# SuperScientificSoftwareLaboratory/PanguLU

Hardware: AMD Instinct MI355X
Metric: numeric factorisation GFLOP/s (pangulu_gstrf, R64) (higher is better)
Workload: dtype f64

## Files before the change

include/pangulu_platform.h:

```cpp
#ifndef PANGULU_PLATFORM_H
#define PANGULU_PLATFORM_H

#include <stddef.h>
#include <stdint.h>

typedef long long int pangulu_int64_t;
typedef unsigned long long int pangulu_uint64_t;
typedef int pangulu_int32_t;
typedef unsigned int pangulu_uint32_t;
typedef short int pangulu_int16_t;
typedef unsigned short int pangulu_uint16_t;

typedef pangulu_uint64_t pangulu_exblock_ptr;
typedef pangulu_uint32_t pangulu_exblock_idx;
typedef pangulu_uint32_t pangulu_inblock_ptr;
typedef pangulu_uint16_t pangulu_inblock_idx;

#if defined(CALCULATE_TYPE_CR64)
#define PANGULU_COMPLEX 1
typedef double calculate_real_type;
#elif defined(CALCULATE_TYPE_CR32)
#define PANGULU_COMPLEX 1
typedef float calculate_real_type;
#elif defined(CALCULATE_TYPE_R32)
typedef float calculate_real_type;
#else
#ifndef CALCULATE_TYPE_R64
#define CALCULATE_TYPE_R64
#endif
typedef double calculate_real_type;
#endif

#ifdef PANGULU_COMPLEX
#if defined(__cplusplus)
typedef struct pangulu_complex_t
{
    calculate_real_type re, im;
} calculate_type;
#elif defined(CALCULATE_TYPE_CR64)
typedef double _Complex calculate_type;
#else
typedef float _Complex calculate_type;
#endif
#else
typedef calculate_real_type calculate_type;
#endif

#define PANGULU_TASK_GETRF 1
#define PANGULU_TASK_TSTRF 2
#define PANGULU_TASK_GESSM 3
#define PANGULU_TASK_SSSSM 4
#define PANGULU_LOWER 0
#define PANGULU_UPPER 1
#define PANGULU_DATA_INVALID 0
#define PANGULU_DATA_PREPARING 1
#define PANGULU_DATA_READY 2
#define PANGULU_TOL 1e-16
#define PANGULU_SPTRSV_TOL 1e-16

#define PANGULU_PLATFORM_CPU_NAIVE 0x0100000
#define PANGULU_PLATFORM_GPU_CUDA 0x0201000
#define PANGULU_PLATFORM_GPU_HIP 0x0201001

#ifdef __cplusplus
extern "C"
{
#endif

    typedef struct pangulu_aggregate_queue_t
    {
        unsigned long long capacity;
        unsigned long long length;
        void *task_descriptors;
    } pangulu_aggregate_queue_t;

    typedef struct pangulu_storage_slot_t
    {
        pangulu_exblock_idx brow_pos;
        pangulu_exblock_idx bcol_pos;
        pangulu_inblock_ptr *columnpointer;
        pangulu_inblock_idx *rowindex;
        calculate_type *value;
        pangulu_inblock_ptr *rowpointer;
        pangulu_inblock_idx *columnindex;
        pangulu_inblock_ptr *idx_of_csc_value_for_csr;
        volatile char data_status;
        struct pangulu_storage_slot_t *related_block;
        pangulu_int32_t is_upper;
        pangulu_int32_t bin_id;
        pangulu_int32_t slot_idx;
        pangulu_aggregate_queue_t *task_queue;
        pangulu_inblock_ptr *d_columnpointer;
        pangulu_inblock_idx *d_rowindex;
        calculate_type *d_value;
        pangulu_inblock_ptr *d_rowpointer;
        pangulu_inblock_idx *d_columnindex;
        pangulu_inblock_ptr *d_idx_of_csc_value_for_csr;
    } pangulu_storage_slot_t;

    typedef struct pangulu_task_t
    {
        pangulu_exblock_idx row;
        pangulu_exblock_idx col;
        pangulu_int16_t kernel_id;
        pangulu_exblock_idx task_level;
        pangulu_int64_t compare_flag;
        pangulu_storage_slot_t *opdst;
        pangulu_storage_slot_t *op1;
        pangulu_storage_slot_t *op2;
    } pangulu_task_t;

#if defined(__cplusplus)
    static_assert(sizeof(pangulu_storage_slot_t) == 144, "slot ABI must match src/pangulu_common.h:207-231 (GPU_OPEN)");
    static_assert(offsetof(pangulu_storage_slot_t, value) == 24, "slot ABI");
    static_assert(offsetof(pangulu_storage_slot_t, related_block) == 64, "slot ABI");
    static_assert(offsetof(pangulu_storage_slot_t, d_columnpointer) == 96, "slot ABI");
    static_assert(offsetof(pangulu_storage_slot_t, d_value) == 112, "slot ABI");
    static_assert(sizeof(pangulu_task_t) == 48, "task ABI must match src/pangulu_common.h:233-243");
    static_assert(offsetof(pangulu_task_t, opdst) == 24, "task ABI");
#endif

    extern int pangulu_gpu_kernel_warp_per_block;
    extern int pangulu_gpu_data_move_warp_per_block;
    extern int pangulu_gpu_shared_mem_size;

    void pangulu_platform_0201001_malloc(void **platform_address, size_t size);
    void pangulu_platform_0201001_malloc_pinned(void **platform_address, size_t size);
    void pangulu_platform_0201001_synchronize(void);
    void pangulu_platform_0201001_memset(void *s, int c, size_t n);
    void pangulu_platform_0201001_create_stream(void **stream);
    void pangulu_platform_0201001_memcpy(void *dst, const void *src, size_t count, unsigned int kind);
    void pangulu_platform_0201001_memcpy_async(void *dst, const void *src, size_t count, unsigned int kind, void *stream);
    void pangulu_platform_0201001_free(void *devptr);
    void pangulu_platform_0201001_get_device_num(int *device_num);
    void pangulu_platform_0201001_set_default_device(int device_num);
    void pangulu_platform_0201001_get_device_name(char *name, int device_num);
    void pangulu_platform_0201001_get_device_memory_usage(size_t *used_byte);

    void pangulu_platform_0201001_getrf(pangulu_inblock_idx nb, pangulu_storage_slot_t *opdst, int tid);
    void pangulu_platform_0201001_tstrf(pangulu_inblock_idx nb, pangulu_storage_slot_t *opdst, pangulu_storage_slot_t *opdiag, int tid);
    void pangulu_platform_0201001_gessm(pangulu_inblock_idx nb, pangulu_storage_slot_t *opdst, pangulu_storage_slot_t *opdiag, int tid);
    void pangulu_platform_0201001_ssssm(pangulu_inblock_idx nb, pangulu_storage_slot_t *opdst, pangulu_storage_slot_t *op1, pangulu_storage_slot_t *op2, int tid);
    void pangulu_platform_0201001_ssssm_batched(pangulu_inblock_idx nb, pangulu_uint64_t ntask, pangulu_task_t *tasks);
    void pangulu_platform_0201001_hybrid_batched(pangulu_inblock_idx nb, pangulu_uint64_t ntask, pangulu_task_t *tasks);

    void pangulu_platform_0201001_spmv(pangulu_inblock_idx nb, pangulu_storage_slot_t *a, calculate_type *x, calculate_type *y);
    void pangulu_platform_0201001_vecadd(pangulu_int64_t length, calculate_type *bval, calculate_type *xval);
    void pangulu_platform_0201001_sptrsv(pangulu_inblock_idx nb, pangulu_storage_slot_t *s, calculate_type *xval, pangulu_int64_t uplo);

#define PANGULU_HIP_OPT_HOST_MIRROR 1
#define PANGULU_HIP_OPT_DENSE_THRESHOLD_PERMILLE 2
#define PANGULU_HIP_OPT_PROFILE 3
#define PANGULU_HIP_OPT_ASSUME_INDEPENDENT 4
#define PANGULU_HIP_OPT_GETRF_STRICT_ORDER 5
#define PANGULU_HIP_OPT_COUNT_FLOPS 6
#define PANGULU_HIP_OPT_RESET_BLOCK_STATE 7
#define PANGULU_HIP_OPT_SSSSM_GROUP_CHUNK 8
#define PANGULU_HIP_OPT_TRSM_DENSE_PERMILLE 9
#define PANGULU_HIP_OPT_TWO_STREAMS 10
#define PANGULU_HIP_OPT_SMALL_LAUNCH_TASKS 11
#define PANGULU_HIP_OPT_XCD_SWIZZLE 12
#define PANGULU_HIP_OPT_RECORDS_STREAM 13
#define PANGULU_HIP_OPT_BACKGROUND_UPDATES 14
#define PANGULU_HIP_OPT_FRONT_STAGES 15
#define PANGULU_HIP_OPT_TILES_STAGES 16
#define PANGULU_HIP_OPT_QUERY_FREE_MIB 17
    int pangulu_platform_0201001_set_option(int option, long long value);
    void pangulu_platform_0201001_prepare_diag(pangulu_inblock_idx nb, pangulu_storage_slot_t *diag);
    void pangulu_platform_0201001_prepare_blocks(pangulu_inblock_idx nb, pangulu_uint64_t nslot, pangulu_storage_slot_t **slots);
    void *pangulu_platform_0201001_marker_record(void);
    int pangulu_platform_0201001_marker_done(void *marker);
    void pangulu_platform_0201001_marker_wait(void *marker);
    typedef struct pangulu_hip_solve_row_t
    {
        pangulu_exblock_idx brow, nblk;
        pangulu_uint64_t first;
        pangulu_storage_slot_t *diag;
    } pangulu_hip_solve_row_t;
    void pangulu_platform_0201001_block_trsv(pangulu_inblock_idx nb, int upper, pangulu_uint64_t nlevel, const pangulu_uint64_t *level_ptr,
                                             const pangulu_hip_solve_row_t *rows, pangulu_storage_slot_t *const *blk_slots,
                                             const pangulu_exblock_idx *blk_bcol, calculate_type *x, pangulu_uint64_t xlen);
    typedef struct pangulu_hip_solve_sweep_t
    {
        pangulu_uint64_t nlevel;
        const pangulu_uint64_t *level_ptr;
        const pangulu_hip_solve_row_t *rows;
        pangulu_storage_slot_t *const *blk_slots;
        const pangulu_exblock_idx *blk_bcol;
    } pangulu_hip_solve_sweep_t;
    int pangulu_platform_0201001_block_trsm_multi(pangulu_inblock_idx nb, const pangulu_hip_solve_sweep_t *lower, const pangulu_hip_solve_sweep_t *upper,
                                                  calculate_type *X, pangulu_uint64_t xlen, pangulu_uint64_t npanel, const int *w);
    int pangulu_platform_0201001_block_trsm_multi_trans(pangulu_inblock_idx nb, const pangulu_hip_solve_sweep_t *forward_ut,
                                                        const pangulu_hip_solve_sweep_t *backward_lt, int conjugate, calculate_type *X,
                                                        pangulu_uint64_t xlen, pangulu_uint64_t npanel, const int *w);
    typedef struct pangulu_hip_solve_maps_t
    {
        pangulu_uint64_t n, n_user;
        const unsigned int *in_idx, *out_idx;
        const double *s_in, *s_out;
    } pangulu_hip_solve_maps_t;
    int pangulu_platform_0201001_block_trsm_multi_device(pangulu_inblock_idx nb, const pangulu_hip_solve_sweep_t *first,
                                                         const pangulu_hip_solve_sweep_t *second, int mode, calculate_type *d_rhs,
                                                         pangulu_uint64_t ldb, pangulu_uint64_t nrhs, pangulu_uint64_t npanel, const int *w,
                                                         pangulu_uint64_t xlen, const pangulu_hip_solve_maps_t *maps, void **workspace,
                                                         void *caller_stream);
    void pangulu_platform_0201001_solve_workspace_free(void **workspace);
    unsigned long long pangulu_platform_0201001_get_solve_workspace_bytes(void);
    void pangulu_platform_0201001_block_spmv_add(pangulu_inblock_idx nb, pangulu_uint64_t nblk, pangulu_storage_slot_t *const *slots,
                                                 const pangulu_exblock_idx *src_seg, const pangulu_exblock_idx *dst_seg, const int *csr,
                                                 const calculate_type *x, calculate_type *y, pangulu_uint64_t xlen);
    int pangulu_platform_0201001_bind_near_device(int enable);
    long long pangulu_platform_0201001_schedule(int cmd, const void *owner);
    int pangulu_platform_0201001_schedule_range(const void *owner, long long first, long long last);
    void *pangulu_platform_0201001_marker_record_replay(void);
    void *pangulu_platform_0201001_get_stream(void);
#define PANGULU_HIP_STAT_CLASSES 9
    typedef struct pangulu_hip_stats_t
    {
        unsigned long long launches[PANGULU_HIP_STAT_CLASSES];
        unsigned long long tasks[PANGULU_HIP_STAT_CLASSES];
        double alg_bytes[PANGULU_HIP_STAT_CLASSES];
        double flops[PANGULU_HIP_STAT_CLASSES];
        double elapsed_ms[PANGULU_HIP_STAT_CLASSES];
        double mfma_flops_executed;
        unsigned long long trsm_dense_tasks;
        unsigned long long ssssm_front_workgroups, ssssm_general_workgroups;
        unsigned long long chase_launches, chase_solves;
        double ssssm_kernel_ms[2];
        double ssssm_front_flops_executed;
    } pangulu_hip_stats_t;
    void pangulu_platform_0201001_get_stats(pangulu_hip_stats_t *out, int reset);
    void pangulu_platform_0201001_get_memory(unsigned long long out[4]);

#ifdef __cplusplus
}
#endif

#endif
```

pangulu_amd/_lib.py:

```python
import ctypes
import os

import numpy as np

_HERE = os.path.dirname(os.path.abspath(__file__))
REPO_ROOT = os.path.dirname(_HERE)
LIB_DIR = os.environ.get("PANGULU_AMD_LIB_DIR") or os.path.join(_HERE, "lib")

VALUE_TYPES = {
    "r64": (np.float64, 8, 0),
    "r32": (np.float32, 4, 0),
    "cr64": (np.complex128, 16, 1),
    "cr32": (np.complex64, 8, 1),
}


class InitOptions(ctypes.Structure):

    _fields_ = [
        ("nthread", ctypes.c_int),
        ("nb", ctypes.c_int),
        ("gpu_kernel_warp_per_block", ctypes.c_int),
        ("gpu_data_move_warp_per_block", ctypes.c_int),
        ("sizeof_value", ctypes.c_int),
        ("is_complex_matrix", ctypes.c_int),
        ("mpi_recv_buffer_level", ctypes.c_float),
    ]


class GstrfOptions(ctypes.Structure):
    _fields_ = [("reserved_", ctypes.c_char)]


class GstrsOptions(ctypes.Structure):
    _fields_ = [("reserved_", ctypes.c_char)]


class Info(ctypes.Structure):

    _fields_ = [
        ("n", ctypes.c_ulonglong),
        ("nnz", ctypes.c_ulonglong),
        ("nb", ctypes.c_ulonglong),
        ("block_length", ctypes.c_ulonglong),
        ("n_padded", ctypes.c_ulonglong),
        ("symbolic_nnz", ctypes.c_ulonglong),
        ("flop", ctypes.c_longlong),
        ("nblocks_nondiag", ctypes.c_ulonglong),
        ("nblocks_owned", ctypes.c_ulonglong),
        ("ntask_getrf", ctypes.c_ulonglong),
        ("ntask_tstrf", ctypes.c_ulonglong),
        ("ntask_gessm", ctypes.c_ulonglong),
        ("ntask_ssssm", ctypes.c_ulonglong),
        ("owned_bytes", ctypes.c_ulonglong),
        ("recv_blocks", ctypes.c_ulonglong),
        ("sent_bytes", ctypes.c_ulonglong),
        ("recv_bytes", ctypes.c_ulonglong),
        ("time_reorder", ctypes.c_double),
        ("time_symbolic", ctypes.c_double),
        ("time_preprocess", ctypes.c_double),
        ("time_numeric", ctypes.c_double),
        ("time_solve", ctypes.c_double),
        ("time_numeric_host_sched", ctypes.c_double),
        ("model_bytes_total", ctypes.c_double),
        ("model_flop_total", ctypes.c_double),
        ("model_tmin_hbm_bound", ctypes.c_double),
        ("model_tmin_fp_bound", ctypes.c_double),
        ("batches", ctypes.c_ulonglong),
        ("sampled_flop", ctypes.c_double),
        ("sampled_tasks", ctypes.c_ulonglong),
        ("time_numeric_platform", ctypes.c_double),
        ("replayed", ctypes.c_ulonglong),
        ("time_schedule_record", ctypes.c_double),
        ("model_ranks_tstar_max", ctypes.c_double),
        ("model_ranks_tstar_sum", ctypes.c_double),
        ("model_ranks_tstar_hbm", ctypes.c_double),
        ("model_ranks_tstar_fp", ctypes.c_double),
        ("model_ranks_bytes_total", ctypes.c_double),
        ("model_rank_flop_share", ctypes.c_double),
        ("model_rank_time_share", ctypes.c_double),
        ("model_comm_seconds_max", ctypes.c_double),
        ("model_sent_bytes_total", ctypes.c_double),
        ("model_critical_path", ctypes.c_double),
        ("model_critical_path_tasks", ctypes.c_ulonglong),
        ("snapshot_device_bytes", ctypes.c_ulonglong),
        ("model_critical_path_latency", ctypes.c_double),
        ("model_rank_hbm_bytes_max", ctypes.c_double),
        ("model_rank_hbm_records", ctypes.c_double),
        ("model_rank_hbm_received", ctypes.c_double),
        ("model_rank_hbm_mirrors", ctypes.c_double),
        ("inserted_diagonals", ctypes.c_ulonglong),
        ("deferred_queues", ctypes.c_ulonglong),
    ]

    def as_dict(self):
        return {name: getattr(self, name) for name, _ in self._fields_}


class HipStats(ctypes.Structure):

    _fields_ = [
        ("launches", ctypes.c_ulonglong * 9),
        ("tasks", ctypes.c_ulonglong * 9),
        ("alg_bytes", ctypes.c_double * 9),
        ("flops", ctypes.c_double * 9),
        ("elapsed_ms", ctypes.c_double * 9),
        ("mfma_flops_executed", ctypes.c_double),
        ("trsm_dense_tasks", ctypes.c_ulonglong),
        ("ssssm_front_workgroups", ctypes.c_ulonglong),
        ("ssssm_general_workgroups", ctypes.c_ulonglong),
        ("chase_launches", ctypes.c_ulonglong),
        ("chase_solves", ctypes.c_ulonglong),
        ("ssssm_kernel_ms", ctypes.c_double * 2),
        ("ssssm_front_flops_executed", ctypes.c_double),
    ]


KERNEL_CLASSES = {1: "getrf", 2: "tstrf", 3: "gessm", 4: "ssssm_sparse", 5: "ssssm_dense_mfma",
                  6: "densify", 7: "sparsify", 8: "remote_lu_image"}

_cache = {}


def library_path(vtype="r64"):
    return os.path.join(LIB_DIR, "libpangulu_amd_%s.so" % vtype)


def test_library_path(vtype="r64"):
    return os.path.join(REPO_ROOT, "oracle", "_build", "libpangulu_amd_test_%s.so" % vtype)


def load(vtype="r64", test_hooks=False):
    vtype = vtype.lower()
    key = (vtype, bool(test_hooks))
    if key in _cache:
        return _cache[key]
    path = test_library_path(vtype) if test_hooks else library_path(vtype)
    if not os.path.exists(path):
        raise RuntimeError(
            "%s is missing: build it with `python -c 'import __graft_entry__ as g; g.build()'` "
            "(or `make -C pangulu_amd/csrc TYPE=%s`); there is no fallback implementation" % (path, vtype.upper())
        )
    lib = ctypes.CDLL(path, mode=ctypes.RTLD_LOCAL)
    vp, vpp = ctypes.c_void_p, ctypes.POINTER(ctypes.c_void_p)
    lib.pangulu_init.argtypes = [ctypes.c_uint32, ctypes.c_uint64, vp, vp, vp, ctypes.POINTER(InitOptions), vpp]
    lib.pangulu_init.restype = None
    lib.pangulu_gstrf.argtypes = [ctypes.POINTER(GstrfOptions), vpp]
    lib.pangulu_gstrf.restype = None
    lib.pangulu_gstrs.argtypes = [vp, ctypes.POINTER(GstrsOptions), vpp]
    lib.pangulu_gstrs.restype = None
    lib.pangulu_amd_gstrs_multi.argtypes = [vp, ctypes.c_uint32, ctypes.c_uint64, ctypes.POINTER(GstrsOptions), vpp]
    lib.pangulu_amd_gstrs_multi.restype = ctypes.c_int
    lib.pangulu_amd_gstrs_trans.argtypes = [vp, ctypes.c_uint32, ctypes.c_uint64, ctypes.c_int, ctypes.POINTER(GstrsOptions), vpp]
    lib.pangulu_amd_gstrs_trans.restype = ctypes.c_int
    lib.pangulu_amd_gstrs_device.argtypes = [vp, ctypes.c_uint32, ctypes.c_uint64, ctypes.c_int, vp, ctypes.POINTER(GstrsOptions), vpp]
    lib.pangulu_amd_gstrs_device.restype = ctypes.c_int
    lib.pangulu_amd_last_solve_path.argtypes = [vpp, ctypes.POINTER(ctypes.c_int), ctypes.POINTER(ctypes.c_int), ctypes.POINTER(ctypes.c_int)]
    lib.pangulu_amd_last_solve_path.restype = ctypes.c_int
    lib.pangulu_gssv.argtypes = [vp, ctypes.POINTER(GstrfOptions), ctypes.POINTER(GstrsOptions), vpp]
    lib.pangulu_gssv.restype = None
    lib.pangulu_finalize.argtypes = [vpp]
    lib.pangulu_finalize.restype = None

    lib.pangulu_amd_comm_init.argtypes = [ctypes.c_int, ctypes.c_int, ctypes.c_char_p, ctypes.c_int, ctypes.c_int, vp]
    lib.pangulu_amd_comm_init.restype = ctypes.c_int
    lib.pangulu_amd_comm_barrier.restype = None
    lib.pangulu_amd_comm_allreduce_max_f64.argtypes = [vp, ctypes.c_int]
    lib.pangulu_amd_comm_allreduce_max_f64.restype = None
    lib.pangulu_amd_comm_finalize.restype = None
    lib.pangulu_amd_comm_transport.restype = ctypes.c_int
    lib.pangulu_amd_comm_rccl_ranks.restype = ctypes.c_int
    lib.pangulu_amd_comm_rank.restype = ctypes.c_int
    lib.pangulu_amd_comm_size.restype = ctypes.c_int
    if test_hooks:
        lib.pangulu_amd_use_platform_library.argtypes = [ctypes.c_char_p, ctypes.c_uint]
        lib.pangulu_amd_use_platform_library.restype = ctypes.c_int
    lib.pangulu_amd_active_platform.restype = ctypes.c_uint
    lib.pangulu_amd_use_builtin_platform.restype = None
    lib.pangulu_amd_set_ordering.argtypes = [ctypes.c_int]
    lib.pangulu_amd_set_ordering.restype = None
    lib.pangulu_amd_set_user_perm.argtypes = [vp, ctypes.c_uint32]
    lib.pangulu_amd_set_user_perm.restype = None
    lib.pangulu_amd_set_coordinates.argtypes = [vp, ctypes.c_uint32, ctypes.c_int]
    lib.pangulu_amd_set_coordinates.restype = None
    lib.pangulu_amd_set_eager_host_mirror.argtypes = [ctypes.c_int]
    lib.pangulu_amd_set_eager_host_mirror.restype = None
    lib.pangulu_amd_set_scaling.argtypes = [ctypes.c_int]
    lib.pangulu_amd_set_scaling.restype = None
    lib.pangulu_amd_reset_options.restype = None
    lib.pangulu_amd_get_info.argtypes = [vpp, ctypes.POINTER(Info)]
    lib.pangulu_amd_get_info.restype = None
    lib.pangulu_amd_model_roofline.argtypes = [vpp, ctypes.c_double, ctypes.c_double]
    lib.pangulu_amd_model_roofline.restype = None
    lib.pangulu_amd_block_owner.argtypes = [vpp, ctypes.c_uint32, ctypes.c_uint32]
    lib.pangulu_amd_block_owner.restype = ctypes.c_int
    lib.pangulu_amd_rank_model.argtypes = [vpp, vp, vp, vp]
    lib.pangulu_amd_rank_model.restype = ctypes.c_int
    lib.pangulu_amd_owned_block_count.argtypes = [vpp]
    lib.pangulu_amd_owned_block_count.restype = ctypes.c_longlong
    lib.pangulu_amd_owned_block.argtypes = [
        vpp, ctypes.c_longlong, ctypes.POINTER(ctypes.c_uint32), ctypes.POINTER(ctypes.c_uint32),
        ctypes.POINTER(ctypes.c_int), ctypes.POINTER(ctypes.c_ulonglong), vpp, vpp, vpp,
    ]
    lib.pangulu_amd_owned_block.restype = ctypes.c_int
    lib.pangulu_amd_update_values.argtypes = [vpp, vp]
    lib.pangulu_amd_update_values.restype = ctypes.c_int
    lib.pangulu_amd_snapshot.argtypes = [vpp]
    lib.pangulu_amd_snapshot.restype = ctypes.c_int
    lib.pangulu_amd_reset_numeric.argtypes = [vpp]
    lib.pangulu_amd_reset_numeric.restype = ctypes.c_int
    lib.pangulu_amd_set_replay.argtypes = [ctypes.c_int]
    lib.pangulu_amd_set_replay.restype = ctypes.c_int
    lib.pangulu_amd_get_perm.argtypes = [vpp]
    lib.pangulu_amd_get_perm.restype = ctypes.POINTER(ctypes.c_uint32)
    lib.pangulu_amd_apply_lu.argtypes = [vpp, vp, vp]
    lib.pangulu_amd_apply_lu.restype = ctypes.c_int
    lib.pangulu_amd_factor_check.argtypes = [vpp, ctypes.POINTER(ctypes.c_double)]
    lib.pangulu_amd_factor_check.restype = ctypes.c_int
    lib.pangulu_amd_factor_check_vectors.argtypes = [vpp, ctypes.c_int, ctypes.c_ulonglong, ctypes.POINTER(ctypes.c_double)]
    lib.pangulu_amd_factor_check_vectors.restype = ctypes.c_int
    lib.pangulu_amd_model_for_ranks.argtypes = [vpp, ctypes.c_int, ctypes.POINTER(ctypes.c_double)]
    lib.pangulu_amd_model_for_ranks.restype = ctypes.c_int

    lib.pangulu_platform_0201001_set_option.argtypes = [ctypes.c_int, ctypes.c_longlong]
    lib.pangulu_platform_0201001_set_option.restype = ctypes.c_int
    lib.pangulu_platform_0201001_get_stats.argtypes = [ctypes.POINTER(HipStats), ctypes.c_int]
    lib.pangulu_platform_0201001_get_stats.restype = None
    lib.pangulu_platform_0201001_get_stream.restype = ctypes.c_void_p
    lib.pangulu_platform_0201001_get_solve_workspace_bytes.restype = ctypes.c_ulonglong
    _cache[key] = lib
    return lib


PLATFORM_SYMBOLS = [
    "malloc", "malloc_pinned", "synchronize", "memset", "create_stream", "memcpy", "memcpy_async", "free",
    "get_device_num", "set_default_device", "get_device_name", "get_device_memory_usage",
    "getrf", "tstrf", "gessm", "ssssm", "ssssm_batched", "hybrid_batched", "spmv", "vecadd", "sptrsv",
]

HIP_OPT_HOST_MIRROR = 1
HIP_OPT_DENSE_THRESHOLD_PERMILLE = 2
HIP_OPT_PROFILE = 3
HIP_OPT_ASSUME_INDEPENDENT = 4
HIP_OPT_GETRF_STRICT_ORDER = 5
HIP_OPT_COUNT_FLOPS = 6
HIP_OPT_RESET_BLOCK_STATE = 7
HIP_OPT_SSSSM_GROUP_CHUNK = 8
HIP_OPT_TRSM_DENSE_PERMILLE = 9
HIP_OPT_TWO_STREAMS = 10
HIP_OPT_SMALL_LAUNCH_TASKS = 11
HIP_OPT_XCD_SWIZZLE = 12
HIP_OPT_RECORDS_STREAM = 13
HIP_OPT_BACKGROUND_UPDATES = 14
HIP_OPT_FRONT_STAGES = 15
HIP_OPT_TILES_STAGES = 16

ORDER_IDENTITY, ORDER_ND, ORDER_USER = 0, 1, 2
TRANSPORT_HOST, TRANSPORT_RCCL, TRANSPORT_IPC = 0, 1, 2
PLATFORM_CPU_NAIVE = 0x0100000
PLATFORM_GPU_HIP = 0x0201001
```

pangulu_amd/csrc/host/pg_api.cpp:

```cpp
#include <cmath>
#include <cstdarg>
#include <dlfcn.h>
#include <omp.h>
#include <sys/time.h>

#include <sys/mman.h>
#include "pg_host.h"

namespace pg
{
#ifdef PANGULU_COMPLEX
static inline val_t make_value(double re) { return val_t{(decltype(val_t{}.re))re, 0}; }
#else
static inline val_t make_value(double re) { return (val_t)re; }
#endif


void fatal(const char *fmt, ...)
{
    va_list ap;
    va_start(ap, fmt);
    fprintf(stderr, "[PanguLU-AMD ERROR] ");
    vfprintf(stderr, fmt, ap);
    fprintf(stderr, "\n");
    va_end(ap);
    fflush(stderr);
    exit(1);
}

double wall_seconds()
{
    struct timeval tv;
    gettimeofday(&tv, nullptr);
    return (double)tv.tv_sec + 1e-6 * (double)tv.tv_usec;
}

static Platform g_platform;
static bool g_platform_ready = false;
static bool g_platform_builtin = true;

void bind_builtin_hip(Platform &p)
{
    p = Platform();
    p.id = PANGULU_PLATFORM_GPU_HIP;
    p.host_memory = false;
    p.malloc_ = pangulu_platform_0201001_malloc;
    p.malloc_pinned = pangulu_platform_0201001_malloc_pinned;
    p.synchronize = pangulu_platform_0201001_synchronize;
    p.memset_ = pangulu_platform_0201001_memset;
    p.create_stream = pangulu_platform_0201001_create_stream;
    p.memcpy_ = pangulu_platform_0201001_memcpy;
    p.memcpy_async = pangulu_platform_0201001_memcpy_async;
    p.free_ = pangulu_platform_0201001_free;
    p.get_device_num = pangulu_platform_0201001_get_device_num;
    p.set_default_device = pangulu_platform_0201001_set_default_device;
    p.get_device_name = pangulu_platform_0201001_get_device_name;
    p.get_device_memory_usage = pangulu_platform_0201001_get_device_memory_usage;
    p.getrf = pangulu_platform_0201001_getrf;
    p.tstrf = pangulu_platform_0201001_tstrf;
    p.gessm = pangulu_platform_0201001_gessm;
    p.ssssm = pangulu_platform_0201001_ssssm;
    p.ssssm_batched = pangulu_platform_0201001_ssssm_batched;
    p.hybrid_batched = pangulu_platform_0201001_hybrid_batched;
    p.spmv = pangulu_platform_0201001_spmv;
    p.vecadd = pangulu_platform_0201001_vecadd;
    p.sptrsv = pangulu_platform_0201001_sptrsv;
    p.set_option = pangulu_platform_0201001_set_option;
    p.prepare_diag = pangulu_platform_0201001_prepare_diag;
    p.prepare_blocks = pangulu_platform_0201001_prepare_blocks;
    p.marker_record = pangulu_platform_0201001_marker_record;
    p.marker_done = pangulu_platform_0201001_marker_done;
    p.marker_wait = pangulu_platform_0201001_marker_wait;
    p.block_trsv = pangulu_platform_0201001_block_trsv;
    p.block_trsm_multi = pangulu_platform_0201001_block_trsm_multi;
    p.block_trsm_multi_trans = pangulu_platform_0201001_block_trsm_multi_trans;
    p.block_trsm_multi_device = pangulu_platform_0201001_block_trsm_multi_device;
    p.solve_workspace_free = pangulu_platform_0201001_solve_workspace_free;
    p.block_spmv_add = pangulu_platform_0201001_block_spmv_add;
    p.schedule = pangulu_platform_0201001_schedule;
    p.schedule_range = pangulu_platform_0201001_schedule_range;
    p.marker_record_replay = pangulu_platform_0201001_marker_record_replay;
    p.bind_near_device = pangulu_platform_0201001_bind_near_device;
}

Platform &active_platform()
{
    if (!g_platform_ready)
    {
        bind_builtin_hip(g_platform);
        g_platform_ready = true;
        g_platform_builtin = true;
    }
    return g_platform;
}

bool platform_is_builtin_hip() { return g_platform_builtin; }

static Options g_options;
Options &pending_options() { return g_options; }

}

using namespace pg;

namespace
{
struct NearDevice
{
    Platform &plat;
    bool bound = false;
    explicit NearDevice(Platform &p) : plat(p)
    {
        if (!plat.host_memory && plat.bind_near_device)
        {
#pragma omp parallel
            {
            }
            bound = plat.bind_near_device(1) == 0;
        }
    }
    ~NearDevice()
    {
        if (bound)
            plat.bind_near_device(0);
    }
};

inline val_t value_times(val_t v, double s)
{
#ifdef PANGULU_COMPLEX
    return val_t{(calculate_real_type)(v.re * s), (calculate_real_type)(v.im * s)};
#else
    return (val_t)(v * s);
#endif
}
}

const SolveMaps &pg::solve_maps(Solver &S, bool transposed)
{
    SolveMaps &M = S.solve_maps[transposed ? 1 : 0];
    if (M.ready)
        return M;
    const bool scaled = !S.scale_row.empty();
    std::vector<u32> row_idx(S.n, SOLVE_MAP_PAD), col_idx(S.n, SOLVE_MAP_PAD);
    std::vector<double> row_s, col_s;
    if (scaled)
    {
        row_s.assign(S.n, 0.0);
        col_s.assign(S.n, 0.0);
    }
    for (u32 i = 0; i < S.n; i++)
    {
        const u32 j = S.perm[i];
        if (j >= S.n_user)
            continue;
        row_idx[i] = j;
        col_idx[i] = scaled ? S.match_col[j] : j;
        if (scaled)
        {
            row_s[i] = S.scale_row[j];
            col_s[i] = S.scale_col[S.match_col[j]];
        }
    }
    M.in_idx = transposed ? col_idx : row_idx;
    M.out_idx = transposed ? row_idx : col_idx;
    M.s_in = transposed ? col_s : row_s;
    M.s_out = transposed ? row_s : col_s;
    M.ready = true;
    return M;
}

namespace
{
void rhs_into_factor_space(const SolveMaps &M, u32 n, const val_t *rhs, val_t *b)
{
    const bool scaled = !M.s_in.empty();
    for (u32 i = 0; i < n; i++)
    {
        if (M.in_idx[i] == SOLVE_MAP_PAD)
            memset(&b[i], 0, sizeof(val_t));
        else
            b[i] = scaled ? value_times(rhs[M.in_idx[i]], M.s_in[i]) : rhs[M.in_idx[i]];
    }
}
void solution_out_of_factor_space(const SolveMaps &M, u32 n, const val_t *b, val_t *rhs)
{
    const bool scaled = !M.s_out.empty();
    for (u32 i = 0; i < n; i++)
        if (M.out_idx[i] != SOLVE_MAP_PAD)
            rhs[M.out_idx[i]] = scaled ? value_times(b[i], M.s_out[i]) : b[i];
}
void rhs_to_factor_space(Solver &S, const val_t *rhs, val_t *b) { rhs_into_factor_space(solve_maps(S, false), S.n, rhs, b); }
void solution_from_factor_space(Solver &S, const val_t *b, val_t *rhs) { solution_out_of_factor_space(solve_maps(S, false), S.n, b, rhs); }
void rhs_to_factor_space_trans(Solver &S, const val_t *rhs, val_t *b) { rhs_into_factor_space(solve_maps(S, true), S.n, rhs, b); }
void solution_from_factor_space_trans(Solver &S, const val_t *b, val_t *rhs) { solution_out_of_factor_space(solve_maps(S, true), S.n, b, rhs); }
}

extern "C"
{

#ifdef PANGULU_AMD_TEST_HOOKS
    int pangulu_amd_use_platform_library(const char *so_path, unsigned int platform_id)
    {
        void *h = dlopen(so_path, RTLD_NOW | RTLD_LOCAL);
        if (!h)
        {
            fprintf(stderr, "[PanguLU-AMD] cannot load platform library %s: %s\n", so_path, dlerror());
            return 1;
        }
        Platform p;
        p.id = platform_id;
        p.dl_handle = h;
        p.host_memory = (platform_id >> 20) == 0x01;
        char sym[128];
        int missing = 0;
        auto get = [&](const char *name) -> void *
        {
            snprintf(sym, sizeof(sym), "pangulu_platform_%07x_%s", platform_id, name);
            void *f = dlsym(h, sym);
            if (!f)
            {
                fprintf(stderr, "[PanguLU-AMD] %s lacks %s\n", so_path, sym);
                missing++;
            }
            return f;
        };
        p.malloc_ = (void (*)(void **, size_t))get("malloc");
        p.malloc_pinned = (void (*)(void **, size_t))get("malloc_pinned");
        p.synchronize = (void (*)())get("synchronize");
        p.memset_ = (void (*)(void *, int, size_t))get("memset");
        p.create_stream = (void (*)(void **))get("create_stream");
        p.memcpy_ = (void (*)(void *, const void *, size_t, unsigned))get("memcpy");
        p.memcpy_async = (void (*)(void *, const void *, size_t, unsigned, void *))get("memcpy_async");
        p.free_ = (void (*)(void *))get("free");
        p.get_device_num = (void (*)(int *))get("get_device_num");
        p.set_default_device = (void (*)(int))get("set_default_device");
        p.get_device_name = (void (*)(char *, int))get("get_device_name");
        p.get_device_memory_usage = (void (*)(size_t *))get("get_device_memory_usage");
        p.getrf = (void (*)(pangulu_inblock_idx, slot_t *, int))get("getrf");
        p.tstrf = (void (*)(pangulu_inblock_idx, slot_t *, slot_t *, int))get("tstrf");
        p.gessm = (void (*)(pangulu_inblock_idx, slot_t *, slot_t *, int))get("gessm");
        p.ssssm = (void (*)(pangulu_inblock_idx, slot_t *, slot_t *, slot_t *, int))get("ssssm");
        p.ssssm_batched = (void (*)(pangulu_inblock_idx, pangulu_uint64_t, task_t *))get("ssssm_batched");
        p.hybrid_batched = (void (*)(pangulu_inblock_idx, pangulu_uint64_t, task_t *))get("hybrid_batched");
        p.spmv = (void (*)(pangulu_inblock_idx, slot_t *, val_t *, val_t *))get("spmv");
        p.vecadd = (void (*)(pangulu_int64_t, val_t *, val_t *))get("vecadd");
        p.sptrsv = (void (*)(pangulu_inblock_idx, slot_t *, val_t *, pangulu_int64_t))get("sptrsv");
        if (missing)
            return 2;
        snprintf(sym, sizeof(sym), "pangulu_platform_%07x_block_trsm_multi_trans", platform_id);
        p.block_trsm_multi_trans = (int (*)(pangulu_inblock_idx, const pangulu_hip_solve_sweep_t *, const pangulu_hip_solve_sweep_t *, int, val_t *,
                                            pangulu_uint64_t, pangulu_uint64_t, const int *))dlsym(h, sym);
        snprintf(sym, sizeof(sym), "pangulu_platform_%07x_block_trsm_multi_device", platform_id);
        p.block_trsm_multi_device = (decltype(p.block_trsm_multi_device))dlsym(h, sym);
        snprintf(sym, sizeof(sym), "pangulu_platform_%07x_solve_workspace_free", platform_id);
        p.solve_workspace_free = (decltype(p.solve_workspace_free))dlsym(h, sym);
        int (*sz)() = (int (*)())dlsym(h, "pangulu_oracle_sizeof_value");
        if (sz && sz() != (int)sizeof(val_t))
        {
            fprintf(stderr, "[PanguLU-AMD] %s was built for another value type\n", so_path);
            return 3;
        }
        g_platform = p;
        g_platform_ready = true;
        g_platform_builtin = false;
        return 0;
    }

    void pangulu_amd_test_set_analysis_ranks(int size) { set_fake_world(size); }

    void pangulu_amd_test_set_task_sampling(int stride) { g_task_sample_stride = stride < 1 ? 1 : stride; }

    long long pangulu_amd_test_heap_script(long long nscript, const long long *script, const pangulu_task_t *tasks, pangulu_task_t *out)
    {
        TaskHeap heap;
        long long npop = 0;
        for (long long i = 0; i < nscript; i++)
        {
            if (script[i] >= 0)
                heap.push(tasks[script[i]]);
            else if (!heap.pop(out[npop++]))
                return -2;
        }
        return npop;
    }

    int pangulu_amd_test_matching(sparse_index_t n, const sparse_pointer_t *colptr, const sparse_index_t *rowidx, const sparse_value_t *value,
                                  sparse_index_t *col_of_row, double *dr, double *dc)
    {
        CscMatrix A;
        A.n = n;
        A.colptr.assign(colptr, colptr + n + 1);
        A.rowidx.assign(rowidx, rowidx + colptr[n]);
        A.value.assign((const val_t *)value, (const val_t *)value + colptr[n]);
        std::vector<u32> q;
        std::vector<double> r, c;
        if (!max_product_matching(A, q, r, c))
            return 1;
        std::copy(q.begin(), q.end(), col_of_row);
        std::copy(r.begin(), r.end(), dr);
        std::copy(c.begin(), c.end(), dc);
        return 0;
    }

    int pangulu_amd_test_symbolic(sparse_index_t n, const sparse_pointer_t *colptr, const sparse_index_t *rowidx,
                                  sparse_pointer_t **out_ptr, sparse_index_t **out_idx, unsigned long long *out_symbolic_nnz, long long *out_flop)
    {
        CscMatrix A;
        A.n = n;
        A.colptr.assign(colptr, colptr + n + 1);
        A.rowidx.assign(rowidx, rowidx + colptr[n]);
        A.value.assign((size_t)colptr[n], val_t());
        Symbolic sym;
        symbolic_factorize(A, sym);
        *out_ptr = (sparse_pointer_t *)malloc(sizeof(sparse_pointer_t) * ((size_t)n + 1));
        *out_idx = (sparse_index_t *)malloc(sizeof(sparse_index_t) * std::max<size_t>(1, sym.idx.size()));
        std::copy(sym.ptr.begin(), sym.ptr.end(), *out_ptr);
        std::copy(sym.idx.begin(), sym.idx.end(), *out_idx);
        *out_symbolic_nnz = sym.symbolic_nnz;
        *out_flop = sym.flop;
        return 0;
    }
#endif

    void pangulu_amd_use_builtin_platform(void)
    {
        bind_builtin_hip(g_platform);
        g_platform_ready = true;
        g_platform_builtin = true;
    }

    unsigned int pangulu_amd_active_platform(void) { return active_platform().id; }

    int pangulu_amd_comm_init(int rank, int size, const char *addr, int base_port, int transport, const void *nccl_unique_id)
    {
        if (size <= 1)
        {
            set_world(nullptr);
            return 0;
        }
        if (size > 64)
        {
            fprintf(stderr, "[PanguLU-AMD ERROR] %d ranks requested: at most 64 are supported\n", size);
            return 1;
        }
        Platform &plat = active_platform();
        if (!plat.host_memory && plat.get_device_num && plat.set_default_device)
        {
            int ndev = 0;
            plat.get_device_num(&ndev);
            if (ndev > 0)
            {
                const char *lr = getenv("LOCAL_RANK");
                plat.set_default_device(lr ? atoi(lr) % ndev : rank % ndev);
// ... 793 lines not shown
```

pangulu_amd/csrc/host/pg_host.h:

```cpp
#pragma once

#include <atomic>
#include <condition_variable>
#include <cstdint>
#include <cstdio>
#include <cstdlib>
#include <cstring>
#include <mutex>
#include <string>
#include <thread>
#include <deque>
#include <vector>

#include "../../../include/pangulu_amd_ext.h"

namespace pg
{

using u16 = uint16_t;
using u32 = uint32_t;
using u64 = uint64_t;
using i32 = int32_t;
using i64 = int64_t;
using val_t = calculate_type;
using slot_t = pangulu_storage_slot_t;
using task_t = pangulu_task_t;

[[noreturn]] void fatal(const char *fmt, ...);
double wall_seconds();

struct Platform
{
    unsigned id = 0;
    bool host_memory = false;
    void *dl_handle = nullptr;
    void (*malloc_)(void **, size_t) = nullptr;
    void (*malloc_pinned)(void **, size_t) = nullptr;
    void (*synchronize)() = nullptr;
    void (*memset_)(void *, int, size_t) = nullptr;
    void (*create_stream)(void **) = nullptr;
    void (*memcpy_)(void *, const void *, size_t, unsigned) = nullptr;
    void (*memcpy_async)(void *, const void *, size_t, unsigned, void *) = nullptr;
    void (*free_)(void *) = nullptr;
    void (*get_device_num)(int *) = nullptr;
    void (*set_default_device)(int) = nullptr;
    void (*get_device_name)(char *, int) = nullptr;
    void (*get_device_memory_usage)(size_t *) = nullptr;
    void (*getrf)(pangulu_inblock_idx, slot_t *, int) = nullptr;
    void (*tstrf)(pangulu_inblock_idx, slot_t *, slot_t *, int) = nullptr;
    void (*gessm)(pangulu_inblock_idx, slot_t *, slot_t *, int) = nullptr;
    void (*ssssm)(pangulu_inblock_idx, slot_t *, slot_t *, slot_t *, int) = nullptr;
    void (*ssssm_batched)(pangulu_inblock_idx, pangulu_uint64_t, task_t *) = nullptr;
    void (*hybrid_batched)(pangulu_inblock_idx, pangulu_uint64_t, task_t *) = nullptr;
    void (*spmv)(pangulu_inblock_idx, slot_t *, val_t *, val_t *) = nullptr;
    void (*vecadd)(pangulu_int64_t, val_t *, val_t *) = nullptr;
    void (*sptrsv)(pangulu_inblock_idx, slot_t *, val_t *, pangulu_int64_t) = nullptr;
    int (*set_option)(int, long long) = nullptr;
    void (*prepare_diag)(pangulu_inblock_idx, slot_t *) = nullptr;
    void (*prepare_blocks)(pangulu_inblock_idx, pangulu_uint64_t, slot_t **) = nullptr;
    void *(*marker_record)() = nullptr;
    int (*marker_done)(void *) = nullptr;
    void (*marker_wait)(void *) = nullptr;
    int (*bind_near_device)(int) = nullptr;
    void (*block_trsv)(pangulu_inblock_idx, int, pangulu_uint64_t, const pangulu_uint64_t *, const pangulu_hip_solve_row_t *, slot_t *const *,
                       const pangulu_exblock_idx *, val_t *, pangulu_uint64_t) = nullptr;
    long long (*schedule)(int, const void *) = nullptr;
    int (*schedule_range)(const void *, long long, long long) = nullptr;
    void *(*marker_record_replay)() = nullptr;
    void (*block_spmv_add)(pangulu_inblock_idx, pangulu_uint64_t, slot_t *const *, const pangulu_exblock_idx *, const pangulu_exblock_idx *, const int *,
                           const val_t *, val_t *, pangulu_uint64_t) = nullptr;
    int (*block_trsm_multi)(pangulu_inblock_idx, const pangulu_hip_solve_sweep_t *, const pangulu_hip_solve_sweep_t *, val_t *, pangulu_uint64_t,
                            pangulu_uint64_t, const int *) = nullptr;
    int (*block_trsm_multi_trans)(pangulu_inblock_idx, const pangulu_hip_solve_sweep_t *, const pangulu_hip_solve_sweep_t *, int, val_t *,
                                  pangulu_uint64_t, pangulu_uint64_t, const int *) = nullptr;
    int (*block_trsm_multi_device)(pangulu_inblock_idx, const pangulu_hip_solve_sweep_t *, const pangulu_hip_solve_sweep_t *, int, val_t *,
                                   pangulu_uint64_t, pangulu_uint64_t, pangulu_uint64_t, const int *, pangulu_uint64_t,
                                   const pangulu_hip_solve_maps_t *, void **, void *) = nullptr;
    void (*solve_workspace_free)(void **) = nullptr;
};
Platform &active_platform();
bool platform_is_builtin_hip();

struct CscMatrix
{
    u32 n = 0;
    std::vector<u64> colptr;
    std::vector<u32> rowidx;
    std::vector<val_t> value;
    u64 nnz() const { return colptr.empty() ? 0 : colptr.back(); }
};

void order_identity(u32 n, std::vector<u32> &perm);
void order_nested_dissection(const CscMatrix &A, const double *coords, int dim, u32 align, std::vector<u32> &perm);
void permute_symmetric(const CscMatrix &A, const std::vector<u32> &perm, CscMatrix &B);

struct Symbolic
{
    u32 n = 0;
    std::vector<u64> ptr;
    std::vector<u32> idx;
    u64 symbolic_nnz = 0;
    i64 flop = 0;
};
void symbolic_factorize(const CscMatrix &A, Symbolic &S);

struct BlockPattern
{
    u32 nb = 0, nbk = 0, n = 0;
    std::vector<u64> lcolptr;
    std::vector<u32> lrowidx;
    std::vector<u32> lnnz;
    std::vector<u64> colptr, first_after_diag;
    std::vector<u32> rowidx;
    std::vector<u64> rowptr, first_after_diag_csr, csr_to_csc;
    std::vector<u32> colidx;
    std::vector<u32> nnz;
    std::vector<u32> diag_lower_nnz;
    std::vector<u32> diag_upper_nnz;
    u64 find(u32 br, u32 bc) const;
};
void build_block_pattern(const Symbolic &S, u32 nb, BlockPattern &P);

size_t record_bytes(u32 nb, u64 nnz, bool lower_offdiag);
void bind_record(slot_t &s, u32 nb, u64 nnz, char *hrec, char *drec, bool lower_offdiag, bool diag_upper);

struct RecvBin
{
    size_t slot_capacity = 0;
    std::vector<slot_t> slots;
    std::deque<i32> free_list;
    char *hbuf = nullptr, *dbuf = nullptr;
};

struct Storage
{
    u32 nb = 0;
    std::vector<slot_t> owned;
    size_t n_owned_nondiag = 0;
    char *harena = nullptr, *darena = nullptr;
    std::vector<char *> dchunks;
    size_t dchunk_bytes = 0;
    char *device_ptr(size_t off) const { return dchunks.empty() ? darena + off : dchunks[off / dchunk_bytes] + off % dchunk_bytes; }
    size_t chunk_len(size_t c) const { return std::min(dchunk_bytes, arena_bytes - c * dchunk_bytes); }
    size_t arena_bytes = 0;
    std::vector<RecvBin> bins;
    std::mutex mutex;
    slot_t *allocate(size_t bytes);
    void recycle(slot_t *s);
};

struct TaskHeap
{
    std::vector<task_t> store;
    std::vector<i64> heap;
    std::vector<i64> free_ids;
    std::mutex mutex;
    void reserve(size_t cap);
    void clear();
    void push(const task_t &t);
    bool pop(task_t &out);
    bool empty();
    size_t size();
    static bool before(const task_t &a, const task_t &b);
};

struct BlockHeader
{
    u64 nnz;
    u32 brow, bcol;
    u32 is_upper;
    u32 bytes_lo;
    u64 reserved;
};
static_assert(sizeof(BlockHeader) == 32, "record header is 32 bytes");

struct Marker
{
    std::atomic<void *> ev{nullptr};
};

class Comm
{
public:
    int rank = 0, size = 1;
    int transport = PANGULU_AMD_TRANSPORT_HOST;
    virtual ~Comm() {}
    virtual void barrier() = 0;
    virtual void bcast(void *buf, size_t bytes, int root) = 0;
    virtual void allreduce_sum_i64(i64 *v, int count) = 0;
    virtual void allreduce_max_f64(double *v, int count) = 0;
    virtual void send_bytes(int dst, int tag, const void *buf, size_t bytes) = 0;
    virtual void recv_bytes(int src, int tag, void *buf, size_t bytes) = 0;
    virtual void isend_block(slot_t *s, const BlockHeader &h, int dst) = 0;
    virtual bool probe_block(BlockHeader &h, int &src) = 0;
    virtual void recv_block(slot_t *s, const BlockHeader &h, int src) = 0;
    virtual void recv_block_begin(slot_t *s, const BlockHeader &h, int src) { recv_block(s, h, src); }
    virtual void recv_blocks_finish() {}
    virtual void flush_sends() = 0;
    virtual bool set_send_gate(Marker * ) { return false; }
    virtual void register_arena(char *const * , size_t , size_t , size_t ) {}
    u64 sent_bytes = 0, recv_bytes_total = 0;
    virtual int rccl_ranks() const { return 0; }
    bool abandoned = false;
};
Comm *world();
void set_world(Comm *c);
void set_fake_world(int size);
Comm *make_socket_comm(int rank, int size, const char *addr, int base_port, int transport, const void *nccl_id);
int rccl_make_unique_id(void *out128);
Comm *make_rccl_comm(int rank, int size, const char *addr, int base_port, const void *nccl_id);
Comm *make_ipc_comm(int rank, int size, const char *addr, int base_port);

bool max_product_matching(const CscMatrix &A, std::vector<u32> &col_of_row, std::vector<double> &dr, std::vector<double> &dc);
void apply_matching(const CscMatrix &A, const std::vector<u32> &col_of_row, const std::vector<double> &dr, const std::vector<double> &dc, CscMatrix &out);

struct Options
{
    bool scaling = false;
    int ordering = PANGULU_AMD_ORDER_ND;
    std::vector<u32> user_perm;
    std::vector<double> coords;
    int coord_dim = 0;
    bool eager_host_mirror = false;
};
Options &pending_options();

struct TaskModel
{
    double bytes[5] = {0, 0, 0, 0, 0};
    double flop[5] = {0, 0, 0, 0, 0};
    u64 count[5] = {0, 0, 0, 0, 0};
};

struct StructureModel
{
    double hbm_bytes_per_s = 8e12, fp_flops_per_s = 78.6e12, link_bytes_per_s = 153e9;
    std::vector<u16> lcount;
    std::vector<double> col_time, col_flop;
    std::vector<double> rank_time_hbm, rank_time_fp, rank_flop, rank_bytes, rank_comm_s;
    std::vector<double> sent_bytes;
    std::vector<double> rank_mem_records, rank_mem_recv, rank_mem_mirrors;
    double critical_path_s = 0;
    double critical_path_latency_s = 0;
    u64 critical_path_tasks = 0;
};

struct SolveSweepPlan
{
    u32 nlevel = 0;
    std::vector<pangulu_uint64_t> level_ptr;
    std::vector<pangulu_hip_solve_row_t> rows;
    std::vector<slot_t *> blk_slots;
    std::vector<pangulu_exblock_idx> blk_bcol;
};

constexpr u32 SOLVE_MAP_PAD = 0xffffffffu;
struct SolveMaps
{
    std::vector<u32> in_idx, out_idx;
    std::vector<double> s_in, s_out;
    bool ready = false;
};

struct Solver
{
    u32 n = 0, nb = 0, nbk = 0;
    u32 n_user = 0;
    int rank = 0, nproc = 1, p = 1, q = 1;
    float recv_buffer_level = 0.5f;
    bool eager_host_mirror = false;
    std::vector<u32> match_col;
    std::vector<double> scale_row, scale_col;
    std::vector<u32> perm, iperm;
    Symbolic sym;
    BlockPattern pat;
    CscMatrix Aperm;
    std::vector<u64> user_colptr;
    std::vector<u32> user_rowidx;
    Storage storage;
    std::vector<slot_t *> slot_of;
    std::vector<slot_t *> diag_lower, diag_upper;
    std::vector<i32> remain;
    std::vector<u64> consumers;
    std::vector<i32> remain_diag;
    std::vector<i32> remain0, remain_diag0;
    i64 rank_remain_task = 0, rank_remain_task0 = 0;
    i64 rank_remain_recv = 0, rank_remain_recv0 = 0;
    TaskHeap heap;
    std::mutex info_mutex;
    std::vector<std::vector<task_t>> pending;
    std::vector<u32> pending_dirty;
    u64 pending_total = 0;
    bool factored = false, host_values_current = true;
    bool schedule_recorded = false;
    SolveSweepPlan solve_plan[2];
    bool solve_plan_ready = false;
    SolveSweepPlan solve_plan_trans[2];
    bool solve_plan_trans_ready = false;
    int last_solve_device_columns = 0, last_solve_panel_width = 0, last_solve_panels = 0;
    SolveMaps solve_maps[2];
    void *solve_workspace = nullptr;
    struct RankLog
    {
        struct Entry
        {
            long long op_end = 0;
            int marker = -1;
            u32 need = 0;
        };
        struct Send
        {
            int marker;
            slot_t *slot;
            BlockHeader h;
            int dst;
        };
        struct Arrival
        {
            u32 brow, bcol, is_upper;
            slot_t *slot;
            u64 nnz;
        };
        std::vector<Entry> entries;
        std::vector<Send> sends;
        std::vector<Arrival> arrivals;
        int nmarkers = 0;
        bool valid = false, slot_reused = false;
        bool unusable = false;
    };
    RankLog rank_log;
    char *arena_snapshot = nullptr;
    bool snapshot_on_host = false;
    std::vector<char *> snapshot_dchunks;
    pangulu_amd_info_t info;
    TaskModel model;
    StructureModel smodel;
    std::vector<int> home;
    struct Group
    {
        unsigned short lo, p, q;
    };
    std::vector<Group> grp;
    bool analysis_only = false;
    int owner(u32 br, u32 bc) const
    {
        if (!home.empty())
        {
            const u32 c = br < bc ? br : bc;
            const int h = home[c];
            if (h >= 0)
                return h;
            if (!grp.empty())
            {
                const Group &g = grp[c];
                return (int)(g.lo + (br % g.p) * g.q + (bc % g.q));
            }
        }
        return (int)((br % (u32)p) * (u32)q + (bc % (u32)q));
    }
    ~Solver();
};

void assign_subtrees(Solver &S);
void preprocess(Solver &S, const CscMatrix &Aperm);
void scatter_values(Solver &S, const CscMatrix &Aperm);
void reload_values(Solver &S, const CscMatrix &Aperm);
void numeric_factorize(Solver &S);
void record_schedule(Solver &S);
void download_factors(Solver &S);
void triangular_solve(Solver &S, val_t *rhs_permuted);
void triangular_solve_multi(Solver &S, val_t *B, u32 nrhs);
void triangular_solve_multi_trans(Solver &S, val_t *B, u32 nrhs, bool conjugate);
const SolveMaps &solve_maps(Solver &S, bool transposed);
int triangular_solve_device(Solver &S, val_t *d_rhs, u32 nrhs, u64 ldb, int trans, void *stream);
void drop_solve_workspace(Solver &S);
double factor_check(Solver &S);
double factor_check_vectors(Solver &S, int nvec, unsigned long long seed);
void compute_task_model(Solver &S, double hbm_bytes_per_s, double fp_flops_per_s);
void build_structure_model(Solver &S);
void evaluate_model_for_ranks(Solver &S, int nranks, double *out12);
void compute_rank_model(Solver &S);
double task_structural_flop(u32 nb, const task_t &t);
extern int g_task_sample_stride;
extern int g_replay_enabled;

}
```

pangulu_amd/csrc/host/pg_preprocess.cpp:

```cpp
#include <algorithm>
#include <cmath>
#include <queue>
#include <string>
#include <omp.h>
#include <sys/mman.h>

#include "pg_host.h"

namespace pg
{

static inline size_t pad8(size_t x) { return (x + 7) & ~(size_t)7; }

size_t record_bytes(u32 nb, u64 nnz, bool lower_offdiag)
{
    size_t sz = 32 + sizeof(val_t) * nnz + sizeof(pangulu_inblock_ptr) * (nb + 1) + sizeof(pangulu_inblock_idx) * nnz;
    sz = pad8(sz);
    if (lower_offdiag)
    {
        sz += sizeof(pangulu_inblock_ptr) * nnz + sizeof(pangulu_inblock_ptr) * (nb + 1) + sizeof(pangulu_inblock_idx) * nnz;
        sz = pad8(sz);
    }
    return sz;
}
// ... 186 lines not shown
            w.lo = 0;
            w.cnt = np;
            todo.push_back(std::move(w));
        }
        while (!todo.empty())
        {
            Work w = std::move(todo.back());
            todo.pop_back();
            if (w.nodes.empty())
                continue;
            if (w.cnt == 1)
            {
                for (u32 k : w.nodes)
                    whole_subtree_to(k, w.lo);
                continue;
            }
            if (w.nodes.size() == 1)
            {
                const u32 k = w.nodes[0];
                if (own[k] >= heavy_abs || own[k] >= heavy_rel)
                {
                    int p = (int)std::sqrt((double)w.cnt);
                    while (w.cnt % p)
                        p--;
                    S.grp[k] = Solver::Group{(unsigned short)w.lo, (unsigned short)p, (unsigned short)(w.cnt / p)};
                    for (int r = w.lo; r < w.lo + w.cnt; r++)
                        load[(size_t)r] += own[k] / w.cnt;
                    ndist++;
                }
                else
                {
                    int best = w.lo;
                    for (int r = w.lo; r < w.lo + w.cnt; r++)
                        if (load[(size_t)r] < load[(size_t)best])
                            best = r;
                    S.home[k] = best;
                    load[(size_t)best] += own[k];
                }
                Work next;
                next.nodes = kids[k];
                next.lo = w.lo;
                next.cnt = w.cnt;
                todo.push_back(std::move(next));
                continue;
            }
            std::sort(w.nodes.begin(), w.nodes.end(), [&](u32 a, u32 b)
                      { return sub[a] > sub[b] || (sub[a] == sub[b] && a < b); });
            double wsum = 0;
            for (u32 k : w.nodes)
                wsum += sub[k];
            const double ideal0 = wsum > 0 ? sub[w.nodes[0]] / wsum * w.cnt : 0.0;
            Work h[2];
            if (ideal0 >= (double)w.cnt - 0.5)
            {
                for (size_t t = 1; t < w.nodes.size(); t++)
                {
                    int best = w.lo;
                    for (int r = w.lo; r < w.lo + w.cnt; r++)
                        if (load[(size_t)r] < load[(size_t)best])
                            best = r;
                    whole_subtree_to(w.nodes[t], best);
                }
                h[0].nodes.assign(1, w.nodes[0]);
                h[0].lo = w.lo;
                h[0].cnt = w.cnt;
            }
            else if (ideal0 >= 1.0)
            {
                const int c0 = std::max(1, std::min(w.cnt - 1, (int)std::floor(ideal0 + 0.5)));
                h[0].nodes.assign(1, w.nodes[0]);
                h[0].lo = w.lo;
                h[0].cnt = c0;
                h[1].nodes.assign(w.nodes.begin() + 1, w.nodes.end());
                h[1].lo = w.lo + c0;
                h[1].cnt = w.cnt - c0;
            }
            else
            {
                h[0].lo = w.lo;
                h[0].cnt = (w.cnt + 1) / 2;
                h[1].lo = w.lo + h[0].cnt;
                h[1].cnt = w.cnt - h[0].cnt;
                double wt[2] = {0, 0};
                for (u32 k : w.nodes)
                {
                    const int side = (wt[0] / h[0].cnt <= wt[1] / h[1].cnt) ? 0 : 1;
                    h[side].nodes.push_back(k);
                    wt[side] += sub[k];
                }
            }
            todo.push_back(std::move(h[1]));
            todo.push_back(std::move(h[0]));
        }
    }
    else
    {
        const char *per_env = getenv("PANGULU_AMD_SUBTREES_PER_RANK");
        const double per_rank = per_env ? atof(per_env) : 8.0;
        const double target = total / (per_rank * (double)np);
        auto cmp = [&](u32 a, u32 b)
        { return sub[a] < sub[b] || (sub[a] == sub[b] && a > b); };
        std::priority_queue<u32, std::vector<u32>, decltype(cmp)> pq(cmp);
        for (u32 k = 0; k < nbk; k++)
            if (parent[k] == NONE)
                pq.push(k);
        while (!pq.empty() && sub[pq.top()] > target)
        {
            u32 k = pq.top();
            pq.pop();
            for (u32 c : kids[k])
                pq.push(c);
        }
        while (!pq.empty())
        {
            u32 root = pq.top();
            pq.pop();
            whole_subtree_to(root, (int)(std::min_element(load.begin(), load.end()) - load.begin()));
        }
        if (mode == "rank0")
        {
            for (u32 k = 0; k < nbk; k++)
                if (S.home[k] < 0)
                    S.home[k] = 0;
        }
        else if (mode == "path")
        {
            for (u32 k = 0; k < nbk; k++)
                if (S.home[k] < 0)
                {
                    int best = -1;
                    double w = -1;
                    for (u32 c : kids[k])
                        if (S.home[c] >= 0 && sub[c] > w)
                        {
                            w = sub[c];
                            best = S.home[c];
                        }
                    S.home[k] = best >= 0 ? best : 0;
                }
        }
        else if (mode != "cyclic")
            fatal("PANGULU_AMD_SEPARATOR_MAP must be group, path, cyclic or rank0");
    }
    if (S.rank == 0 && getenv("PANGULU_AMD_TRACE"))
    {
        size_t top = 0;
        for (int h : S.home)
            top += h < 0;
        fprintf(stderr, "[pangulu_amd trace] mapping '%s': %zu whole subtrees over %d ranks, %zu of %u block columns distributed block-cyclic (%zu over rank groups)\n",
                mode.c_str(), nsub, np, top, nbk, ndist);
    }
}

void scatter_values(Solver &S, const CscMatrix &A)
{
    const BlockPattern &P = S.pat;
    const u32 nb = S.nb, n = S.n;
    const int me = S.rank;
#pragma omp parallel for schedule(dynamic, 256)
    for (i64 j_ = 0; j_ < (i64)n; j_++)
    {
        u32 j = (u32)j_, bj = j / nb, c = j % nb;
        for (u64 p = A.colptr[j]; p < A.colptr[j + 1]; p++)
        {
            u32 i = A.rowidx[p], bi = i / nb, r = i % nb;
            slot_t *s = nullptr;
            bool csr_row_search = false;
            if (bi == bj)
            {
                if (i > j)
                    s = S.diag_lower[bj];
                else
                {
                    s = S.diag_upper[bj];
                    csr_row_search = true;
                }
            }
            else
            {
                if (S.owner(bi, bj) != me)
                    continue;
                u64 b = P.find(bi, bj);
                if (b == ~0ull)
                    fatal("entry (%u,%u) of A outside the symbolic block pattern", i, j);
                s = S.slot_of[b];
            }
            if (!s)
                continue;
            u32 major = csr_row_search ? r : c, minor = csr_row_search ? c : r;
            const pangulu_inblock_idx *b0 = s->rowindex + s->columnpointer[major];
            const pangulu_inblock_idx *b1 = s->rowindex + s->columnpointer[major + 1];
            const pangulu_inblock_idx *hit = std::lower_bound(b0, b1, (pangulu_inblock_idx)minor);
            if (hit == b1 || *hit != minor)
                fatal("entry (%u,%u) of A outside the symbolic pattern", i, j);
            s->value[hit - s->rowindex] = A.value[p];
        }
    }
}

void reload_values(Solver &S, const CscMatrix &A)
{
    Platform &plat = active_platform();
    Storage &st = S.storage;
    const u32 nb = S.nb;
    for (auto &s : st.owned)
        if (s.value)
            memset((void *)s.value, 0, sizeof(val_t) * (size_t)s.columnpointer[nb]);
    scatter_values(S, A);
    if (!plat.host_memory)
    {
        plat.synchronize();
        for (size_t c = 0; c < st.dchunks.size(); c++)
            plat.memcpy_(st.dchunks[c], st.harena + c * st.dchunk_bytes, st.chunk_len(c), 0);
        plat.synchronize();
    }
    S.remain = S.remain0;
    S.remain_diag = S.remain_diag0;
    S.rank_remain_task = S.rank_remain_task0;
    S.rank_remain_recv = S.rank_remain_recv0;
    for (auto &s : st.owned)
        s.data_status = PANGULU_DATA_PREPARING;
    for (auto &q : S.pending)
        q.clear();
    S.pending_dirty.clear();
    S.pending_total = 0;
    S.factored = false;
    S.host_values_current = true;
}

void preprocess(Solver &S, const CscMatrix &A)
{
    assign_subtrees(S);
    const BlockPattern &P = S.pat;
    const Symbolic &sym = S.sym;
    Platform &plat = active_platform();
    u32 nb = S.nb, nbk = S.nbk, n = S.n;
    int me = S.rank;
    u64 nblk = P.colptr[nbk];

    const bool trace_pre = getenv("PANGULU_AMD_TRACE") != nullptr && S.rank == 0;
    double t_mark = wall_seconds();
    auto lap = [&](const char *what)
    {
        const double now = wall_seconds();
        if (trace_pre)
            fprintf(stderr, "[pangulu_amd trace] preprocess: %s %.2f s\n", what, now - t_mark);
        t_mark = now;
    };
    Storage &st = S.storage;
    st.nb = nb;
    std::vector<u64> owned_bidx;
    for (u32 bc = 0; bc < nbk; bc++)
        for (u64 b = P.colptr[bc]; b < P.colptr[bc + 1]; b++)
            if (S.owner(P.rowidx[b], bc) == me)
                owned_bidx.push_back(b);
    std::vector<u32> owned_diag;
    for (u32 k = 0; k < nbk; k++)
        if (S.owner(k, k) == me)
            owned_diag.push_back(k);
    st.n_owned_nondiag = owned_bidx.size();
    st.owned.assign(owned_bidx.size() + 2 * owned_diag.size(), slot_t());
    for (auto &s : st.owned)
        memset((void *)&s, 0, sizeof(slot_t));

    std::vector<size_t> off(st.owned.size() + 1, 0);
    auto align64 = [](size_t x)
    { return (x + 63) & ~(size_t)63; };
    size_t cursor = 0;
    const char *chunk_env = getenv("PANGULU_AMD_ARENA_CHUNK_MB");
    const size_t chunk = (size_t)(chunk_env ? atol(chunk_env) : 1024) << 20;
    auto place = [&](size_t bytes)
    {
        if (bytes > chunk)
            fatal("a block record of %zu bytes does not fit an arena chunk (PANGULU_AMD_ARENA_CHUNK_MB)", bytes);
        if (cursor / chunk != (cursor + bytes - 1) / chunk)
            cursor = (cursor / chunk + 1) * chunk;
        size_t at = cursor;
        cursor = align64(cursor + bytes);
        return at;
    };
    for (size_t i = 0; i < owned_bidx.size(); i++)
    {
        u64 b = owned_bidx[i];
        u32 br = P.rowidx[b];
        u32 bc = (u32)(std::upper_bound(P.colptr.begin(), P.colptr.end(), b) - P.colptr.begin() - 1);
        off[i] = place(record_bytes(nb, P.nnz[b], br > bc));
    }
    for (size_t d = 0; d < owned_diag.size(); d++)
    {
        u32 k = owned_diag[d];
        size_t i = owned_bidx.size() + 2 * d;
        off[i] = place(record_bytes(nb, P.diag_lower_nnz[k], false));
        off[i + 1] = place(record_bytes(nb, P.diag_upper_nnz[k], false));
    }
    st.arena_bytes = cursor ? cursor : 64;
    S.info.nblocks_owned = st.owned.size();
    S.info.owned_bytes = st.arena_bytes;
    const bool analysis_only = S.analysis_only;
    if (analysis_only)
        st.arena_bytes = 64;
    if (posix_memalign((void **)&st.harena, st.arena_bytes >= ((size_t)2 << 20) ? ((size_t)2 << 20) : 64, st.arena_bytes) != 0)
        fatal("host arena allocation of %zu bytes failed", st.arena_bytes);
#ifdef MADV_HUGEPAGE
    if (st.arena_bytes >= ((size_t)2 << 20) && !getenv("PANGULU_AMD_NO_HUGEPAGES"))
        (void)madvise(st.harena, st.arena_bytes, MADV_HUGEPAGE);
#endif
    lap("mapping + slots");
    {
        const size_t piece = (size_t)64 << 20;
        const i64 npiece = (i64)((st.arena_bytes + piece - 1) / piece);
#pragma omp parallel for schedule(static)
        for (i64 k = 0; k < npiece; k++)
            memset(st.harena + (size_t)k * piece, 0, std::min(piece, st.arena_bytes - (size_t)k * piece));
    }
    lap("host arena zeroed");
    if (plat.host_memory || analysis_only)
    {
        st.darena = st.harena;
    }
    else
    {
        st.dchunk_bytes = chunk;
        size_t nchunks = (st.arena_bytes + chunk - 1) / chunk;
        st.dchunks.assign(nchunks, nullptr);
        for (size_t c = 0; c < nchunks; c++)
            plat.malloc_((void **)&st.dchunks[c], st.chunk_len(c));
    }

    S.slot_of.assign(nblk, nullptr);
    S.diag_lower.assign(nbk, nullptr);
    S.diag_upper.assign(nbk, nullptr);
    for (size_t i = 0; i < owned_bidx.size() && !analysis_only; i++)
    {
        u64 b = owned_bidx[i];
        u32 br = P.rowidx[b];
        u32 bc = (u32)(std::upper_bound(P.colptr.begin(), P.colptr.end(), b) - P.colptr.begin() - 1);
        slot_t &s = st.owned[i];
        s.brow_pos = br;
        s.bcol_pos = bc;
        s.is_upper = 0;
        s.bin_id = 0;
        s.slot_idx = (i32)i;
        s.data_status = PANGULU_DATA_PREPARING;
        bind_record(s, nb, P.nnz[b], st.harena + off[i], st.device_ptr(off[i]), br > bc, false);
        S.slot_of[b] = &s;
    }
    for (size_t d = 0; d < owned_diag.size() && !analysis_only; d++)
    {
        u32 k = owned_diag[d];
        size_t i = owned_bidx.size() + 2 * d;
        slot_t &lo = st.owned[i], &up = st.owned[i + 1];
        lo.brow_pos = lo.bcol_pos = up.brow_pos = up.bcol_pos = k;
        lo.is_upper = 0;
        up.is_upper = 1;
        lo.slot_idx = (i32)i;
        up.slot_idx = (i32)(i + 1);
        lo.related_block = &up;
        up.related_block = &lo;
        lo.data_status = up.data_status = PANGULU_DATA_PREPARING;
        bind_record(lo, nb, P.diag_lower_nnz[k], st.harena + off[i], st.device_ptr(off[i]), false, false);
        bind_record(up, nb, P.diag_upper_nnz[k], st.harena + off[i + 1], st.device_ptr(off[i + 1]), false, true);
        S.diag_lower[k] = &lo;
        S.diag_upper[k] = &up;
    }
    lap("device arena + records bound");
#pragma omp parallel if (!analysis_only)
    {
        std::vector<i64> local_of(nbk, -1);
        std::vector<std::vector<pangulu_inblock_idx>> tmp_ri;
        std::vector<std::vector<pangulu_inblock_ptr>> tmp_cp;
        std::vector<u32> cursor_nnz;
#pragma omp for schedule(dynamic, 2)
        for (i64 bc_ = 0; bc_ < (analysis_only ? (i64)0 : (i64)nbk); bc_++)
        {
            u32 bc = (u32)bc_;
            u64 l0 = P.lcolptr[bc], l1 = P.lcolptr[bc + 1];
            size_t nl = (size_t)(l1 - l0);
            std::vector<char> need(nl, 0);
            bool any = false;
            for (size_t t = 0; t < nl; t++)
            {
                u32 br = P.lrowidx[l0 + t];
                bool mine = (br == bc) ? (S.owner(bc, bc) == me) : (S.owner(br, bc) == me || S.owner(bc, br) == me);
                need[t] = mine;
                any |= mine;
                local_of[br] = (i64)t;
            }
            if (any)
            {
                tmp_ri.assign(nl, {});
                tmp_cp.assign(nl, {});
                for (size_t t = 0; t < nl; t++)
                    if (need[t])
                    {
                        tmp_ri[t].reserve(P.lnnz[l0 + t]);
                        tmp_cp[t].assign(nb + 1, 0);
                    }
                u32 j0 = bc * nb, j1 = std::min(n, j0 + nb);
                for (u32 j = j0; j < j1; j++)
                {
                    u32 c = j - j0;
                    for (u64 p = sym.ptr[j]; p < sym.ptr[j + 1]; p++)
                    {
                        u32 i = sym.idx[p];
                        i64 t = local_of[i / nb];
                        if (t >= 0 && need[(size_t)t])
                        {
                            tmp_ri[(size_t)t].push_back((pangulu_inblock_idx)(i % nb));
                        }
                    }
                    for (size_t t = 0; t < nl; t++)
                        if (need[t])
                            tmp_cp[t][c + 1] = (pangulu_inblock_ptr)tmp_ri[t].size();
                }
                for (u32 c = j1 - j0; c < nb; c++)
                    for (size_t t = 0; t < nl; t++)
                        if (need[t])
                            tmp_cp[t][c + 1] = (pangulu_inblock_ptr)tmp_ri[t].size();

                for (size_t t = 0; t < nl; t++)
                {
                    if (!need[t])
                        continue;
                    u32 br = P.lrowidx[l0 + t];
                    const auto &cp = tmp_cp[t];
                    const auto &ri = tmp_ri[t];
                    if (br == bc)
                    {
                        slot_t *lo = S.diag_lower[bc], *up = S.diag_upper[bc];
                        u32 ol = 0, ou = 0;
                        lo->columnpointer[0] = 0;
                        up->columnpointer[0] = 0;
                        for (u32 c = 0; c < nb; c++)
                        {
                            for (u32 p = cp[c]; p < cp[c + 1]; p++)
                            {
                                u32 r = ri[p];
                                up->rowindex[ou++] = (pangulu_inblock_idx)r;
                                if (r != c)
                                    lo->rowindex[ol++] = (pangulu_inblock_idx)r;
                            }
                            lo->columnpointer[c + 1] = ol;
                            up->columnpointer[c + 1] = ou;
                        }
                        continue;
                    }
                    u64 bl = P.find(br, bc);
                    u64 bu = P.find(bc, br);
                    slot_t *sl = S.slot_of[bl], *su = S.slot_of[bu];
                    if (sl)
                    {
                        std::copy(cp.begin(), cp.end(), sl->columnpointer);
                        std::copy(ri.begin(), ri.end(), sl->rowindex);
                        transpose_inblock(nb, sl->columnpointer, sl->rowindex, sl->rowpointer, sl->columnindex, sl->idx_of_csc_value_for_csr);
                    }
                    if (su)
                    {
                        transpose_inblock(nb, cp.data(), ri.data(), su->columnpointer, su->rowindex, nullptr);
                    }
                }
            }
            for (size_t t = 0; t < nl; t++)
                local_of[P.lrowidx[l0 + t]] = -1;
        }
    }

    if (!analysis_only)
        scatter_values(S, A);

    lap("patterns + values into the records");
    S.remain.assign(nblk, 0);
    S.remain_diag.assign(nbk, 0);
    const bool consumer_rule = S.nproc > 1 && S.nproc <= 64 && !getenv("PANGULU_AMD_REFERENCE_FORWARDING");
    S.consumers.clear();
    if (consumer_rule)
        S.consumers.assign(nblk, 0);
    i64 my_ssssm = 0;
#pragma omp parallel
    {
        std::vector<i64> pos(nbk, -1);
#pragma omp for schedule(dynamic, 2) reduction(+ : my_ssssm)
        for (i64 b_ = 0; b_ < (i64)nbk; b_++)
        {
            u32 b = (u32)b_;
            for (u64 t = P.colptr[b]; t < P.colptr[b + 1]; t++)
                pos[P.rowidx[t]] = (i64)t;
            for (u64 t = P.colptr[b]; t < P.first_after_diag[b]; t++)
            {
                u32 k = P.rowidx[t];
                u64 ukb = t;
                for (u64 la = P.first_after_diag[k]; la < P.colptr[k + 1]; la++)
                {
                    u32 a = P.rowidx[la];
                    bool dst_mine;
                    if (consumer_rule && (a == b || pos[a] >= 0))
                    {
                        const int od = a == b ? S.owner(b, b) : S.owner(a, b);
                        if (S.owner(a, k) != od)
                        {
#pragma omp atomic
                            S.consumers[la] |= 1ull << od;
                        }
                        if (S.owner(k, b) != od)
                        {
#pragma omp atomic
                            S.consumers[ukb] |= 1ull << od;
                        }
                    }
                    if (a == b)
                    {
                        dst_mine = S.owner(b, b) == me;
                        if (dst_mine)
                        {
#pragma omp atomic
                            S.remain_diag[b]++;
                        }
                    }
                    else
                    {
                        i64 d = pos[a];
                        if (d < 0)
                            continue;
                        dst_mine = S.owner(a, b) == me;
                        if (dst_mine)
                            S.remain[(size_t)d]++;
                    }
                    if (dst_mine)
                    {
                        my_ssssm++;
                        if (S.owner(a, k) != me)
                        {
#pragma omp atomic
                            S.remain[la]++;
                        }
                        if (S.owner(k, b) != me)
                        {
#pragma omp atomic
                            S.remain[ukb]++;
                        }
                    }
                }
            }
            for (u64 t = P.colptr[b]; t < P.colptr[b + 1]; t++)
                pos[P.rowidx[t]] = -1;
        }
    }
    i64 my_tasks = 0, my_getrf = 0, my_tstrf = 0, my_gessm = 0, my_recv = 0;
    std::vector<i64> last_owned_col(nbk, -1), last_owned_row(nbk, -1);
    for (u32 bc = 0; bc < nbk; bc++)
        for (u64 t = P.colptr[bc]; t < P.colptr[bc + 1]; t++)
            if (S.owner(P.rowidx[t], bc) == me)
            {
                u32 br = P.rowidx[t];
                last_owned_col[br] = std::max<i64>(last_owned_col[br], bc);
                last_owned_row[bc] = std::max<i64>(last_owned_row[bc], br);
            }
    for (u32 k = 0; k < nbk; k++)
        if (S.owner(k, k) == me)
        {
            last_owned_col[k] = std::max<i64>(last_owned_col[k], k);
            last_owned_row[k] = std::max<i64>(last_owned_row[k], k);
        }
    for (u32 bc = 0; bc < nbk; bc++)
    {
        for (u64 t = P.colptr[bc]; t < P.colptr[bc + 1]; t++)
        {
            u32 br = P.rowidx[t];
            if (S.owner(br, bc) == me)
            {
                S.remain[t] += 1;
                my_tasks++;
                u32 level = std::min(br, bc);
                if (br > bc)
                    my_tstrf++;
                else
                    my_gessm++;
                if (S.owner(level, level) != me)
                    S.remain_diag[level]++;
            }
            else
            {
                bool sent_to_me = consumer_rule ? ((S.consumers[t] >> me) & 1ull) != 0
                                                : ((br > bc) ? (last_owned_col[br] > (i64)bc) : (last_owned_row[bc] > (i64)br));
                if (sent_to_me)
                    my_recv++;
            }
        }
    }
    for (u32 k = 0; k < nbk; k++)
    {
        if (S.owner(k, k) == me)
        {
            S.remain_diag[k] += 1;
            my_tasks++;
            my_getrf++;
        }
        else if (S.remain_diag[k] > 0)
        {
            bool need_u = false, need_l = false;
            for (u64 t = P.first_after_diag[k]; t < P.colptr[k + 1] && !need_u; t++)
                need_u = S.owner(P.rowidx[t], k) == me;
            for (u64 t = P.first_after_diag_csr[k]; t < P.rowptr[k + 1] && !need_l; t++)
                need_l = S.owner(k, P.colidx[t]) == me;
            my_recv += (need_u ? 1 : 0) + (need_l ? 1 : 0);
        }
    }
    S.rank_remain_task = my_tasks;
    S.rank_remain_recv = my_recv;
    S.remain0 = S.remain;
    S.remain_diag0 = S.remain_diag;
    S.rank_remain_task0 = S.rank_remain_task;
    S.rank_remain_recv0 = S.rank_remain_recv;
    S.info.ntask_getrf = (u64)my_getrf;
    S.info.ntask_tstrf = (u64)my_tstrf;
    S.info.ntask_gessm = (u64)my_gessm;
    S.info.ntask_ssssm = (u64)my_ssssm;
    S.info.recv_blocks = (u64)my_recv;
    S.heap.reserve((size_t)my_tasks + 1);
    S.pending.assign(st.owned.size(), {});

    lap("dependency counters");
    st.bins.clear();
    st.bins.resize(7);
    if (S.nproc > 1 && !analysis_only)
    {
        u64 full = (u64)nb * nb;
        u64 cls_nnz[7] = {0,
                          std::max<u64>(5, full / 1024),
                          std::max<u64>(4ull * nb, full / 256),
                          std::max<u64>((u64)nb * std::max<u32>(nb / 100, 8), full / 64),
                          full / 16,
                          full / 4,
                          full};
        for (int b = 1; b <= 6; b++)
            cls_nnz[b] = std::min(cls_nnz[b], full);
        u64 need_cnt[7] = {0, 0, 0, 0, 0, 0, 0};
        size_t cls_cap[7] = {0, 0, 0, 0, 0, 0, 0};
        for (int b = 1; b <= 6; b++)
            cls_cap[b] = (record_bytes(nb, cls_nnz[b], true) + 63) & ~(size_t)63;
        auto classify = [&](u64 nnz, bool lower_offdiag)
        {
            const size_t bytes = record_bytes(nb, nnz, lower_offdiag);
            for (int b = 1; b <= 6; b++)
                if (bytes <= cls_cap[b])
                    return b;
            return 6;
        };
        for (u32 bc = 0; bc < nbk; bc++)
            for (u64 t = P.colptr[bc]; t < P.colptr[bc + 1]; t++)
            {
                u32 br = P.rowidx[t];
                if (S.owner(br, bc) == me)
                    continue;
                bool sent_to_me = consumer_rule ? ((S.consumers[t] >> me) & 1ull) != 0
                                                : ((br > bc) ? (last_owned_col[br] > (i64)bc) : (last_owned_row[bc] > (i64)br));
                if (sent_to_me)
                    need_cnt[classify(P.nnz[t], br > bc)]++;
            }
        for (u32 k = 0; k < nbk; k++)
            if (S.owner(k, k) != me && S.remain_diag[k] > 0)
            {
                need_cnt[classify(P.diag_lower_nnz[k], false)]++;
                need_cnt[classify(P.diag_upper_nnz[k], false)]++;
            }
        float level = S.recv_buffer_level > 0 ? S.recv_buffer_level : 0.5f;
        const char *budget_env = getenv("PANGULU_AMD_RECV_BUDGET_GB");
        double budget = (budget_env ? atof(budget_env) : 48.0) * 1e9;
        double full_bytes = 0;
        for (int b = 1; b <= 6; b++)
            full_bytes += (double)((record_bytes(nb, cls_nnz[b], true) + 63) & ~(size_t)63) * (double)(need_cnt[b] + 2);
        bool provision_all = full_bytes <= budget;
        for (int b = 1; b <= 6; b++)
        {
            RecvBin &bin = st.bins[b];
            bin.slot_capacity = (record_bytes(nb, cls_nnz[b], true) + 63) & ~(size_t)63;
            u64 want = (u64)(level * (float)need_cnt[b]) + 64;
            u64 cnt = provision_all ? need_cnt[b] + 2 : std::min<u64>(need_cnt[b] + 2, want);
            if (need_cnt[b] == 0)
                cnt = 0;
            size_t bytes = bin.slot_capacity * cnt;
            bin.slots.assign(cnt, slot_t());
            bin.free_list.clear();
            if (cnt == 0)
                continue;
            if (posix_memalign((void **)&bin.hbuf, 64, bytes) != 0)
                fatal("receive bin allocation failed");
            if (plat.host_memory)
                bin.dbuf = bin.hbuf;
            else
                plat.malloc_((void **)&bin.dbuf, bytes);
            for (u64 i = 0; i < cnt; i++)
            {
                slot_t &s = bin.slots[i];
                memset((void *)&s, 0, sizeof(slot_t));
                s.value = (val_t *)(bin.hbuf + i * bin.slot_capacity + 32);
                s.d_value = (val_t *)(bin.dbuf + i * bin.slot_capacity + 32);
                s.bin_id = b;
                s.slot_idx = (i32)i;
                bin.free_list.push_back((i32)i);
            }
        }
    }

    lap("receive bins");
    if (!plat.host_memory && !analysis_only)
    {
        for (size_t c = 0; c < st.dchunks.size(); c++)
            plat.memcpy_(st.dchunks[c], st.harena + c * st.dchunk_bytes, st.chunk_len(c), 0);
        plat.synchronize();
        lap("upload of the records");
        if (plat.prepare_diag)
            for (u32 k : owned_diag)
                plat.prepare_diag((pangulu_inblock_idx)nb, S.diag_lower[k]);
        if (plat.prepare_blocks && st.n_owned_nondiag)
        {
            std::vector<slot_t *> offdiag(st.n_owned_nondiag);
            for (size_t i = 0; i < st.n_owned_nondiag; i++)
                offdiag[i] = &st.owned[i];
            plat.prepare_blocks((pangulu_inblock_idx)nb, offdiag.size(), offdiag.data());
        }
        lap("back-end preparation (diagonal column views, pattern summaries)");
    }
    if (world()->size > 1 && !analysis_only)
        world()->register_arena(st.dchunks.data(), plat.host_memory ? 0 : st.dchunks.size(), st.dchunk_bytes, st.arena_bytes);
    S.host_values_current = true;
}

void download_factors(Solver &S)
{
    if (S.host_values_current)
        return;
    Platform &plat = active_platform();
    if (!plat.host_memory)
    {
        plat.synchronize();
        for (size_t c = 0; c < S.storage.dchunks.size(); c++)
            plat.memcpy_(S.storage.harena + c * S.storage.dchunk_bytes, S.storage.dchunks[c], S.storage.chunk_len(c), 1);
    }
    S.host_values_current = true;
}

Solver::~Solver()
{
    Platform &plat = active_platform();
    drop_solve_workspace(*this);
    if (schedule_recorded && plat.schedule)
        plat.schedule(0, this);
    for (char *c : snapshot_dchunks)
        if (c)
            plat.free_(c);
    if (arena_snapshot)
    {
        if (plat.host_memory || snapshot_on_host)
            free(arena_snapshot);
        else
            plat.free_(arena_snapshot);
    }
    if (storage.harena)
    {
        for (char *c : storage.dchunks)
            if (c)
                plat.free_(c);
        free(storage.harena);
    }
    for (auto &bin : storage.bins)
    {
        if (bin.hbuf)
        {
            if (!plat.host_memory && bin.dbuf)
                plat.free_(bin.dbuf);
            free(bin.hbuf);
        }
    }
}

}
```

pangulu_amd/csrc/platform/pg_hip_backend.h:

```cpp
#pragma once

struct DiagAux
{
    u32 *d_cp = nullptr;
    u16 *d_ri = nullptr;
    u32 *d_vi = nullptr;
    u32 nnz = 0;
    u32 brow = 0;
};

struct Ring
{
    static const int NSEG = 32;
    std::vector<int> pending;
    size_t seg_bytes = 0;
    char *h = nullptr, *d = nullptr;
    hipEvent_t ev[NSEG];
    bool used[NSEG];
    int cur = 0;
};

struct EventPair
{
    hipEvent_t a, b;
    int cls;
    int split_cls;
    double split_frac;
    unsigned long long tag[3];
};

#define PG_FLOP_WORDS 48

struct Backend
{
    bool ready = false;
    int device = 0;
    hipStream_t stream = nullptr;
    bool bulk_streams_masked = false;
    hipStream_t stream2 = nullptr;
    hipStream_t stream3 = nullptr;
    hipEvent_t ev_fork = nullptr, ev_join = nullptr, ev_fork3 = nullptr, ev_join3 = nullptr;
    hipStream_t stream_front = nullptr;
    hipEvent_t ev_front_fork = nullptr, ev_front_join = nullptr;
    long long opt_front_fork = 1;
    bool getrf_join_pending = false;
    hipStream_t stream_rec = nullptr;
    hipEvent_t ev_rec_fork = nullptr, ev_rec = nullptr;
    std::atomic<bool> rec_dirty{false};
    hipStream_t stream_bg = nullptr;
    hipEvent_t ev_bg_fork = nullptr, ev_bg_done = nullptr;
    hipStream_t stream_early = nullptr;
    bool bg_active = false;
    std::unordered_set<const void *> bg_tiles;
    long long opt_background_updates = 1;
    long long opt_front_stages = 2;
    long long opt_front_min_wgs = 2048;
    long long opt_ksplit = 1;
    long long opt_front_unit = 1;
    long long opt_tiles_stages = 2;
    long long opt_tiles_unit = 1;
    unsigned long long front_workgroups = 0, general_workgroups = 0;
    long long opt_records_stream = 1;
    int nb_cfg = 0;
    unsigned long long generation = 0;
    long long opt_host_mirror = 1;
    long long opt_dense_permille = 2;
    long long opt_profile = 0;
    long long opt_assume_independent = 0;
    long long opt_getrf_strict = 0;
    long long opt_count_flops = 1;
    long long opt_group_chunk = 8;
    long long opt_small_launch_tasks = 2048;
    long long opt_trsm_dense_permille = 5;
    long long opt_two_streams = 1;
    double mfma_flops_executed = 0;
    Ring ring;
    unsigned *d_progress = nullptr;
    size_t progress_next = 0;
    unsigned long long chase_launches = 0, chase_solves = 0;
    unsigned long long zgetrf_tasks = 0;
    unsigned long long *d_flops = nullptr;
    val_t *getrf_scratch = nullptr;
    int getrf_scratch_slots = 0;
    std::unordered_map<const void *, DiagAux> diag_aux;
    pangulu_hip_stats_t stats;
    std::vector<EventPair> pending_events;
    std::vector<hipEvent_t> event_pool;
    std::mutex mutex;
};

Backend B;

struct Recorder
{
    int mode = 0;
    bool valid = false;
    const void *owner = nullptr;
    unsigned long long signature = 0;
    std::vector<std::function<void()>> ops;
    std::vector<std::function<void()>> prologue;
    bool in_prologue = false;
    std::vector<hipEvent_t> early_events;
    struct Seg
    {
        char *h, *d, *twin;
        size_t cap;
    };
    std::vector<Seg> segs;
    size_t descriptor_bytes = 0;
    bool pack = false;
    struct Tail
    {
        int seg;
        size_t used;
    };
    std::vector<Tail> tails;
    int nb = 0;
    unsigned long long generation = 0;
    pangulu_hip_stats_t stats_before, stats_delta;
    unsigned long long wgs_before[4] = {0, 0, 0, 0}, wgs_delta[4] = {0, 0, 0, 0};
};
Recorder REC;

#define PROGRESS_WORDS 8192
struct PendingGetrf
{
    bool active = false, hold = false;
    int nb = 0;
    size_t take = 0;
    const void *d_tasks = nullptr;
    unsigned *d_progress = nullptr;
    std::vector<const double *> images;
    std::function<void()> plain;
    std::function<void()> post;
};
PendingGetrf PEND;
inline void flush_pending_getrf()
{
    if (!PEND.active || PEND.hold)
        return;
    PEND.active = false;
    PEND.plain();
    PEND.post();
    PEND.plain = nullptr;
    PEND.post = nullptr;
}

inline void flush_pending_getrf_locked();

template <class T>
inline T rec_xl(T v)
{
    if constexpr (std::is_pointer<T>::value)
    {
        const char *p = reinterpret_cast<const char *>(v);
        for (const Recorder::Seg &sg : REC.segs)
            if (p >= sg.d && p < sg.d + sg.cap)
                return reinterpret_cast<T>(const_cast<char *>(sg.twin + (p - sg.d)));
    }
    return v;
}

template <class K, class... A>
inline void pg_launch(K kernel, dim3 grid, dim3 block, size_t shmem, hipStream_t st, A... args)
{
    flush_pending_getrf();
    if (REC.mode != 0)
    {
        auto targs = std::make_tuple(rec_xl(args)...);
        (REC.in_prologue ? REC.prologue : REC.ops).emplace_back([=]()
                             { std::apply([&](auto... a)
                                          { hipLaunchKernelGGL(kernel, grid, block, (unsigned)shmem, st, a...); },
                                          targs); });
        if (REC.mode == 2)
            return;
    }
    hipLaunchKernelGGL(kernel, grid, block, (unsigned)shmem, st, args...);
}
#define PG_LAUNCH(kernel_, grid_, block_, shmem_, stream_, ...) pg_launch(kernel_, grid_, block_, shmem_, stream_, __VA_ARGS__)

inline void pg_event_record(hipEvent_t e, hipStream_t s)
{
    flush_pending_getrf();
    if (REC.mode != 0)
        (REC.in_prologue ? REC.prologue : REC.ops).emplace_back([e, s]() { HIP_CHECK(hipEventRecord(e, s)); });
    if (REC.mode != 2)
        HIP_CHECK(hipEventRecord(e, s));
}
inline void pg_stream_wait(hipStream_t s, hipEvent_t e)
{
    flush_pending_getrf();
    if (REC.mode != 0)
        REC.ops.emplace_back([e, s]() { HIP_CHECK(hipStreamWaitEvent(s, e, 0)); });
    if (REC.mode != 2)
        HIP_CHECK(hipStreamWaitEvent(s, e, 0));
}

inline void flush_pending_getrf_locked()
{
    if (!PEND.active)
        return;
    std::lock_guard<std::mutex> g(B.mutex);
    flush_pending_getrf();
}

void ensure_ready()
{
    if (B.ready)
        return;
    int ndev = 0;
    hipError_t e = hipGetDeviceCount(&ndev);
    if (e != hipSuccess || ndev <= 0)
    {
        fprintf(stderr, "[PanguLU-AMD ERROR] no HIP device available (%s); the GPU_HIP platform has no CPU fallback\n",
                e == hipSuccess ? "device count is 0" : hipGetErrorString(e));
        exit(EXIT_FAILURE);
    }
    HIP_CHECK(hipSetDevice(B.device));
    {
        long reserved = 0;
        if (const char *e = getenv("PANGULU_HIP_RESERVED_CUS"))
            reserved = atol(e);
        hipDeviceProp_t prop;
        HIP_CHECK(hipGetDeviceProperties(&prop, B.device));
        const int ncu = prop.multiProcessorCount;
        if (reserved > 0 && reserved < ncu / 2 && ncu % 32 == 0)
        {
            std::vector<uint32_t> mask((size_t)ncu / 32, 0xFFFFFFFFu);
            for (int i = ncu - (int)reserved; i < ncu; i++)
                mask[(size_t)i / 32] &= ~(1u << (i % 32));
            HIP_CHECK(hipExtStreamCreateWithCUMask(&B.stream, (uint32_t)mask.size(), mask.data()));
            HIP_CHECK(hipExtStreamCreateWithCUMask(&B.stream2, (uint32_t)mask.size(), mask.data()));
            B.bulk_streams_masked = true;
        }
        else
        {
            HIP_CHECK(hipStreamCreateWithFlags(&B.stream, hipStreamNonBlocking));
            HIP_CHECK(hipStreamCreateWithFlags(&B.stream2, hipStreamNonBlocking));
        }
    }
    HIP_CHECK(hipStreamCreateWithFlags(&B.stream_front, hipStreamNonBlocking));
    HIP_CHECK(hipEventCreateWithFlags(&B.ev_front_fork, hipEventDisableTiming));
    HIP_CHECK(hipEventCreateWithFlags(&B.ev_front_join, hipEventDisableTiming));
    if (const char *e = getenv("PANGULU_HIP_FRONT_FORK"))
        B.opt_front_fork = atol(e);
    HIP_CHECK(hipEventCreateWithFlags(&B.ev_fork, hipEventDisableTiming));
    HIP_CHECK(hipEventCreateWithFlags(&B.ev_join, hipEventDisableTiming));
    HIP_CHECK(hipStreamCreateWithFlags(&B.stream3, hipStreamNonBlocking));
    HIP_CHECK(hipEventCreateWithFlags(&B.ev_fork3, hipEventDisableTiming));
    HIP_CHECK(hipEventCreateWithFlags(&B.ev_join3, hipEventDisableTiming));
    HIP_CHECK(hipStreamCreateWithFlags(&B.stream_rec, hipStreamNonBlocking));
    HIP_CHECK(hipEventCreateWithFlags(&B.ev_rec_fork, hipEventDisableTiming));
    HIP_CHECK(hipEventCreateWithFlags(&B.ev_rec, hipEventDisableTiming));
    if (const char *e = getenv("PANGULU_HIP_RECORDS_STREAM"))
        B.opt_records_stream = atol(e);
    HIP_CHECK(hipStreamCreateWithFlags(&B.stream_early, hipStreamNonBlocking));
    HIP_CHECK(hipStreamCreateWithFlags(&B.stream_bg, hipStreamNonBlocking));
    HIP_CHECK(hipEventCreateWithFlags(&B.ev_bg_fork, hipEventDisableTiming));
    HIP_CHECK(hipEventCreateWithFlags(&B.ev_bg_done, hipEventDisableTiming));
    if (const char *e = getenv("PANGULU_HIP_BACKGROUND_UPDATES"))
        B.opt_background_updates = atol(e);
    if (const char *e = getenv("PANGULU_HIP_FRONT_STAGES"))
        B.opt_front_stages = atol(e);
    if (const char *e = getenv("PANGULU_HIP_FRONT_UNIT"))
        B.opt_front_unit = atol(e);
    if (const char *e = getenv("PANGULU_HIP_FRONT_MIN_WGS"))
        B.opt_front_min_wgs = atol(e);
    if (const char *e = getenv("PANGULU_HIP_KSPLIT"))
        B.opt_ksplit = atol(e);
    if (const char *e = getenv("PANGULU_HIP_TILES_STAGES"))
        B.opt_tiles_stages = atol(e);
    if (const char *e = getenv("PANGULU_HIP_GROUP_CHUNK"))
        B.opt_group_chunk = atol(e);
    if (const char *e = getenv("PANGULU_HIP_TILES_UNIT"))
        B.opt_tiles_unit = atol(e);
    if (const char *e = getenv("PANGULU_HIP_DENSE_PERMILLE"))
        B.opt_dense_permille = atol(e);
    if (const char *e = getenv("PANGULU_HIP_TRSM_DENSE_PERMILLE"))
        B.opt_trsm_dense_permille = atol(e);
    if (const char *e = getenv("PANGULU_HIP_SMALL_LAUNCH_TASKS"))
        B.opt_small_launch_tasks = atol(e);
    B.ring.seg_bytes = (size_t)8 << 20;
    HIP_CHECK(hipHostMalloc((void **)&B.ring.h, B.ring.seg_bytes * Ring::NSEG, hipHostMallocNonCoherent | hipHostMallocMapped));
    HIP_CHECK(hipHostGetDevicePointer((void **)&B.ring.d, B.ring.h, 0));
    for (int i = 0; i < Ring::NSEG; i++)
    {
        HIP_CHECK(hipEventCreateWithFlags(&B.ring.ev[i], hipEventDisableTiming));
        B.ring.used[i] = false;
    }
    HIP_CHECK(hipMalloc((void **)&B.d_flops, sizeof(unsigned long long) * PG_FLOP_WORDS));
    HIP_CHECK(hipMemset(B.d_flops, 0, sizeof(unsigned long long) * PG_FLOP_WORDS));
    memset(&B.stats, 0, sizeof(B.stats));
    B.ready = true;
}

struct Segment
{
    char *h, *d;
    size_t cap, used;
    int index;
    int rec_idx = -1;
    size_t rec_off = 0;
    template <typename T>
    T *alloc(size_t count, T **dev)
    {
        size_t off = (used + 15) & ~(size_t)15;
        if (off + sizeof(T) * count > cap)
            return nullptr;
        used = off + sizeof(T) * count;
        *dev = reinterpret_cast<T *>(d + off);
        return reinterpret_cast<T *>(h + off);
    }
};

double g_host_seconds[6] = {0, 0, 0, 0, 0, 0};
struct HostTimer
{
    int k;
    std::chrono::steady_clock::time_point t0;
    explicit HostTimer(int k_) : k(k_), t0(std::chrono::steady_clock::now()) {}
    ~HostTimer() { g_host_seconds[k] += std::chrono::duration<double>(std::chrono::steady_clock::now() - t0).count(); }
};

void release_pending_segments(hipStream_t on = nullptr)
{
    Ring &r = B.ring;
    for (int i : r.pending)
    {
        HIP_CHECK(hipEventRecord(r.ev[i], on ? on : B.stream));
        r.used[i] = true;
    }
    r.pending.clear();
}

void join_records(hipStream_t s)
{
    if (!B.rec_dirty.load(std::memory_order_acquire))
        return;
    pg_stream_wait(s, B.ev_rec);
    if (s == B.stream)
        B.rec_dirty.store(false, std::memory_order_release);
}

void join_background(hipStream_t s)
{
    if (!B.bg_active)
        return;
    pg_stream_wait(s, B.ev_bg_done);
    if (s == B.stream)
    {
        B.bg_active = false;
        B.bg_tiles.clear();
    }
}

Segment acquire_segment(size_t want = 0)
{
    Ring &r = B.ring;
    if (REC.mode != 0)
    {
        const size_t min_room = want ? std::min(r.seg_bytes, (want + 4096 + 65535) & ~(size_t)65535) : ((size_t)2 << 20);
        for (size_t k = REC.tails.size(); k-- > 0;)
        {
            const Recorder::Tail t = REC.tails[k];
            const Recorder::Seg &sg = REC.segs[(size_t)t.seg];
            if (sg.cap - t.used < min_room)
                continue;
            REC.tails.erase(REC.tails.begin() + (long)k);
            Segment s;
            s.h = sg.h + t.used;
            s.d = sg.d + t.used;
            s.cap = sg.cap - t.used;
            s.used = 0;
            s.index = -2;
            s.rec_idx = t.seg;
            s.rec_off = t.used;
            return s;
        }
        const size_t bytes = std::min(r.seg_bytes, std::max(min_room, (size_t)4 << 20));
        char *h = nullptr, *d = nullptr, *twin = nullptr;
        HIP_CHECK(hipHostMalloc((void **)&h, bytes, hipHostMallocNonCoherent | hipHostMallocMapped));
        HIP_CHECK(hipHostGetDevicePointer((void **)&d, h, 0));
        HIP_CHECK(hipMalloc((void **)&twin, bytes));
        REC.segs.push_back(Recorder::Seg{h, d, twin, bytes});
        REC.descriptor_bytes += bytes;
        Segment s;
        s.h = h;
        s.d = d;
        s.cap = bytes;
        s.used = 0;
        s.index = -2;
        s.rec_idx = (int)REC.segs.size() - 1;
        s.rec_off = 0;
        return s;
    }
    int i = r.cur;
    r.cur = (r.cur + 1) % Ring::NSEG;
    if (r.used[i])
// ... 201 lines not shown
```

pangulu_amd/csrc/platform/pg_hip_dense.h:

```cpp
#pragma once

#define MIRROR_MAP_BYTES 64
__host__ __device__ inline size_t mirror_plane_stride(int nb)
{
    return (size_t)nb * nb + MIRROR_MAP_BYTES / sizeof(double) + (size_t)16 * nb;
}
__device__ inline const unsigned short *mirror_map(const double *mirror, int nb)
{
    return reinterpret_cast<const unsigned short *>(mirror + (size_t)nb * nb);
}

#define DG_TILE 128
#define DG_K 16
__device__ inline const char __attribute__((address_space(1))) *dg_scalar_base(const char __attribute__((address_space(1))) *p)
{
    unsigned long long v = (unsigned long long)p;
    asm("" : "+s"(v));
    return (const char __attribute__((address_space(1))) *)v;
}
__device__ inline unsigned dg_lane_offset(unsigned v)
{
    asm("" : "+v"(v));
    return v;
}
// ... 284 lines not shown
                }
    }
    else
    {
#pragma unroll
        for (int ni = 0; ni < DG_NI; ni++)
#pragma unroll
            for (int mi = 0; mi < 4; mi++)
                acc[ni][mi] = (v4f64){0.0, 0.0, 0.0, 0.0};
    }
#if DG_WAVES == 8
    DG_FETCH(ab1, bb1, k01, pa1, pb1, sg1)
    DG_STAMP(1)
    DG_STORE_LDS(0, raX, rbX, sg0)
    DG_STAMP(2)
    __syncthreads();
    DG_STAMP(3)
    do
    {
        DG_LOAD_SLAB(raX, rbX, ab1, bb1, k01, pa1, pb1)
        DG_STAMP(4)
        DG_PRODUCTS(0, ab0, bb0)
        DG_STAMP(5)
        DG_STORE_LDS(1, raX, rbX, sg1)
        DG_STAMP(2)
        __syncthreads();
        DG_STAMP(3)
        DG_FETCH(ab0, bb0, k00, pa0, pb0, sg0)
        DG_LOAD_SLAB(raX, rbX, ab0, bb0, k00, pa0, pb0)
        DG_STAMP(4)
        DG_PRODUCTS(1, ab1, bb1)
        DG_STAMP(5)
        if (stamping)
            atomicAdd(&dbg[7], (ab1 ? 2ull : 1ull));
        DG_STORE_LDS(0, raX, rbX, sg0)
        DG_STAMP(2)
        __syncthreads();
        DG_STAMP(3)
        DG_FETCH(ab1, bb1, k01, pa1, pb1, sg1)
    } while (ab0 | bb0);
#else
    DG_FETCH(ab1, bb1, k01, pa1, pb1, sg1)
    DG_LOAD_SLAB(raY, rbY, ab1, bb1, k01, pa1, pb1)
    DG_STAMP(1)
    DG_STORE_LDS(0, raX, rbX, sg0)
    DG_STAMP(2)
    __syncthreads();
    DG_STAMP(3)
    do
    {
        const unsigned cab0 = ab0, cbb0 = bb0;
        DG_FETCH(ab0, bb0, k00, pa0, pb0, sg0)
        DG_LOAD_SLAB(raX, rbX, ab0, bb0, k00, pa0, pb0)
        DG_STAMP(4)
        DG_PRODUCTS(0, cab0, cbb0)
        DG_STAMP(5)
        DG_STORE_LDS(1, raY, rbY, sg1)
        DG_STAMP(2)
        __syncthreads();
        DG_STAMP(3)
        const unsigned cab1 = ab1, cbb1 = bb1;
        DG_FETCH(ab1, bb1, k01, pa1, pb1, sg1)
        DG_LOAD_SLAB(raY, rbY, ab1, bb1, k01, pa1, pb1)
        DG_STAMP(4)
        DG_PRODUCTS(1, cab1, cbb1)
        DG_STAMP(5)
        if (stamping)
            atomicAdd(&dbg[7], (cab1 ? 2ull : 1ull));
        DG_STORE_LDS(0, raX, rbX, sg0)
        DG_STAMP(2)
        __syncthreads();
        DG_STAMP(3)
    } while (ab0 | bb0);
#endif
#undef DG_STORE_LDS
#undef DG_FETCH
#undef DG_FILL_WINDOW
#undef DG_LOAD_SLAB
#undef DG_PRODUCTS
#undef DG_SIGNED
#undef DG_SET_SIGN
#undef DG_STEP_SIGN
#undef DG_STEP_NOSIGN
    if (product_counter && lane == 0 && nprod)
        atomicAdd(product_counter, (unsigned long long)nprod);

    if (pre)
    {
#pragma unroll
        for (int ni = 0; ni < DG_NI; ni++)
#pragma unroll
            for (int mi = 0; mi < 4; mi++)
                if ((pre >> (4 * ni + mi)) & 1u)
                {
#pragma unroll
                    for (int r = 0; r < 4; r++)
                        DG_C(ni, mi, r) = acc[ni][mi][r];
                }
        touched = 0;
    }
#pragma unroll
    for (int ni = 0; ni < DG_NI; ni++)
    {
        const unsigned t4 = (touched >> (4 * ni)) & 0xFu;
        if (!t4)
            continue;
        if (G.atomic)
        {
#pragma unroll
            for (int mi = 0; mi < 4; mi++)
            {
                if (!((t4 >> mi) & 1u))
                    continue;
#pragma unroll
                for (int r = 0; r < 4; r++)
                {
                    if (acc[ni][mi][r] != 0.0)
                        atomicAdd((double *)&DG_C(ni, mi, r), acc[ni][mi][r]);
                }
            }
            continue;
        }
        double old[4][4];
#pragma unroll
        for (int mi = 0; mi < 4; mi++)
#pragma unroll
            for (int r = 0; r < 4; r++)
                old[mi][r] = ((t4 >> mi) & 1u) ? DG_C(ni, mi, r) : 0.0;
#pragma unroll
        for (int mi = 0; mi < 4; mi++)
        {
            if (!((t4 >> mi) & 1u))
                continue;
#pragma unroll
            for (int r = 0; r < 4; r++)
                DG_C(ni, mi, r) = old[mi][r] + acc[ni][mi][r];
        }
    }
    DG_STAMP(6)
#undef DG_STAMP
#undef DG_C
}

struct MirrorJobD
{
    BlkView lo;
    const u32 *ucp;
    const u16 *uri;
    const u32 *uvi;
    val_t *uval;
    double *dense;
    const double *diag_tiles;
    unsigned long long move_bytes;
};

#define MIRROR_MAX_COLS 256
__device__ inline int mirror_column_of(const u32 *sp, int ncols, u32 p)
{
    int lo = 0, hi = ncols;
    while (hi - lo > 1)
    {
        const int mid = (lo + hi) >> 1;
        if (sp[mid] <= p)
            lo = mid;
        else
            hi = mid;
    }
    return lo;
}

__device__ inline void mirror_put(double *dense, size_t at, int nb, val_t v)
{
#if PG_PLANES > 1
    dense[at] = v.re;
    dense[at + mirror_plane_stride(nb)] = v.im;
#else
    (void)nb;
    dense[at] = v;
#endif
}
__device__ inline val_t mirror_get(const double *dense, size_t at, int nb)
{
#if PG_PLANES > 1
    return val_t{(real_t)dense[at], (real_t)dense[at + mirror_plane_stride(nb)]};
#else
    (void)nb;
    return dense[at];
#endif
}

__global__ __launch_bounds__(256) void densify_kernel(const MirrorJobD *__restrict__ jobs, int nb)
{
    __shared__ unsigned occ[16];
    __shared__ u32 sp[MIRROR_MAX_COLS + 1], su[MIRROR_MAX_COLS + 1];
    const MirrorJobD J = jobs[blockIdx.x];
    int per = (nb + (int)gridDim.y - 1) / (int)gridDim.y;
    if (per > MIRROR_MAX_COLS)
        per = MIRROR_MAX_COLS;
    const bool mapped = nb <= 256;
    unsigned short *map = reinterpret_cast<unsigned short *>(J.dense + (size_t)nb * nb);
    for (int c0 = (int)blockIdx.y * per; c0 < nb; c0 += per * (int)gridDim.y)
    {
        const int c1 = min(nb, c0 + per), ncols = c1 - c0;
        __syncthreads();
        if (threadIdx.x < 16)
            occ[threadIdx.x] = 0;
        for (int i = threadIdx.x; i <= ncols; i += blockDim.x)
        {
            sp[i] = ptr0(J.lo.ptr, c0 + i);
            su[i] = J.ucp ? J.ucp[c0 + i] : 0u;
        }
        __syncthreads();
        const u32 e0 = sp[0], e1 = sp[ncols], f0 = su[0], f1 = su[ncols];
        const bool by_tiles = mapped && !J.ucp;
        if (by_tiles)
        {
            for (u32 p0 = e0 + threadIdx.x; p0 < e1; p0 += 4 * blockDim.x)
            {
                u32 r4[4];
#pragma unroll
                for (int u = 0; u < 4; u++)
                    r4[u] = p0 + u * blockDim.x < e1 ? J.lo.idx[p0 + u * blockDim.x] : 0u;
#pragma unroll
                for (int u = 0; u < 4; u++)
                    if (p0 + u * blockDim.x < e1)
                        atomicOr(&occ[(c0 + mirror_column_of(sp, ncols, p0 + u * blockDim.x)) >> 4], 1u << (r4[u] >> 4));
            }
            __syncthreads();
            const int tpc = nb / 2;
            for (int i = threadIdx.x; i < ncols * tpc; i += blockDim.x)
            {
                const int c = c0 + i / tpc, within = i % tpc;
                if ((occ[c >> 4] >> (within >> 3)) & 1u)
                {
                    reinterpret_cast<double2 *>(J.dense + (size_t)c * nb)[within] = make_double2(0.0, 0.0);
#if PG_PLANES > 1
                    reinterpret_cast<double2 *>(J.dense + mirror_plane_stride(nb) + (size_t)c * nb)[within] = make_double2(0.0, 0.0);
#endif
                }
            }
        }
        else
        {
#if PG_PLANES > 1
          for (int pl_ = 0; pl_ < PG_PLANES; pl_++)
          {
            double *base = J.dense + pl_ * mirror_plane_stride(nb) + (size_t)c0 * nb;
#else
          {
            double *base = J.dense + (size_t)c0 * nb;
#endif
            const int words = ncols * nb;
            if ((words & 1) == 0 && (((size_t)c0 * nb) & 1) == 0)
            {
                double2 *d2 = reinterpret_cast<double2 *>(base);
                for (int i = threadIdx.x; i < words / 2; i += blockDim.x)
                    d2[i] = make_double2(0.0, 0.0);
            }
            else
                for (int i = threadIdx.x; i < words; i += blockDim.x)
                    base[i] = 0.0;
          }
        }
        __syncthreads();
        for (u32 p0 = e0 + threadIdx.x; p0 < e1; p0 += 4 * blockDim.x)
        {
            u32 r4[4];
            val_t v4[4];
#pragma unroll
            for (int u = 0; u < 4; u++)
            {
                const u32 p = p0 + u * blockDim.x;
                r4[u] = p < e1 ? J.lo.idx[p] : 0u;
                v4[u] = p < e1 ? J.lo.val[p] : v_make(0);
            }
#pragma unroll
            for (int u = 0; u < 4; u++)
            {
                const u32 p = p0 + u * blockDim.x;
                if (p < e1)
                {
                    const int c = c0 + mirror_column_of(sp, ncols, p);
                    mirror_put(J.dense, (size_t)c * nb + r4[u], nb, v4[u]);
                    if (mapped && !by_tiles)
                        atomicOr(&occ[c >> 4], 1u << (r4[u] >> 4));
                }
            }
        }
        for (u32 p = f0 + threadIdx.x; p < f1; p += blockDim.x)
        {
            const int c = c0 + mirror_column_of(su, ncols, p);
            const u32 r = J.uri[p];
            mirror_put(J.dense, (size_t)c * nb + r, nb, J.uval[J.uvi[p]]);
            if (mapped)
                atomicOr(&occ[c >> 4], 1u << (r >> 4));
        }
        if (mapped)
        {
            __syncthreads();
            const int s_ = threadIdx.x;
            if (s_ < 16 && s_ * 16 >= c0 && s_ * 16 < c1)
            {
                map[s_] = (unsigned short)occ[s_];
#if PG_PLANES > 1
                reinterpret_cast<unsigned short *>(J.dense + mirror_plane_stride(nb) + (size_t)nb * nb)[s_] = (unsigned short)occ[s_];
#endif
            }
        }
    }
}

__global__ __launch_bounds__(256) void sparsify_kernel(const MirrorJobD *__restrict__ jobs, int nb)
{
    __shared__ u32 sp[MIRROR_MAX_COLS + 1], su[MIRROR_MAX_COLS + 1];
    const MirrorJobD J = jobs[blockIdx.x];
    int per = (nb + (int)gridDim.y - 1) / (int)gridDim.y;
    if (per > MIRROR_MAX_COLS)
        per = MIRROR_MAX_COLS;
    for (int c0 = (int)blockIdx.y * per; c0 < nb; c0 += per * (int)gridDim.y)
    {
        const int c1 = min(nb, c0 + per), ncols = c1 - c0;
        __syncthreads();
        for (int i = threadIdx.x; i <= ncols; i += blockDim.x)
        {
            sp[i] = ptr0(J.lo.ptr, c0 + i);
            su[i] = J.ucp ? J.ucp[c0 + i] : 0u;
        }
        __syncthreads();
        const u32 e0 = sp[0], e1 = sp[ncols], f0 = su[0], f1 = su[ncols];
        for (u32 p0 = e0 + threadIdx.x; p0 < e1; p0 += 4 * blockDim.x)
        {
            u32 r4[4];
            val_t v4[4];
#pragma unroll
            for (int u = 0; u < 4; u++)
                r4[u] = p0 + u * blockDim.x < e1 ? J.lo.idx[p0 + u * blockDim.x] : 0u;
#pragma unroll
            for (int u = 0; u < 4; u++)
            {
                const u32 p = p0 + u * blockDim.x;
                const int c = c0 + mirror_column_of(sp, ncols, p < e1 ? p : e0);
                const u32 r = r4[u];
#if PG_PLANES == 1
                v4[u] = p >= e1 ? 0.0
                                : (J.diag_tiles && (r >> 4) == (u32)(c >> 4)) ? J.diag_tiles[((c >> 4) << 8) + ((c & 15) << 4) + (r & 15)]
                                                                            : J.dense[(size_t)c * nb + r];
#else
                v4[u] = p >= e1 ? v_make(0) : mirror_get(J.dense, (size_t)c * nb + r, nb);
#endif
            }
#pragma unroll
            for (int u = 0; u < 4; u++)
                if (p0 + u * blockDim.x < e1)
                    J.lo.val[p0 + u * blockDim.x] = v4[u];
        }
        for (u32 p = f0 + threadIdx.x; p < f1; p += blockDim.x)
        {
            const int c = c0 + mirror_column_of(su, ncols, p);
            const u32 r = J.uri[p];
#if PG_PLANES == 1
            J.uval[J.uvi[p]] = (J.diag_tiles && (r >> 4) == (u32)(c >> 4)) ? J.diag_tiles[((c >> 4) << 8) + ((c & 15) << 4) + (r & 15)]
                                                                        : J.dense[(size_t)c * nb + r];
#else
            J.uval[J.uvi[p]] = mirror_get(J.dense, (size_t)c * nb + r, nb);
#endif
        }
    }
}

__global__ __launch_bounds__(256) void ssssm_flop_count_kernel(const SsssmTaskD *__restrict__ tasks, int nb,
                                                               unsigned long long *flop_counter)
{
    const SsssmTaskD T = tasks[blockIdx.x];
    if (!T.count)
        return;
    const u32 nnzb = T.b.ptr[nb];
    unsigned long long s = 0;
    for (u32 p = threadIdx.x; p < nnzb; p += blockDim.x)
    {
        const u32 k = T.b.idx[p];
        s += T.a.ptr[k + 1] - ptr0(T.a.ptr, (int)k);
    }
    s = wave_sum(s);
    if ((threadIdx.x & 63) == 0 && s)
        atomicAdd(flop_counter, 2ull * s);
}
```

pangulu_amd/csrc/platform/pg_hip_dense_host.h:

```cpp
#pragma once

#if defined(PG_DENSE_UPDATES)

struct BlockState
{
    double *mirror = nullptr;
    bool mirror_current = false;
    bool sparse_current = true;
    bool lu_image = false;
    bool lu_map = false;
    bool written = false;
    bool densified_once = false;
    unsigned char image_halves = 0;
    u32 brow = 0, bcol = 0, nnz = 0;
    bool occ_valid = false;
    unsigned short occ_a[2] = {0, 0}, occ_b[2] = {0, 0}, occ_rows = 0, occ_cols = 0;
    unsigned short occ_map[16] = {0}, occ_map_t[16] = {0};
};

struct BlockTable
{
    struct Entry
    {
        const void *key = nullptr;
        BlockState st;
    };
    std::vector<Entry> tab;
    size_t mask = 0, count = 0;
    static size_t hash(const void *k)
    {
        unsigned long long x = (unsigned long long)(uintptr_t)k >> 3;
        x *= 0x9E3779B97F4A7C15ull;
        return (size_t)(x >> 24);
    }
    void prefetch(const void *k) const
    {
        if (count)
            __builtin_prefetch(&tab[hash(k) & mask]);
    }
    BlockState *find(const void *k)
    {
        if (count == 0)
            return nullptr;
        for (size_t i = hash(k) & mask;; i = (i + 1) & mask)
        {
            if (tab[i].key == k)
                return &tab[i].st;
            if (!tab[i].key)
                return nullptr;
        }
    }
    BlockState &operator[](const void *k)
    {
        if ((count + 1) * 2 > tab.size())
            grow();
        for (size_t i = hash(k) & mask;; i = (i + 1) & mask)
        {
            if (tab[i].key == k)
                return tab[i].st;
            if (!tab[i].key)
            {
                tab[i].key = k;
                tab[i].st = BlockState();
                count++;
                return tab[i].st;
            }
        }
    }
    void grow()
    {
        std::vector<Entry> old;
        old.swap(tab);
        tab.resize(old.empty() ? (size_t)1 << 16 : old.size() * 2);
        mask = tab.size() - 1;
        count = 0;
        for (const Entry &e : old)
            if (e.key)
                (*this)[e.key] = e.st;
    }
    void clear()
    {
        for (Entry &e : tab)
            e.key = nullptr;
        count = 0;
    }
    template <class F>
    void for_each(F f)
    {
        for (Entry &e : tab)
            if (e.key)
                f(e.st);
    }
};

struct MirrorPool
{
    std::vector<char *> chunks;
    size_t chunk_bytes = 0, cursor = 0, mirror_bytes = 0;
    size_t limit_mirrors = 0, peak = 0;
    BlockTable blocks;
    std::vector<MirrorJobD> to_densify, to_sparsify;
    std::vector<MirrorJobD> early;
    char *early_h = nullptr, *early_d = nullptr;
    size_t early_cap = 0, early_used = 0;
    unsigned long long early_jobs = 0, early_chunks = 0;
};
MirrorPool MP;

inline bool dense_mode_available(int nb)
{
    return (nb % DG_TILE == 0) && nb <= 256 && B.opt_dense_permille <= 1000;
}

inline bool is_heavy_update(u32 nnz_a, u32 nnz_b, int nb)
{
    const double full = (double)nb * (double)nb;
    const double t = (double)B.opt_dense_permille / 1000.0;
    return (double)nnz_a * (double)nnz_b >= t * t * full * full;
}

inline const void *block_key(slot_t *s)
{
    if (s->brow_pos == s->bcol_pos && s->is_upper && s->related_block)
        return (const void *)s->related_block->d_value;
    return (const void *)s->d_value;
}

BlockState &block_state(slot_t *s, int nb)
{
    s = canon_dst(s);
    BlockState &st = MP.blocks[block_key(s)];
    u32 nnz = host_nnz(s, nb);
    if (st.brow != s->brow_pos || st.bcol != s->bcol_pos || st.nnz != nnz)
    {
        double *keep = st.mirror;
        st = BlockState();
        st.mirror = keep;
        st.brow = s->brow_pos;
        st.bcol = s->bcol_pos;
        st.nnz = nnz;
    }
    return st;
}

double *obtain_mirror(BlockState &st, int nb)
{
    if (st.mirror)
        return st.mirror;
    size_t mb = PG_PLANES * (sizeof(double) * (size_t)nb * nb + MIRROR_MAP_BYTES + sizeof(double) * 16 * (size_t)nb);
    if (MP.mirror_bytes != mb)
    {
        B.generation++;
        for (char *c : MP.chunks)
            HIP_CHECK(hipFree(c));
        MP.chunks.clear();
        MP.blocks.for_each([](BlockState &st)
                           { st.mirror = nullptr; });
        MP.mirror_bytes = mb;
        MP.cursor = 0;
        MP.peak = 0;
        size_t free_b = 0, total_b = 0;
        HIP_CHECK(hipMemGetInfo(&free_b, &total_b));
        const char *frac_env = getenv("PANGULU_HIP_MIRROR_FRACTION");
        double frac = frac_env ? atof(frac_env) : 0.85;
        MP.limit_mirrors = (size_t)(frac * (double)free_b / (double)mb);
        MP.chunk_bytes = mb * 1024;
    }
    if (MP.cursor >= MP.limit_mirrors)
        return nullptr;
    size_t per_chunk = MP.chunk_bytes / mb;
    size_t chunk = MP.cursor / per_chunk, slot = MP.cursor % per_chunk;
    if (chunk >= MP.chunks.size())
    {
        char *c = nullptr;
        if (hipMalloc((void **)&c, MP.chunk_bytes) != hipSuccess)
        {
            (void)hipGetLastError();
            MP.limit_mirrors = MP.cursor;
            return nullptr;
        }
        MP.chunks.push_back(c);
    }
    MP.cursor++;
    MP.peak = std::max(MP.peak, MP.cursor);
    st.mirror = reinterpret_cast<double *>(MP.chunks[chunk] + slot * mb);
    return st.mirror;
}

MirrorJobD mirror_job(slot_t *s, double *dense, int nb)
{
    MirrorJobD J;
    memset(&J, 0, sizeof(J));
    if (s->brow_pos == s->bcol_pos)
    {
        slot_t *up, *lo;
        diag_halves(s, &up, &lo);
        J.lo = BlkView{lo->d_columnpointer, lo->d_rowindex, lo->d_value};
        const DiagAux &aux = get_diag_aux(up, nb);
        J.ucp = aux.d_cp;
        J.uri = aux.d_ri;
        J.uvi = aux.d_vi;
        J.uval = up->d_value;
    }
    else
    {
        J.lo = BlkView{s->d_columnpointer, s->d_rowindex, s->d_value};
    }
    J.dense = dense;
    {
        double nnz = host_nnz(canon_dst(s), nb);
        double ptrs = 4.0 * (nb + 1);
        if (s->brow_pos == s->bcol_pos)
        {
            slot_t *up, *lo;
            diag_halves(s, &up, &lo);
            nnz = (double)host_nnz(lo, nb) + host_nnz(up, nb);
            ptrs *= 2;
        }
        J.move_bytes = (unsigned long long)(nnz * (sizeof(double) + 2.0 + sizeof(double)) + ptrs);
    }
    return J;
}

bool mirror_is_ahead(slot_t *s)
{
    s = canon_dst(s);
    const BlockState *found = MP.blocks.find(block_key(s));
    if (!found)
        return false;
    const BlockState &st = *found;
    return st.brow == s->brow_pos && st.bcol == s->bcol_pos && st.mirror && !st.sparse_current;
}

#if defined(PG_DENSE_PANELS) || defined(PG_COMPLEX_PANELS)
const double *lu_image_of(slot_t *half)
{
    slot_t *lo = canon_dst(half);
    const BlockState *found = MP.blocks.find(block_key(lo));
    if (!found)
        return nullptr;
    const BlockState &st = *found;
    if (st.brow != lo->brow_pos || st.bcol != lo->bcol_pos || !st.lu_image || !(st.image_halves & (half->is_upper ? 2 : 1)))
        return nullptr;
    return st.mirror;
}
bool lu_image_has_map(slot_t *half)
{
    slot_t *lo = canon_dst(half);
    const BlockState *found = MP.blocks.find(block_key(lo));
    return found && found->lu_image && found->lu_map;
}
#endif
#if defined(PG_DENSE_PANELS)

std::vector<HalfImageJobD> g_half_image_jobs;
const double *request_half_image(slot_t *half, int nb)
{
    slot_t *key_slot = canon_dst(half);
    BlockState &st = block_state(key_slot, nb);
    double *m = obtain_mirror(st, nb);
    if (!m)
        return nullptr;
    slot_t *lower = half->is_upper ? half->related_block : half;
    slot_t *upper = half->is_upper ? half : half->related_block;
    HalfImageJobD J;
    memset(&J, 0, sizeof(J));
    unsigned char halves = 0;
    if (lower && lower->d_columnpointer)
    {
        J.lcp = lower->d_columnpointer;
        J.lri = lower->d_rowindex;
        J.lval = lower->d_value;
        halves |= 1;
    }
    if (upper && upper->d_rowpointer)
    {
        J.urp = upper->d_rowpointer;
        J.uci = upper->d_columnindex;
        J.uval = upper->d_value;
        halves |= 2;
    }
    J.dense = m;
    g_half_image_jobs.push_back(J);
    st.lu_image = true;
    st.lu_map = false;
    st.image_halves = halves;
    st.mirror_current = false;
    st.sparse_current = true;
    return m;
}

#endif

inline bool early_densify_on()
{
    static const bool on = getenv("PANGULU_HIP_EARLY_DENSIFY") && atoi(getenv("PANGULU_HIP_EARLY_DENSIFY")) != 0;
    return on && REC.mode == 2;
}

double *current_mirror(slot_t *s, int nb)
{
    BlockState &st = block_state(s, nb);
    double *m = obtain_mirror(st, nb);
    if (!m)
        return nullptr;
    if (!st.mirror_current)
    {
        if (early_densify_on() && !st.written && !st.densified_once)
            MP.early.push_back(mirror_job(s, m, nb));
        else
            MP.to_densify.push_back(mirror_job(s, m, nb));
        st.densified_once = true;
        st.mirror_current = true;
    }
    return m;
}

void require_sparse(slot_t *s, int nb)
{
    s = canon_dst(s);
    BlockState *found = MP.blocks.find(block_key(s));
    if (!found)
        return;
    BlockState &st = *found;
    if (st.brow != s->brow_pos || st.bcol != s->bcol_pos)
        return;
    if (!st.sparse_current && st.mirror)
    {
        MP.to_sparsify.push_back(mirror_job(s, st.mirror, nb));
        st.sparse_current = true;
    }
}

void flush_mirror_jobs(int nb, std::vector<MirrorJobD> &jobs, bool densify, bool on_records_stream = false, hipStream_t after = nullptr,
                       bool fork_recorded = false)
{
    HostTimer ht(3);
    hipStream_t st = B.stream;
    if (on_records_stream && !densify && B.opt_records_stream && !jobs.empty())
    {
        st = B.stream_rec;
        if (!fork_recorded)
            pg_event_record(B.ev_rec_fork, after ? after : B.stream);
        pg_stream_wait(st, B.ev_rec_fork);
    }
    size_t i = 0;
    while (i < jobs.size())
    {
        Segment seg = acquire_segment();
        size_t take = std::min(jobs.size() - i, seg.cap / (sizeof(MirrorJobD) + 16));
        MirrorJobD *d_jobs;
        MirrorJobD *h = seg.alloc<MirrorJobD>(take, &d_jobs);
        memcpy(h, jobs.data() + i, sizeof(MirrorJobD) * take);
        commit_segment(seg);
        static const long target_env = getenv("PANGULU_HIP_MIRROR_JOB_WGS") ? atol(getenv("PANGULU_HIP_MIRROR_JOB_WGS")) : 16384;
        unsigned slices = 16;
        while (slices > 1 && (size_t)slices * take > (size_t)target_env)
            slices >>= 1;
        slices = std::min<unsigned>(slices, (unsigned)std::max(1, nb / 16));
        {
            LaunchTimer lt(densify ? 6 : 7, st);
            if (densify)
                PG_LAUNCH(densify_kernel, dim3((unsigned)take, slices), dim3(256), 0, st, d_jobs, nb);
            else
                PG_LAUNCH(sparsify_kernel, dim3((unsigned)take, slices), dim3(256), 0, st, d_jobs, nb);
        }
        HIP_CHECK(hipGetLastError());
        B.stats.launches[densify ? 6 : 7]++;
        B.stats.tasks[densify ? 6 : 7] += take;
        for (size_t k = 0; k < take; k++)
            B.stats.alg_bytes[densify ? 6 : 7] += jobs[i + k].move_bytes;
        release_pending_segments(st);
        i += take;
    }
    if (st == B.stream_rec)
    {
        pg_event_record(B.ev_rec, st);
        B.rec_dirty.store(true, std::memory_order_release);
    }
    jobs.clear();
}

void flush_early_jobs(int nb)
{
    if (MP.early.empty())
        return;
    HostTimer ht(3);
    const size_t take = MP.early.size();
    const size_t need = sizeof(MirrorJobD) * take + 64;
    if (MP.early_used + need > MP.early_cap)
    {
        Segment seg = acquire_segment();
        if (need > seg.cap)
        {
            MP.to_densify.insert(MP.to_densify.end(), MP.early.begin(), MP.early.end());
            MP.early.clear();
            return;
        }
        MP.early_h = seg.h;
        MP.early_d = seg.d;
        MP.early_cap = seg.cap;
        MP.early_used = 0;
    }
    const size_t off = (MP.early_used + 15) & ~(size_t)15;
    memcpy(MP.early_h + off, MP.early.data(), sizeof(MirrorJobD) * take);
    const MirrorJobD *d_jobs = reinterpret_cast<const MirrorJobD *>(MP.early_d + off);
    MP.early_used = off + sizeof(MirrorJobD) * take;
    static const long target_env = getenv("PANGULU_HIP_MIRROR_JOB_WGS") ? atol(getenv("PANGULU_HIP_MIRROR_JOB_WGS")) : 16384;
    unsigned slices = 16;
    while (slices > 1 && (size_t)slices * take > (size_t)target_env)
        slices >>= 1;
    slices = std::min<unsigned>(slices, (unsigned)std::max(1, nb / 16));
    hipEvent_t ev;
    HIP_CHECK(hipEventCreateWithFlags(&ev, hipEventDisableTiming));
    REC.early_events.push_back(ev);
    REC.in_prologue = true;
    PG_LAUNCH(densify_kernel, dim3((unsigned)take, slices), dim3(256), 0, B.stream_early, d_jobs, nb);
    pg_event_record(ev, B.stream_early);
    REC.in_prologue = false;
    pg_stream_wait(B.stream, ev);
    B.stats.launches[6]++;
    B.stats.tasks[6] += take;
    for (const MirrorJobD &J : MP.early)
        B.stats.alg_bytes[6] += J.move_bytes;
    MP.early_jobs += take;
    MP.early_chunks++;
    MP.early.clear();
}

void reset_block_states()
{
    MP.blocks.for_each([](BlockState &st)
                       {
                           BlockState fresh;
                           fresh.brow = st.brow;
                           fresh.bcol = st.bcol;
                           fresh.nnz = st.nnz;
                           fresh.occ_valid = st.occ_valid;
                           fresh.occ_a[0] = st.occ_a[0];
                           fresh.occ_a[1] = st.occ_a[1];
                           fresh.occ_b[0] = st.occ_b[0];
                           fresh.occ_b[1] = st.occ_b[1];
                           fresh.occ_rows = st.occ_rows;
                           fresh.occ_cols = st.occ_cols;
                           memcpy(fresh.occ_map, st.occ_map, sizeof(fresh.occ_map));
                           memcpy(fresh.occ_map_t, st.occ_map_t, sizeof(fresh.occ_map_t));
                           st = fresh; });
    MP.cursor = 0;
    MP.to_densify.clear();
    MP.to_sparsify.clear();
    MP.early.clear();
}

#else

inline bool dense_mode_available(int) { return false; }
inline void require_sparse(slot_t *, int) {}
inline void reset_block_states() {}

#endif
```

pangulu_amd/csrc/platform/pg_hip_platform.hip:

```cpp
#include <hip/hip_runtime.h>

#include <sched.h>
#include <cctype>

#include <algorithm>
#include <chrono>
#include <cstdio>
#include <cstdlib>
#include <cstring>
#include <atomic>
#include <thread>
#include <mutex>
#include <functional>
#include <tuple>
#include <type_traits>
#include <unordered_map>
#include <unordered_set>
#include <unordered_set>
#include <vector>

#include "../../../include/pangulu_platform.h"

typedef calculate_type val_t;
typedef calculate_real_type real_t;
// ... 256 lines not shown
    u32 c0 = 0, c1 = 0, u0 = 0, u1 = 0;
    const bool atomic = G.atomic != 0;
    if (G.cdense)
    {
        for (int r = lane; r < nb; r += 64)
            acc[r] = atomic ? v_make(0) : cdense_get(G.cdense, (size_t)j * nb + r, nb);
    }
    else
    {
        c0 = ptr0(G.c.ptr, j);
        c1 = G.c.ptr[j + 1];
        for (u32 p = c0 + lane; p < c1; p += 64)
            acc[G.c.idx[p]] = atomic ? v_make(0) : G.c.val[p];
        if (G.ucp)
        {
            u0 = G.ucp[j];
            u1 = G.ucp[j + 1];
            for (u32 p = u0 + lane; p < u1; p += 64)
                acc[G.uri[p]] = atomic ? v_make(0) : G.uval[G.uvi[p]];
        }
    }
    wave_lds_fence();

    for (u32 t = G.task_begin; t < G.task_end; t++)
    {
        const BlkView A = tasks[t].a, B = tasks[t].b;
        const u32 b0 = ptr0(B.ptr, j), b1 = B.ptr[j + 1];
        for (u32 qb = b0; qb < b1; qb += 64)
        {
            const u32 cnt = min(64u, b1 - qb);
            u32 my_k = 0, my_a0 = 0, my_a1 = 0;
            val_t my_b = v_make(0);
            if ((u32)lane < cnt)
            {
                my_k = B.idx[qb + lane];
                my_b = B.val[qb + lane];
                my_a0 = ptr0(A.ptr, (int)my_k);
                my_a1 = A.ptr[my_k + 1];
            }
            if (!STRICT)
            {
                const int sub = lane / SSSSM_SUBW, sl = lane % SSSSM_SUBW;
                for (u32 i = 0; i < cnt; i += 64 / SSSSM_SUBW)
                {
                    const int src = (int)min(i + (u32)sub, cnt - 1);
                    const u32 a0 = __shfl(my_a0, src, 64);
                    const u32 a1s = __shfl(my_a1, src, 64);
                    const u32 a1 = (i + (u32)sub < cnt) ? a1s : a0;
#ifdef PANGULU_COMPLEX
                    val_t bv;
                    bv.re = __shfl(my_b.re, src, 64);
                    bv.im = __shfl(my_b.im, src, 64);
#else
                    const val_t bv = __shfl(my_b, src, 64);
#endif
                    for (u32 r = a0 + (u32)sl; r < a1; r += SSSSM_SUBW)
                    {
                        const val_t prod = v_mul(A.val[r], bv);
                        lds_atomic_sub(&acc[A.idx[r]], prod);
                        fmas++;
                    }
                }
                wave_lds_fence();
                continue;
            }
            for (u32 i = 0; i < cnt; i += 4)
            {
                u32 a0[4], a1[4], row[4];
                val_t bv[4], av[4];
                bool ok[4];
#pragma unroll
                for (int u = 0; u < 4; u++)
                {
                    const int src = (int)min(i + (u32)u, cnt - 1);
                    a0[u] = __shfl(my_a0, src, 64);
                    a1[u] = (i + (u32)u < cnt) ? __shfl(my_a1, src, 64) : a0[u];
#ifdef PANGULU_COMPLEX
                    bv[u].re = __shfl(my_b.re, src, 64);
                    bv[u].im = __shfl(my_b.im, src, 64);
#else
                    bv[u] = __shfl(my_b, src, 64);
#endif
                    const u32 r = a0[u] + (u32)lane;
                    ok[u] = r < a1[u];
                    row[u] = 0;
                    av[u] = v_make(0);
                    if (ok[u])
                    {
                        row[u] = A.idx[r];
                        av[u] = A.val[r];
                    }
                }
#pragma unroll
                for (int u = 0; u < 4; u++)
                {
                    if (ok[u])
                    {
                        acc[row[u]] = v_submul(acc[row[u]], av[u], bv[u]);
                        fmas++;
                    }
                    for (u32 r = a0[u] + 64 + lane; r < a1[u]; r += 64)
                    {
                        const u32 rr = A.idx[r];
                        acc[rr] = v_submul(acc[rr], A.val[r], bv[u]);
                        fmas++;
                    }
                    wave_lds_fence();
                }
            }
        }
    }

    if (atomic)
    {
        if (G.cdense)
        {
            for (int r = lane; r < nb; r += 64)
                cdense_atomic_add(G.cdense, (size_t)j * nb + r, nb, acc[r]);
        }
        else
        {
            for (u32 p = c0 + lane; p < c1; p += 64)
                v_atomic_add(&G.c.val[p], acc[G.c.idx[p]]);
            if (G.ucp)
                for (u32 p = u0 + lane; p < u1; p += 64)
                    v_atomic_add(&G.uval[G.uvi[p]], acc[G.uri[p]]);
        }
    }
    else if (G.cdense)
    {
        for (int r = lane; r < nb; r += 64)
            cdense_put(G.cdense, (size_t)j * nb + r, nb, acc[r]);
    }
    else
    {
        for (u32 p = c0 + lane; p < c1; p += 64)
            G.c.val[p] = acc[G.c.idx[p]];
        if (G.ucp)
        {
            for (u32 p = u0 + lane; p < u1; p += 64)
                G.uval[G.uvi[p]] = acc[G.uri[p]];
        }
    }
    wave_lds_fence();
    }
    fmas = wave_sum(fmas);
    if (lane == 0 && fmas)
        atomicAdd(flop_counter, 2ull * fmas);
}

#if defined(PG_DENSE_UPDATES)
typedef double v4f64 __attribute__((ext_vector_type(4)));
#include "pg_hip_dense.h"
#include "pg_hip_front.h"
#endif
#if defined(PG_DENSE_PANELS) || defined(PG_COMPLEX_PANELS)
#include "pg_hip_trsm_dense.h"
#include "pg_hip_trsm_ring.h"
#endif
#if defined(PG_COMPLEX_PANELS)
#include "pg_hip_panels_complex.h"
#endif

#define TRSM_WAVES 4

__global__ __launch_bounds__(TRSM_WAVES * 64) void trsm_sparse_kernel(const TrsmTaskD *__restrict__ tasks, int nb,
                                                                       unsigned long long *flop_tstrf,
                                                                       unsigned long long *flop_gessm)
{
    extern __shared__ __align__(16) unsigned char smem_raw[];
    val_t *smem = reinterpret_cast<val_t *>(smem_raw);
    const int wave = threadIdx.x >> 6, lane = threadIdx.x & 63;
    const int vblocks = (nb + TRSM_WAVES - 1) / TRSM_WAVES;
    const unsigned bid = logical_block_id((unsigned)vblocks);
    const int t = bid / vblocks;
    const int v = (bid % vblocks) * TRSM_WAVES + wave;
    if (v >= nb)
        return;
    const TrsmTaskD T = tasks[t];
    const u32 s = ptr0(T.vptr, v), e = T.vptr[v + 1];
    if (s == e)
        return;
    val_t *x = smem + (size_t)wave * nb;
    for (u32 p = s + lane; p < e; p += 64)
        x[T.vidx[p]] = T.bval[T.vmap ? T.vmap[p] : p];
    wave_lds_fence();

    unsigned long long ops = 0;
    for (u32 pb = s; pb < e; pb += 64)
    {
        const u32 cnt = min(64u, e - pb);
        u32 my_c = 0, my_t0 = 0, my_t1 = 0;
        if ((u32)lane < cnt)
        {
            my_c = T.vidx[pb + lane];
            my_t0 = T.tptr[my_c];
            my_t1 = T.tptr[my_c + 1];
        }
        u32 n_c, n_t0, n_t1, n_k = 0;
        val_t n_d = v_make(1), n_v = v_make(0);
        bool n_ok;
#define TRSM_FETCH(i_)                                                   \
    {                                                                    \
        n_c = __shfl(my_c, (int)(i_), 64);                               \
        n_t0 = __shfl(my_t0, (int)(i_), 64);                             \
        n_t1 = __shfl(my_t1, (int)(i_), 64);                             \
        if (T.is_tstrf)                                                  \
        {                                                                \
            n_d = T.tval[n_t0];                                          \
            n_t0++;                                                      \
        }                                                                \
        const u32 r_ = n_t0 + (u32)lane;                                 \
        n_ok = r_ < n_t1;                                                \
        if (n_ok)                                                        \
        {                                                                \
            n_k = T.tidx[r_];                                            \
            n_v = T.tval[r_];                                            \
        }                                                                \
    }
        TRSM_FETCH(0)
        for (u32 i = 0; i < cnt; i++)
        {
            const u32 c = n_c, t0 = n_t0, t1 = n_t1, k0 = n_k;
            const val_t d = n_d, v0 = n_v;
            const bool ok = n_ok;
            if (i + 1 < cnt)
                TRSM_FETCH(i + 1)
            val_t xc = x[c];
            if (T.is_tstrf)
            {
                xc = v_div(xc, clamp_pivot(d));
                if (lane == 0)
                {
                    x[c] = xc;
                    ops += 1;
                }
            }
            if (ok)
            {
                x[k0] = v_submul(x[k0], xc, v0);
                ops += 2;
            }
            for (u32 r = t0 + 64 + lane; r < t1; r += 64)
            {
                const u32 k = T.tidx[r];
                x[k] = v_submul(x[k], xc, T.tval[r]);
                ops += 2;
            }
            wave_lds_fence();
        }
#undef TRSM_FETCH
    }
    for (u32 p = s + lane; p < e; p += 64)
        T.bval[T.vmap ? T.vmap[p] : p] = x[T.vidx[p]];
    ops = wave_sum(ops);
    if (lane == 0 && ops)
        atomicAdd(T.is_tstrf ? flop_tstrf : flop_gessm, ops);
}

#define GETRF_THREADS 1024

__global__ __launch_bounds__(GETRF_THREADS) void getrf_kernel(const GetrfTaskD *__restrict__ tasks, int nb,
                                                              unsigned long long *flop_counter)
{
    extern __shared__ __align__(16) unsigned char smem_raw[];
    val_t *sL = reinterpret_cast<val_t *>(smem_raw);
    val_t *sU = sL + nb;
    u16 *sLi = reinterpret_cast<u16 *>(sU + nb);
    u16 *sUi = sLi + nb;
    const GetrfTaskD T = tasks[blockIdx.x];
    val_t *D = T.dense;
    const int tid = threadIdx.x;

    for (int c = tid; c < nb; c += GETRF_THREADS)
    {
        for (u32 p = T.lcp[c]; p < T.lcp[c + 1]; p++)
            D[(size_t)c * nb + T.lri[p]] = T.lval[p];
        for (u32 p = T.urp[c]; p < T.urp[c + 1]; p++)
            D[(size_t)T.uci[p] * nb + c] = T.uval[p];
    }
    __syncthreads();

    unsigned long long ops = 0;
    for (int k = 0; k < nb; k++)
    {
        const u32 u0 = T.urp[k], u1 = T.urp[k + 1];
        if (u0 == u1)
            continue;
        const u32 l0 = T.lcp[k], l1 = T.lcp[k + 1];
        const int nL = (int)(l1 - l0), nU = (int)(u1 - u0 - 1);
        if (nL == 0)
            continue;
        const val_t pivot = clamp_pivot(D[(size_t)k * nb + k]);
        for (int i = tid; i < nL; i += GETRF_THREADS)
        {
            const u32 r = T.lri[l0 + i];
            const val_t v = v_div(D[(size_t)k * nb + r], pivot);
            D[(size_t)k * nb + r] = v;
            sL[i] = v;
            sLi[i] = (u16)r;
            ops += 1;
        }
        for (int jx = tid; jx < nU; jx += GETRF_THREADS)
        {
            const u32 c = T.uci[u0 + 1 + jx];
            sU[jx] = D[(size_t)c * nb + k];
// ... 861 lines not shown
        join_records(B.stream);
        hipLaunchKernelGGL(spmv_kernel, dim3(1), dim3(256), 0, B.stream, (int)nb, a->d_columnpointer, a->d_rowindex, a->d_value, x, y);
        HIP_CHECK(hipGetLastError());
    }

    void pangulu_platform_0201001_vecadd(pangulu_int64_t length, calculate_type *bval, calculate_type *xval)
    {
        ensure_ready();
        flush_pending_getrf_locked();
        if (length <= 0)
            return;
        hipLaunchKernelGGL(vecadd_kernel, dim3((unsigned)((length + 255) / 256)), dim3(256), 0, B.stream, (long long)length, bval, xval);
        HIP_CHECK(hipGetLastError());
    }

    void pangulu_platform_0201001_sptrsv(pangulu_inblock_idx nb, pangulu_storage_slot_t *s, calculate_type *xval, pangulu_int64_t uplo)
    {
        ensure_ready();
        flush_pending_getrf_locked();
        size_t lds = sizeof(val_t) * (size_t)nb;
        join_records(B.stream);
        if (uplo == PANGULU_LOWER)
            hipLaunchKernelGGL(sptrsv_kernel, dim3(1), dim3(256), lds, B.stream, (int)nb, s->d_columnpointer, s->d_rowindex, s->d_value, xval, 0);
        else
            hipLaunchKernelGGL(sptrsv_kernel, dim3(1), dim3(256), lds, B.stream, (int)nb, s->d_rowpointer, s->d_columnindex, s->d_value, xval, 1);
        HIP_CHECK(hipGetLastError());
    }

    void *pangulu_platform_0201001_marker_record(void)
    {
        ensure_ready();
        std::lock_guard<std::mutex> g(B.mutex);
        flush_pending_getrf();
        HIP_CHECK(hipSetDevice(B.device));
        static std::vector<hipEvent_t> ring;
        static size_t next = 0;
        if (ring.empty())
        {
            ring.resize(1024);
            for (hipEvent_t &e : ring)
                HIP_CHECK(hipEventCreateWithFlags(&e, hipEventDisableTiming));
        }
        hipEvent_t e = ring[next];
        next = (next + 1) % ring.size();
        join_records(B.stream);
        join_background(B.stream);
        HIP_CHECK(hipEventRecord(e, B.stream));
        return (void *)e;
    }

    int pangulu_platform_0201001_marker_done(void *marker)
    {
        hipError_t r = hipEventQuery((hipEvent_t)marker);
        if (r == hipSuccess)
            return 1;
        if (r != hipErrorNotReady)
            HIP_CHECK(r);
        (void)hipGetLastError();
        return 0;
    }

    void pangulu_platform_0201001_marker_wait(void *marker)
    {
        HIP_CHECK(hipSetDevice(B.device));
        HIP_CHECK(hipEventSynchronize((hipEvent_t)marker));
    }

    void pangulu_platform_0201001_prepare_diag(pangulu_inblock_idx nb, pangulu_storage_slot_t *diag)
    {
        ensure_ready();
        std::lock_guard<std::mutex> g(B.mutex);
        flush_pending_getrf();
        slot_t *up, *lo;
        diag_halves(diag, &up, &lo);
        (void)get_diag_aux(up, nb);
    }

    void pangulu_platform_0201001_prepare_blocks(pangulu_inblock_idx nb, pangulu_uint64_t nslot, pangulu_storage_slot_t **slots)
    {
        flush_pending_getrf_locked();
#if defined(PG_DENSE_UPDATES)
        if (nb > 256 || nb % 16 != 0 || nslot == 0)
            return;
        static const bool enabled = !(getenv("PANGULU_HIP_OCCUPANCY_SUMMARIES") && atoi(getenv("PANGULU_HIP_OCCUPANCY_SUMMARIES")) == 0);
        if (!enabled)
            return;
        ensure_ready();
        std::lock_guard<std::mutex> g(B.mutex);
        struct Occ
        {
            unsigned short a[2], b[2], rows, cols, map[16], map_t[16];
        };
        std::vector<Occ> occ((size_t)nslot);
        const unsigned nthr = std::max(1u, std::min(32u, std::thread::hardware_concurrency()));
        std::vector<std::thread> pool;
        for (unsigned t = 0; t < nthr; t++)
            pool.emplace_back([&, t]()
                              {
                                  for (size_t i = t; i < (size_t)nslot; i += nthr)
                                  {
                                      const slot_t *s = slots[i];
                                      unsigned short m[16] = {0};
                                      const u32 *cp = s->columnpointer;
                                      const u16 *ri = s->rowindex;
                                      for (int c = 0; c < (int)nb; c++)
                                      {
                                          unsigned short bits = 0;
                                          for (u32 p = c == 0 ? 0u : cp[c]; p < cp[c + 1]; p++)
                                              bits |= (unsigned short)(1u << (ri[p] >> 4));
                                          m[c >> 4] |= bits;
                                      }
                                      Occ o;
                                      memset(&o, 0, sizeof(o));
                                      memcpy(o.map, m, sizeof(o.map));
                                      for (int c = 0; c < 16; c++)
                                          for (int r = 0; r < 16; r++)
                                              if ((m[c] >> r) & 1)
                                                  o.map_t[r] |= (unsigned short)(1u << c);
                                      for (int sl = 0; sl < (int)nb / 16; sl++)
                                      {
                                          if (m[sl] & 0x00FF)
                                              o.a[0] |= (unsigned short)(1u << sl);
                                          if (m[sl] & 0xFF00)
                                              o.a[1] |= (unsigned short)(1u << sl);
                                          o.b[sl >> 3] |= m[sl];
                                          o.rows |= m[sl];
                                          if (m[sl])
                                              o.cols |= (unsigned short)(1u << sl);
                                      }
                                      occ[i] = o;
                                  } });
        for (auto &th : pool)
            th.join();
        for (size_t i = 0; i < (size_t)nslot; i++)
        {
            BlockState &st = block_state(slots[i], (int)nb);
            st.occ_valid = true;
            st.occ_a[0] = occ[i].a[0];
            st.occ_a[1] = occ[i].a[1];
            st.occ_b[0] = occ[i].b[0];
            st.occ_b[1] = occ[i].b[1];
            st.occ_rows = occ[i].rows;
            st.occ_cols = occ[i].cols;
            memcpy(st.occ_map, occ[i].map, sizeof(st.occ_map));
            memcpy(st.occ_map_t, occ[i].map_t, sizeof(st.occ_map_t));
        }
#else
        (void)nb;
        (void)nslot;
        (void)slots;
#endif
    }

    int pangulu_platform_0201001_set_option(int option, long long value)
    {
        switch (option)
        {
        case PANGULU_HIP_OPT_HOST_MIRROR:
            B.opt_host_mirror = value;
            return 0;
        case PANGULU_HIP_OPT_DENSE_THRESHOLD_PERMILLE:
            B.opt_dense_permille = value;
            return 0;
        case PANGULU_HIP_OPT_PROFILE:
            B.opt_profile = value;
            return 0;
        case PANGULU_HIP_OPT_ASSUME_INDEPENDENT:
            B.opt_assume_independent = value;
            return 0;
        case PANGULU_HIP_OPT_GETRF_STRICT_ORDER:
            B.opt_getrf_strict = value;
            return 0;
        case PANGULU_HIP_OPT_COUNT_FLOPS:
            B.opt_count_flops = value;
            return 0;
        case PANGULU_HIP_OPT_SSSSM_GROUP_CHUNK:
            B.opt_group_chunk = value;
            return 0;
        case PANGULU_HIP_OPT_TRSM_DENSE_PERMILLE:
            B.opt_trsm_dense_permille = value;
            return 0;
        case PANGULU_HIP_OPT_TWO_STREAMS:
            B.opt_two_streams = value;
            return 0;
        case PANGULU_HIP_OPT_SMALL_LAUNCH_TASKS:
            B.opt_small_launch_tasks = value;
            return 0;
        case PANGULU_HIP_OPT_XCD_SWIZZLE:
        {
            ensure_ready();
            int v = value ? 1 : 0;
            HIP_CHECK(hipStreamSynchronize(B.stream));
            HIP_CHECK(hipMemcpyToSymbol(HIP_SYMBOL(c_xcd_swizzle), &v, sizeof(v)));
            return 0;
        }
        case PANGULU_HIP_OPT_RESET_BLOCK_STATE:
        {
            std::lock_guard<std::mutex> g(B.mutex);
            reset_block_states();
            return 0;
        }
        case PANGULU_HIP_OPT_BACKGROUND_UPDATES:
            B.opt_background_updates = value;
            return 0;
        case PANGULU_HIP_OPT_FRONT_STAGES:
            B.opt_front_stages = value;
            return 0;
        case PANGULU_HIP_OPT_TILES_STAGES:
            B.opt_tiles_stages = value;
            return 0;
        case PANGULU_HIP_OPT_QUERY_FREE_MIB:
        {
            ensure_ready();
            size_t free_b = 0, total_b = 0;
            HIP_CHECK(hipMemGetInfo(&free_b, &total_b));
            return (int)(free_b >> 20);
        }
        case PANGULU_HIP_OPT_RECORDS_STREAM:
        {
            ensure_ready();
            std::lock_guard<std::mutex> g(B.mutex);
            join_records(B.stream);
            B.opt_records_stream = value;
            return 0;
        }
        default:
            return 1;
        }
    }

    void pangulu_platform_0201001_block_trsv(pangulu_inblock_idx nb, int upper, pangulu_uint64_t nlevel, const pangulu_uint64_t *level_ptr,
                                             const pangulu_hip_solve_row_t *rows, pangulu_storage_slot_t *const *blk_slots,
                                             const pangulu_exblock_idx *blk_bcol, calculate_type *x, pangulu_uint64_t xlen)
    {
        const pangulu_hip_solve_sweep_t sw = {nlevel, level_ptr, rows, blk_slots, blk_bcol};
        const int one = 1;
        block_solve_panels((int)nb, {&sw}, {upper ? SOLVE_UPPER : SOLVE_LOWER}, x, (size_t)xlen, 1, &one);
    }

    int pangulu_platform_0201001_block_trsm_multi(pangulu_inblock_idx nb, const pangulu_hip_solve_sweep_t *lower, const pangulu_hip_solve_sweep_t *upper,
                                                  calculate_type *X, pangulu_uint64_t xlen, pangulu_uint64_t npanel, const int *w)
    {
        const int wmax = solve_widest_panel(nb);
        if (npanel == 0)
            return wmax;
        for (size_t p = 0; p < (size_t)npanel; p++)
            if (w[p] < 1 || w[p] > wmax || (w[p] & (w[p] - 1)))
            {
                fprintf(stderr, "[PanguLU-AMD ERROR] block_trsm_multi: panel width %d (nb = %d takes powers of two up to %d)\n", w[p], (int)nb, wmax);
                exit(EXIT_FAILURE);
            }
        block_solve_panels((int)nb, {lower, upper}, {SOLVE_LOWER, SOLVE_UPPER}, X, (size_t)xlen, (size_t)npanel, w);
        return wmax;
    }

    int pangulu_platform_0201001_block_trsm_multi_trans(pangulu_inblock_idx nb, const pangulu_hip_solve_sweep_t *forward_ut,
                                                        const pangulu_hip_solve_sweep_t *backward_lt, int conjugate, calculate_type *X,
                                                        pangulu_uint64_t xlen, pangulu_uint64_t npanel, const int *w)
    {
        if (solve_by_column(nb))
            return 0;
        const int wmax = solve_widest_panel(nb);
        if (npanel == 0)
            return wmax;
        for (size_t p = 0; p < (size_t)npanel; p++)
            if (w[p] < 1 || w[p] > wmax || (w[p] & (w[p] - 1)))
            {
                fprintf(stderr, "[PanguLU-AMD ERROR] block_trsm_multi_trans: panel width %d (nb = %d takes powers of two up to %d)\n", w[p], (int)nb, wmax);
                exit(EXIT_FAILURE);
            }
#ifdef PANGULU_COMPLEX
        const int conj = conjugate ? SOLVE_CONJ : 0;
#else
        const int conj = 0;
        (void)conjugate;
#endif
        block_solve_panels((int)nb, {forward_ut, backward_lt}, {SOLVE_UT | conj, SOLVE_LT | conj}, X, (size_t)xlen, (size_t)npanel, w);
        return wmax;
    }

    int pangulu_platform_0201001_block_trsm_multi_device(pangulu_inblock_idx nb, const pangulu_hip_solve_sweep_t *first,
                                                         const pangulu_hip_solve_sweep_t *second, int mode, calculate_type *d_rhs,
                                                         pangulu_uint64_t ldb, pangulu_uint64_t nrhs, pangulu_uint64_t npanel, const int *w,
                                                         pangulu_uint64_t xlen, const pangulu_hip_solve_maps_t *maps, void **workspace,
                                                         void *caller_stream)
    {
        if (mode < 0 || mode > 2 || (mode != 0 && solve_by_column(nb)))
            return 0;
        const int wmax = solve_widest_panel(nb);
        if (npanel == 0 || nrhs == 0)
            return wmax;
        pangulu_uint64_t held = 0;
        for (size_t p = 0; p < (size_t)npanel; p++)
        {
            if (w[p] < 1 || w[p] > wmax || (w[p] & (w[p] - 1)))
            {
                fprintf(stderr, "[PanguLU-AMD ERROR] block_trsm_multi_device: panel width %d (nb = %d takes powers of two up to %d)\n", w[p], (int)nb, wmax);
                exit(EXIT_FAILURE);
            }
            held += (pangulu_uint64_t)w[p];
        }
        if (held < nrhs || maps->n > xlen || maps->n_user > ldb || !workspace)
        {
            fprintf(stderr, "[PanguLU-AMD ERROR] block_trsm_multi_device: panels for %llu of %llu columns, n = %llu, xlen = %llu, ldb = %llu\n",
                    (unsigned long long)held, (unsigned long long)nrhs, (unsigned long long)maps->n, (unsigned long long)xlen, (unsigned long long)ldb);
            exit(EXIT_FAILURE);
        }
        ensure_ready();
        std::lock_guard<std::mutex> g(B.mutex);
        HIP_CHECK(hipSetDevice(B.device));
        if (!solve_pointer_on_device(d_rhs, sizeof(val_t) * ((size_t)(nrhs - 1) * (size_t)ldb + (size_t)maps->n_user)))
            return -1;
        solve_join_factor_streams();
        SolveWorkspace *ws = (SolveWorkspace *)*workspace;
        if (ws && (ws->nb != (int)nb || ws->xlen != (size_t)xlen || ws->n != (size_t)maps->n))
        {
            solve_workspace_release(ws);
            ws = nullptr;
        }
        if (!ws)
        {
            ws = new SolveWorkspace();
            ws->nb = (int)nb;
            ws->xlen = (size_t)xlen;
            ws->n = (size_t)maps->n;
            solve_workspace_alloc(*ws, &ws->d_x, (size_t)xlen * (size_t)wmax);
            HIP_CHECK(hipEventCreateWithFlags(&ws->after_caller, hipEventDisableTiming));
            *workspace = ws;
        }
        SolveWorkspace::Direction &D = ws->dir[mode == 0 ? 0 : 1];
        std::vector<SolveRowD> hr;
        std::vector<SolveBlkD> hb;
        if (!D.ready)
        {
            if (mode == 0)
                build_solve_sweeps({first, second}, {SOLVE_LOWER, SOLVE_UPPER}, hr, hb, D.sweeps);
            else
                build_solve_sweeps({first, second}, {SOLVE_UT, SOLVE_LT}, hr, hb, D.sweeps);
            solve_workspace_alloc(*ws, &D.d_rows, hr.size());
            solve_workspace_alloc(*ws, &D.d_blks, hb.size());
            HIP_CHECK(hipMemcpyAsync(D.d_rows, hr.data(), sizeof(SolveRowD) * hr.size(), hipMemcpyHostToDevice, B.stream));
            HIP_CHECK(hipMemcpyAsync(D.d_blks, hb.data(), sizeof(SolveBlkD) * hb.size(), hipMemcpyHostToDevice, B.stream));
            const size_t n = ws->n;
            solve_workspace_alloc(*ws, &D.d_in_idx, n);
            solve_workspace_alloc(*ws, &D.d_out_idx, n);
            HIP_CHECK(hipMemcpyAsync(D.d_in_idx, maps->in_idx, sizeof(u32) * n, hipMemcpyHostToDevice, B.stream));
            HIP_CHECK(hipMemcpyAsync(D.d_out_idx, maps->out_idx, sizeof(u32) * n, hipMemcpyHostToDevice, B.stream));
            if (maps->s_in)
            {
                solve_workspace_alloc(*ws, &D.d_s_in, n);
                HIP_CHECK(hipMemcpyAsync(D.d_s_in, maps->s_in, sizeof(double) * n, hipMemcpyHostToDevice, B.stream));
            }
            if (maps->s_out)
            {
                solve_workspace_alloc(*ws, &D.d_s_out, n);
                HIP_CHECK(hipMemcpyAsync(D.d_s_out, maps->s_out, sizeof(double) * n, hipMemcpyHostToDevice, B.stream));
            }
            D.ready = true;
        }
#ifdef PANGULU_COMPLEX
        const int conj = mode == 2 ? SOLVE_CONJ : 0;
#else
        const int conj = 0;
#endif
        HIP_CHECK(hipEventRecord(ws->after_caller, (hipStream_t)caller_stream));
        HIP_CHECK(hipStreamWaitEvent(B.stream, ws->after_caller, 0));
        u32 j0 = 0;
        for (size_t p = 0; p < (size_t)npanel && j0 < (u32)nrhs; p++)
        {
            const u32 nc = std::min<u32>((u32)w[p], (u32)nrhs - j0);
            launch_solve_pack_of(w[p], true, d_rhs, (size_t)ldb, j0, nc, *ws, D);
            launch_solve_panel_of(w[p], (int)nb, D.sweeps, conj, D.d_rows, D.d_blks, ws->d_x);
            launch_solve_pack_of(w[p], false, d_rhs, (size_t)ldb, j0, nc, *ws, D);
            j0 += nc;
        }
        HIP_CHECK(hipStreamSynchronize(B.stream));
        return wmax;
    }

    void pangulu_platform_0201001_solve_workspace_free(void **workspace)
    {
        if (!workspace || !*workspace)
            return;
        std::lock_guard<std::mutex> g(B.mutex);
        solve_workspace_release((SolveWorkspace *)*workspace);
        *workspace = nullptr;
    }

    unsigned long long pangulu_platform_0201001_get_solve_workspace_bytes(void)
    {
        std::lock_guard<std::mutex> g(B.mutex);
        return (unsigned long long)g_solve_workspace_bytes;
    }

    void pangulu_platform_0201001_block_spmv_add(pangulu_inblock_idx nb, pangulu_uint64_t nblk, pangulu_storage_slot_t *const *slots,
                                                 const pangulu_exblock_idx *src_seg, const pangulu_exblock_idx *dst_seg, const int *csr,
                                                 const calculate_type *x, calculate_type *y, pangulu_uint64_t xlen)
    {
        ensure_ready();
        std::lock_guard<std::mutex> g(B.mutex);
        flush_pending_getrf();
        HIP_CHECK(hipSetDevice(B.device));
        join_records(B.stream);
        join_background(B.stream);
        std::vector<SpmvBlkD> hb(std::max<size_t>((size_t)nblk, 1));
        for (size_t i = 0; i < (size_t)nblk; i++)
        {
            const slot_t *s = slots[i];
            hb[i].ptr = csr[i] ? s->d_rowpointer : s->d_columnpointer;
            hb[i].idx = csr[i] ? s->d_columnindex : s->d_rowindex;
            hb[i].val = s->d_value;
            hb[i].src = src_seg[i];
            hb[i].dst = dst_seg[i];
            hb[i].csr = csr[i] ? 1u : 0u;
            hb[i].pad_ = 0;
        }
        SpmvBlkD *d_blks = nullptr;
        val_t *d_x = nullptr, *d_y = nullptr;
        HIP_CHECK(hipMalloc((void **)&d_blks, sizeof(SpmvBlkD) * hb.size()));
        HIP_CHECK(hipMalloc((void **)&d_x, sizeof(val_t) * (size_t)xlen));
        HIP_CHECK(hipMalloc((void **)&d_y, sizeof(val_t) * (size_t)xlen));
        HIP_CHECK(hipMemcpyAsync(d_blks, hb.data(), sizeof(SpmvBlkD) * hb.size(), hipMemcpyHostToDevice, B.stream));
        HIP_CHECK(hipMemcpyAsync(d_x, x, sizeof(val_t) * (size_t)xlen, hipMemcpyHostToDevice, B.stream));
        HIP_CHECK(hipMemcpyAsync(d_y, y, sizeof(val_t) * (size_t)xlen, hipMemcpyHostToDevice, B.stream));
        if (nblk)
            hipLaunchKernelGGL(block_spmv_add_kernel, dim3((unsigned)nblk), dim3(256), 0, B.stream, d_blks, (int)nb, d_x, d_y);
        HIP_CHECK(hipGetLastError());
        HIP_CHECK(hipMemcpyAsync(y, d_y, sizeof(val_t) * (size_t)xlen, hipMemcpyDeviceToHost, B.stream));
        HIP_CHECK(hipStreamSynchronize(B.stream));
        HIP_CHECK(hipFree(d_blks));
        HIP_CHECK(hipFree(d_x));
        HIP_CHECK(hipFree(d_y));
    }

    static unsigned long long options_signature()
    {
        const long long v[] = {B.opt_host_mirror, B.opt_dense_permille, B.opt_profile, B.opt_assume_independent, B.opt_getrf_strict, B.opt_count_flops,
                               B.opt_group_chunk, B.opt_small_launch_tasks, B.opt_trsm_dense_permille, B.opt_two_streams, B.opt_records_stream,
                               B.opt_background_updates, B.opt_front_stages, B.opt_front_unit, B.opt_tiles_stages, B.opt_tiles_unit, B.opt_front_min_wgs};
        unsigned long long h = 1469598103934665603ull;
        for (long long x : v)
        {
            h ^= (unsigned long long)x;
            h *= 1099511628211ull;
        }
        return h;
    }

    static void drop_schedule()
    {
        for (Recorder::Seg &sg : REC.segs)
        {
            if (sg.h)
                (void)hipHostFree(sg.h);
            if (sg.twin)
                (void)hipFree(sg.twin);
        }
        for (hipEvent_t e : REC.early_events)
            (void)hipEventDestroy(e);
#if defined(PG_DENSE_UPDATES)
        MP.early.clear();
        MP.early_h = MP.early_d = nullptr;
        MP.early_cap = MP.early_used = 0;
#endif
        REC = Recorder();
    }

    static void host_counters_delta(const pangulu_hip_stats_t &before, const pangulu_hip_stats_t &after, pangulu_hip_stats_t &d)
    {
        memset(&d, 0, sizeof(d));
        for (int c = 0; c < PANGULU_HIP_STAT_CLASSES; c++)
        {
            d.launches[c] = after.launches[c] - before.launches[c];
            d.tasks[c] = after.tasks[c] - before.tasks[c];
            d.alg_bytes[c] = after.alg_bytes[c] - before.alg_bytes[c];
        }
        d.trsm_dense_tasks = after.trsm_dense_tasks - before.trsm_dense_tasks;
    }
    static void host_counters_add(pangulu_hip_stats_t &to, const pangulu_hip_stats_t &d)
    {
        for (int c = 0; c < PANGULU_HIP_STAT_CLASSES; c++)
        {
            to.launches[c] += d.launches[c];
            to.tasks[c] += d.tasks[c];
            to.alg_bytes[c] += d.alg_bytes[c];
        }
        to.trsm_dense_tasks += d.trsm_dense_tasks;
    }

    long long pangulu_platform_0201001_schedule(int cmd, const void *owner)
    {
        ensure_ready();
        std::lock_guard<std::mutex> g(B.mutex);
        if (cmd == 6)
            return (long long)REC.ops.size();
        if (cmd == 9)
            return (REC.valid && REC.owner == owner && REC.signature == options_signature() && REC.generation == B.generation) ? 0 : 1;
        flush_pending_getrf();
        HIP_CHECK(hipSetDevice(B.device));
        switch (cmd)
        {
        case 0:
            if (!owner || owner == REC.owner)
            {
                HIP_CHECK(hipDeviceSynchronize());
                drop_schedule();
            }
            return 0;
        case 1:
        case 4:
        case 5:
            HIP_CHECK(hipDeviceSynchronize());
            drop_schedule();
            if (B.opt_profile || B.opt_host_mirror || !B.opt_assume_independent)
                return -1;
            REC.mode = cmd == 4 ? 2 : 1;
            REC.pack = true;
            REC.owner = owner;
            REC.signature = options_signature();
            REC.stats_before = B.stats;
            REC.wgs_before[0] = B.front_workgroups;
            REC.wgs_before[1] = B.general_workgroups;
            REC.wgs_before[2] = B.chase_launches;
            REC.wgs_before[3] = B.chase_solves;
            return 0;
        case 2:
        {
            if (REC.mode == 0)
                return -1;
            const int mode = REC.mode;
            REC.mode = 0;
            HIP_CHECK(hipDeviceSynchronize());
            for (Recorder::Seg &sg : REC.segs)
            {
                HIP_CHECK(hipMemcpy(sg.twin, sg.h, sg.cap, hipMemcpyHostToDevice));
                HIP_CHECK(hipHostFree(sg.h));
                sg.h = sg.d = nullptr;
            }
            host_counters_delta(REC.stats_before, B.stats, REC.stats_delta);
            REC.wgs_delta[0] = B.front_workgroups - REC.wgs_before[0];
            REC.wgs_delta[1] = B.general_workgroups - REC.wgs_before[1];
            REC.wgs_delta[2] = B.chase_launches - REC.wgs_before[2];
            REC.wgs_delta[3] = B.chase_solves - REC.wgs_before[3];
            if (mode == 2)
            {
                for (int c = 0; c < PANGULU_HIP_STAT_CLASSES; c++)
                {
                    B.stats.launches[c] = REC.stats_before.launches[c];
                    B.stats.tasks[c] = REC.stats_before.tasks[c];
                    B.stats.alg_bytes[c] = REC.stats_before.alg_bytes[c];
                }
                B.stats.trsm_dense_tasks = REC.stats_before.trsm_dense_tasks;
                B.front_workgroups = REC.wgs_before[0];
                B.general_workgroups = REC.wgs_before[1];
                B.chase_launches = REC.wgs_before[2];
                B.chase_solves = REC.wgs_before[3];
            }
#if defined(PG_DENSE_UPDATES)
            if (!MP.early.empty())
            {
                fprintf(stderr, "[PanguLU-AMD ERROR] %zu early densify jobs were never given a wait point\n", MP.early.size());
                exit(EXIT_FAILURE);
            }
            if (getenv("PANGULU_AMD_TRACE") && MP.early_chunks)
                fprintf(stderr, "[pangulu_amd trace] schedule: %llu first-touch densify jobs moved into %llu prologue chunks on the early stream\n",
                        MP.early_jobs, MP.early_chunks);
            MP.early_jobs = MP.early_chunks = 0;
#endif
            REC.nb = B.nb_cfg;
            REC.generation = B.generation;
            REC.valid = true;
            return (long long)REC.ops.size();
        }
        case 7:
            if (!REC.valid || REC.owner != owner || REC.signature != options_signature() || REC.generation != B.generation)
                return 1;
            for (auto &op : REC.prologue)
                op();
            return 0;
        case 8:
            if (!REC.valid || REC.owner != owner)
                return 1;
            HIP_CHECK(hipGetLastError());
            host_counters_add(B.stats, REC.stats_delta);
            B.front_workgroups += REC.wgs_delta[0];
            B.general_workgroups += REC.wgs_delta[1];
            B.chase_launches += REC.wgs_delta[2];
            B.chase_solves += REC.wgs_delta[3];
            B.rec_dirty.store(true, std::memory_order_release);
            return 0;
        case 3:
            if (!REC.valid || REC.owner != owner || REC.signature != options_signature() || REC.generation != B.generation)
                return 1;
            for (auto &op : REC.prologue)
                op();
            for (auto &op : REC.ops)
                op();
            HIP_CHECK(hipGetLastError());
            host_counters_add(B.stats, REC.stats_delta);
            B.front_workgroups += REC.wgs_delta[0];
            B.general_workgroups += REC.wgs_delta[1];
            B.chase_launches += REC.wgs_delta[2];
            B.chase_solves += REC.wgs_delta[3];
            B.rec_dirty.store(true, std::memory_order_release);
            return 0;
        default:
            return -1;
        }
    }

    int pangulu_platform_0201001_schedule_range(const void *owner, long long first, long long last)
    {
        std::lock_guard<std::mutex> g(B.mutex);
        if (!REC.valid || REC.owner != owner || first < 0 || last > (long long)REC.ops.size() || first > last)
            return 1;
        HIP_CHECK(hipSetDevice(B.device));
        for (long long i = first; i < last; i++)
            REC.ops[(size_t)i]();
        return 0;
    }

    void *pangulu_platform_0201001_marker_record_replay(void)
    {
        std::lock_guard<std::mutex> g(B.mutex);
        HIP_CHECK(hipSetDevice(B.device));
        static std::vector<hipEvent_t> ring;
        static size_t next = 0;
        if (ring.empty())
        {
            ring.resize(4096);
            for (hipEvent_t &e : ring)
                HIP_CHECK(hipEventCreateWithFlags(&e, hipEventDisableTiming));
        }
        hipEvent_t e = ring[next];
        next = (next + 1) % ring.size();
        HIP_CHECK(hipEventRecord(e, B.stream));
        return (void *)e;
    }

    void *pangulu_platform_0201001_get_stream(void)
    {
        ensure_ready();
        return (void *)B.stream;
    }

    void pangulu_platform_0201001_get_memory(unsigned long long out[4])
    {
        std::lock_guard<std::mutex> g(B.mutex);
        out[0] = out[1] = out[2] = out[3] = 0;
#if defined(PG_DENSE_UPDATES)
        out[0] = (unsigned long long)MP.chunks.size() * MP.chunk_bytes;
        out[3] = (unsigned long long)MP.peak;
#endif
        out[1] = (unsigned long long)REC.descriptor_bytes;
        out[2] = B.getrf_scratch ? (unsigned long long)B.getrf_scratch_slots * std::max(sizeof(val_t), sizeof(double)) * (size_t)B.nb_cfg * B.nb_cfg : 0ull;
    }

    void pangulu_platform_0201001_get_stats(pangulu_hip_stats_t *out, int reset)
    {
        flush_pending_getrf_locked();
        if (reset && getenv("PANGULU_HIP_HOST_TIMING"))
        {
            fprintf(stderr, "[PanguLU-AMD] host seconds in the back-end: calls %.4f (ssssm %.4f, trsm %.4f, getrf %.4f, mirror jobs %.4f, staging waits %.4f)\n",
                    g_host_seconds[5], g_host_seconds[0], g_host_seconds[1], g_host_seconds[2], g_host_seconds[3], g_host_seconds[4]);
            for (double &x : g_host_seconds)
                x = 0;
        }
        ensure_ready();
        std::lock_guard<std::mutex> g(B.mutex);
        join_records(B.stream);
        join_background(B.stream);
        HIP_CHECK(hipStreamSynchronize(B.stream));
        harvest_events();
        unsigned long long f[PG_FLOP_WORDS];
        HIP_CHECK(hipMemcpy(f, B.d_flops, sizeof(f), hipMemcpyDeviceToHost));
        if (getenv("PANGULU_HIP_DEBUG_SSSSM"))
            fprintf(stderr, "[ssssm_dense stamps, every 64th workgroup, shader clocks] bookkeeping+first step %llu | barrier A %llu | LDS stage (waits for the slab) %llu | barrier B %llu | next step + loads issued %llu | mfma %llu | C update %llu | slab steps %llu, empty workgroups %llu\n",
                    f[8], f[9], f[10], f[11], f[12], f[13], f[14], f[15] & 0xFFFFFFFFull, f[15] >> 32);
        if (getenv("PANGULU_HIP_DEBUG_TRSM"))
            fprintf(stderr, "[trsm stamps, every 64th workgroup, shader clocks] setup+x loads %llu | prefetch issue %llu | barrier A %llu | stage %llu | barrier B %llu | mfma loop %llu | tail chain %llu | stores %llu, empty workgroups %llu\n",
                    f[8], f[9], f[10], f[11], f[12], f[13], f[14], f[15] & ((1ull << 40) - 1), f[15] >> 40);
        if (getenv("PANGULU_HIP_DEBUG_GETRF"))
            fprintf(stderr, "[getrf stamps, block 0, shader clocks; tiled kernel: 1 = diag+priority tiles, 2 = trailing passes, 3 = wait for LU, 4 = substitution (wavefront 0), lu = tile LU (wavefront 7)] prologue %llu | 1 %llu | 2 %llu | 3 %llu | 4 %llu | loop %llu | gather %llu | lu %llu\n",
                    f[8], f[9], f[10], f[11], f[12], f[13], f[14], f[15]);
        if (getenv("PANGULU_HIP_DEBUG_GETRF"))
            fprintf(stderr, "[getrf_pipe stamps, block 0, shader clocks; factorisation wavefront: wait A %llu | tile LU %llu | inverses %llu | wait B %llu | wait C %llu; trailing wavefront 1: update %llu | wait B %llu | panel+strip %llu | wait C %llu | hand-over %llu | wait A %llu]\n",
                    f[8 + 16], f[8 + 17], f[8 + 18], f[8 + 19], f[8 + 20], f[8 + 24], f[8 + 25], f[8 + 26], f[8 + 27], f[8 + 28], f[8 + 29]);
        for (int c = 1; c <= 5; c++)
            B.stats.flops[c] = (double)f[c];
        B.stats.mfma_flops_executed = 8192.0 * (double)(f[6] + f[7]);
        B.stats.ssssm_front_flops_executed = 8192.0 * (double)f[7];
        B.stats.ssssm_front_workgroups = B.front_workgroups;
        B.stats.ssssm_general_workgroups = B.general_workgroups;
        B.stats.chase_launches = B.chase_launches;
        B.stats.chase_solves = B.chase_solves;
        if (out)
            *out = B.stats;
        if (reset)
        {
            memset(&B.stats, 0, sizeof(B.stats));
            B.mfma_flops_executed = 0;
            B.front_workgroups = B.general_workgroups = 0;
            B.chase_launches = B.chase_solves = 0;
            HIP_CHECK(hipMemset(B.d_flops, 0, sizeof(f)));
        }
// ... 3 lines not shown
```

pangulu_amd/solver.py:

```python
import ctypes
import sys

import numpy as np

from . import _lib


class Handle:

    def __init__(self, lib, vtype):
        self.lib = lib
        self.vtype = vtype
        self.dtype = _lib.VALUE_TYPES[vtype][0]
        self.ptr = ctypes.c_void_p(None)
        self.n = 0
        self._keep = []

    @property
    def ref(self):
        return ctypes.byref(self.ptr)

    def info(self):
        out = _lib.Info()
        self.lib.pangulu_amd_get_info(self.ref, ctypes.byref(out))
# ... 134 lines not shown
        nrhs = B.shape[1]
        ptr = x.ctypes.data_as(ctypes.c_void_p)
    else:
        x, ptr = None, None
    if code != 0:
        rc = h.lib.pangulu_amd_gstrs_trans(ptr, int(nrhs), h.n, code, ctypes.byref(opt), h.ref)
        if rc != 0:
            raise RuntimeError("pangulu_amd_gstrs_trans failed (%d): %s" % (rc, _GSTRS_ERRORS.get(rc, "?")))
        return x
    rc = h.lib.pangulu_amd_gstrs_multi(ptr, int(nrhs), h.n, ctypes.byref(opt), h.ref)
    if rc != 0:
        raise RuntimeError("pangulu_amd_gstrs_multi failed (%d): %s" % (rc, "the handle has not been factorised" if rc == 1 else "bad rhs / ldb"))
    return x


def last_solve_path(h):
    d, w, p = ctypes.c_int(), ctypes.c_int(), ctypes.c_int()
    h.lib.pangulu_amd_last_solve_path(h.ref, ctypes.byref(d), ctypes.byref(w), ctypes.byref(p))
    return {"device_columns": int(d.value), "panel_width": int(w.value), "panels": int(p.value)}


def pangulu_gssv(h, rhs):
    pangulu_gstrf(h)
    return pangulu_gstrs(h, rhs)


def pangulu_finalize(h):
    if h.ptr:
        h.lib.pangulu_finalize(h.ref)
    h.ptr = ctypes.c_void_p(None)



def owned_blocks(h):
    nb = int(h.info()["nb"])
    cnt = h.lib.pangulu_amd_owned_block_count(h.ref)
    for i in range(cnt):
        brow, bcol = ctypes.c_uint32(), ctypes.c_uint32()
        up, nnz = ctypes.c_int(), ctypes.c_ulonglong()
        cp, ri, va = ctypes.c_void_p(), ctypes.c_void_p(), ctypes.c_void_p()
        rc = h.lib.pangulu_amd_owned_block(h.ref, i, ctypes.byref(brow), ctypes.byref(bcol), ctypes.byref(up), ctypes.byref(nnz),
                                           ctypes.byref(cp), ctypes.byref(ri), ctypes.byref(va))
        assert rc == 0
        k = int(nnz.value)
        colptr = np.ctypeslib.as_array(ctypes.cast(cp, ctypes.POINTER(ctypes.c_uint32)), shape=(nb + 1,)).copy()
        if k:
            rowidx = np.ctypeslib.as_array(ctypes.cast(ri, ctypes.POINTER(ctypes.c_uint16)), shape=(k,)).copy()
            raw = np.ctypeslib.as_array(ctypes.cast(va, ctypes.POINTER(ctypes.c_uint8)), shape=(k * np.dtype(h.dtype).itemsize,))
            values = raw.view(h.dtype).copy()
        else:
            rowidx = np.zeros(0, np.uint16)
            values = np.zeros(0, h.dtype)
        yield int(brow.value), int(bcol.value), int(up.value), colptr, rowidx, values


def permutation(h):
    p = h.lib.pangulu_amd_get_perm(h.ref)
    return np.ctypeslib.as_array(p, shape=(int(h.info()["n_padded"]),)).copy()


def factors_as_scipy(h):
    import scipy.sparse as sp

    info = h.info()
    nb, n = int(info["nb"]), int(info["n_padded"])
    npad = int(info["block_length"]) * nb
    rows_l, cols_l, vals_l, rows_u, cols_u, vals_u = [], [], [], [], [], []
    for brow, bcol, up, cp, ri, va in owned_blocks(h):
        major = np.repeat(np.arange(nb, dtype=np.int64), np.diff(cp.astype(np.int64)))
        minor = ri.astype(np.int64)
        if brow == bcol and up:
            r, c = major + brow * nb, minor + bcol * nb
            rows_u.append(r), cols_u.append(c), vals_u.append(va)
        elif brow < bcol:
            r, c = minor + brow * nb, major + bcol * nb
            rows_u.append(r), cols_u.append(c), vals_u.append(va)
        else:
            r, c = minor + brow * nb, major + bcol * nb
            rows_l.append(r), cols_l.append(c), vals_l.append(va)

    def build(rows, cols, vals):
        if not rows:
            return sp.csc_matrix((npad, npad), dtype=h.dtype)
        return sp.csc_matrix((np.concatenate(vals), (np.concatenate(rows), np.concatenate(cols))), shape=(npad, npad))

    L = build(rows_l, cols_l, vals_l)[:n, :n] + sp.identity(n, dtype=h.dtype, format="csc")
    U = build(rows_u, cols_u, vals_u)[:n, :n]
    return L.tocsc(), U.tocsc()


def update_values(h, csc_value):
    if csc_value is not None:
        va = np.ascontiguousarray(csc_value, dtype=h.dtype)
        ptr = va.ctypes.data_as(ctypes.c_void_p)
    else:
        ptr = None
    rc = h.lib.pangulu_amd_update_values(h.ref, ptr)
    if rc != 0:
        raise RuntimeError("pangulu_amd_update_values failed (%d)" % rc)


def factor_check(h):
    out = ctypes.c_double(0.0)
    rc = h.lib.pangulu_amd_factor_check(h.ref, ctypes.byref(out))
    if rc != 0:
        raise RuntimeError("pangulu_amd_factor_check: the handle has not been factorised")
    return float(out.value)


def factor_check_vectors(h, nvec=8, seed=20251003):
    out = ctypes.c_double(0.0)
    rc = h.lib.pangulu_amd_factor_check_vectors(h.ref, int(nvec), int(seed), ctypes.byref(out))
    if rc != 0:
        raise RuntimeError("pangulu_amd_factor_check_vectors: the handle has not been factorised")
    return float(out.value)


MODEL_FIELDS = ("T_star_s", "sum_over_ranks_s", "link_term_s_max", "sent_bytes", "critical_path_s", "latency_chain_s", "rank_flop_share",
                "rank_T_star_share", "hbm_bytes_fullest_rank", "hbm_records_owned", "hbm_records_received", "hbm_dense_mirrors")


def model_for_ranks(h, nranks):
    out = (ctypes.c_double * 12)()
    if h.lib.pangulu_amd_model_for_ranks(h.ref, int(nranks), out) != 0:
        return None
    return dict(zip(MODEL_FIELDS, (float(x) for x in out)))


def hip_memory(h_or_lib):
    lib = h_or_lib.lib if isinstance(h_or_lib, Handle) else h_or_lib
    v = (ctypes.c_ulonglong * 4)()
    lib.pangulu_platform_0201001_get_memory(v)
    return {"mirror_pool_bytes": int(v[0]), "schedule_descriptor_bytes": int(v[1]), "getrf_scratch_bytes": int(v[2]), "dense_mode_blocks": int(v[3]),
            "solve_workspace_bytes": int(lib.pangulu_platform_0201001_get_solve_workspace_bytes())}


def hip_stats(h_or_lib, reset=False):
    lib = h_or_lib.lib if isinstance(h_or_lib, Handle) else h_or_lib
    st = _lib.HipStats()
    lib.pangulu_platform_0201001_get_stats(ctypes.byref(st), 1 if reset else 0)
    out = {}
    for k, name in _lib.KERNEL_CLASSES.items():
        out[name] = dict(launches=int(st.launches[k]), tasks=int(st.tasks[k]), alg_bytes=float(st.alg_bytes[k]),
                         flops=float(st.flops[k]), elapsed_ms=float(st.elapsed_ms[k]))
    out["ssssm_dense_mfma"]["mfma_flops_executed"] = float(st.mfma_flops_executed)
    out["tstrf"]["dense_path_tasks"] = int(st.trsm_dense_tasks)
    out["ssssm_dense_mfma"]["front_workgroups"] = int(st.ssssm_front_workgroups)
    out["ssssm_dense_mfma"]["general_workgroups"] = int(st.ssssm_general_workgroups)
    out["ssssm_dense_mfma"]["front_kernel_ms"] = float(st.ssssm_kernel_ms[0])
    out["ssssm_dense_mfma"]["general_kernel_ms"] = float(st.ssssm_kernel_ms[1])
    out["ssssm_dense_mfma"]["front_flops_executed"] = float(st.ssssm_front_flops_executed)
    out["getrf"]["chase_launches"] = int(st.chase_launches)
    out["tstrf"]["chase_solves"] = int(st.chase_solves)
    return out
```

Before: 49710.

## Specialise first-touch densify using precomputed occupancy maps and A-entry lists

Record at preprocessing how many original A entries fall into each off-diagonal block and upload per-block packed lists of their positions to the device. First-touch densify jobs for blocks with no A entries become a cheap tile-clearing kernel. Blocks that do have A entries scatter only those entries instead of walking the full record pattern, and occupancy tiles are taken from the host-side map instead of being rebuilt with atomics. This adds device memory for the entry lists, extra host bookkeeping in scatter_values, and a second kernel launch per densify batch.

```diff
diff --git a/include/pangulu_platform.h b/include/pangulu_platform.h
--- a/include/pangulu_platform.h
+++ b/include/pangulu_platform.h
@@ -168,6 +168,8 @@
     int pangulu_platform_0201001_set_option(int option, long long value);
     void pangulu_platform_0201001_prepare_diag(pangulu_inblock_idx nb, pangulu_storage_slot_t *diag);
     void pangulu_platform_0201001_prepare_blocks(pangulu_inblock_idx nb, pangulu_uint64_t nslot, pangulu_storage_slot_t **slots);
+    void pangulu_platform_0201001_prepare_fill(pangulu_inblock_idx nb, pangulu_uint64_t nslot, pangulu_storage_slot_t **slots,
+                                               const unsigned int *a_entries, const unsigned int *a_list_off, const unsigned int *d_a_list);
     void *pangulu_platform_0201001_marker_record(void);
     int pangulu_platform_0201001_marker_done(void *marker);
     void pangulu_platform_0201001_marker_wait(void *marker);
@@ -228,6 +230,8 @@
         unsigned long long chase_launches, chase_solves;
         double ssssm_kernel_ms[2];
         double ssssm_front_flops_executed;
+        unsigned long long densify_jobs[3];
+        double densify_record_bytes[3];
     } pangulu_hip_stats_t;
     void pangulu_platform_0201001_get_stats(pangulu_hip_stats_t *out, int reset);
     void pangulu_platform_0201001_get_memory(unsigned long long out[4]);
diff --git a/pangulu_amd/_lib.py b/pangulu_amd/_lib.py
--- a/pangulu_amd/_lib.py
+++ b/pangulu_amd/_lib.py
@@ -113,6 +113,8 @@
         ("chase_solves", ctypes.c_ulonglong),
         ("ssssm_kernel_ms", ctypes.c_double * 2),
         ("ssssm_front_flops_executed", ctypes.c_double),
+        ("densify_jobs", ctypes.c_ulonglong * 3),
+        ("densify_record_bytes", ctypes.c_double * 3),
     ]
 
 
diff --git a/pangulu_amd/csrc/host/pg_api.cpp b/pangulu_amd/csrc/host/pg_api.cpp
--- a/pangulu_amd/csrc/host/pg_api.cpp
+++ b/pangulu_amd/csrc/host/pg_api.cpp
@@ -68,6 +68,7 @@
     p.set_option = pangulu_platform_0201001_set_option;
     p.prepare_diag = pangulu_platform_0201001_prepare_diag;
     p.prepare_blocks = pangulu_platform_0201001_prepare_blocks;
+    p.prepare_fill = pangulu_platform_0201001_prepare_fill;
     p.marker_record = pangulu_platform_0201001_marker_record;
     p.marker_done = pangulu_platform_0201001_marker_done;
     p.marker_wait = pangulu_platform_0201001_marker_wait;
@@ -200,6 +201,14 @@
 {
 
 #ifdef PANGULU_AMD_TEST_HOOKS
+    long long pangulu_amd_test_slot_a_entries(void **pangulu_handle, long long idx)
+    {
+        Solver *S = (Solver *)*pangulu_handle;
+        if (idx < 0 || (size_t)idx >= S->storage.a_entries.size())
+            return -1;
+        return (long long)S->storage.a_entries[(size_t)idx];
+    }
+
     int pangulu_amd_use_platform_library(const char *so_path, unsigned int platform_id)
     {
         void *h = dlopen(so_path, RTLD_NOW | RTLD_LOCAL);
diff --git a/pangulu_amd/csrc/host/pg_host.h b/pangulu_amd/csrc/host/pg_host.h
--- a/pangulu_amd/csrc/host/pg_host.h
+++ b/pangulu_amd/csrc/host/pg_host.h
@@ -58,6 +58,7 @@
     int (*set_option)(int, long long) = nullptr;
     void (*prepare_diag)(pangulu_inblock_idx, slot_t *) = nullptr;
     void (*prepare_blocks)(pangulu_inblock_idx, pangulu_uint64_t, slot_t **) = nullptr;
+    void (*prepare_fill)(pangulu_inblock_idx, pangulu_uint64_t, slot_t **, const unsigned int *, const unsigned int *, const unsigned int *) = nullptr;
     void *(*marker_record)() = nullptr;
     int (*marker_done)(void *) = nullptr;
     void (*marker_wait)(void *) = nullptr;
@@ -137,6 +138,9 @@
     u32 nb = 0;
     std::vector<slot_t> owned;
     size_t n_owned_nondiag = 0;
+    std::vector<u32> a_entries;
+    std::vector<u32> a_list_off, a_list;
+    u32 *d_a_list = nullptr;
     char *harena = nullptr, *darena = nullptr;
     std::vector<char *> dchunks;
     size_t dchunk_bytes = 0;
@@ -363,7 +367,7 @@
 
 void assign_subtrees(Solver &S);
 void preprocess(Solver &S, const CscMatrix &Aperm);
-void scatter_values(Solver &S, const CscMatrix &Aperm);
+void scatter_values(Solver &S, const CscMatrix &Aperm, bool build_lists);
 void reload_values(Solver &S, const CscMatrix &Aperm);
 void numeric_factorize(Solver &S);
 void record_schedule(Solver &S);
diff --git a/pangulu_amd/csrc/host/pg_preprocess.cpp b/pangulu_amd/csrc/host/pg_preprocess.cpp
--- a/pangulu_amd/csrc/host/pg_preprocess.cpp
+++ b/pangulu_amd/csrc/host/pg_preprocess.cpp
@@ -362,11 +362,22 @@
     }
 }
 
-void scatter_values(Solver &S, const CscMatrix &A)
+void scatter_values(Solver &S, const CscMatrix &A, bool build_lists)
 {
     const BlockPattern &P = S.pat;
     const u32 nb = S.nb, n = S.n;
     const int me = S.rank;
+    std::vector<u32> &placed = S.storage.a_entries;
+    placed.assign(S.storage.owned.size(), 0u);
+    const slot_t *owned0 = S.storage.owned.data();
+    const size_t noff = S.storage.n_owned_nondiag;
+    build_lists = build_lists && nb <= 256;
+    std::vector<u32> ent_slot, ent_code;
+    if (build_lists)
+    {
+        ent_slot.assign(A.rowidx.size(), ~0u);
+        ent_code.assign(A.rowidx.size(), 0u);
+    }
 #pragma omp parallel for schedule(dynamic, 256)
     for (i64 j_ = 0; j_ < (i64)n; j_++)
     {
@@ -404,7 +415,29 @@
             if (hit == b1 || *hit != minor)
                 fatal("entry (%u,%u) of A outside the symbolic pattern", i, j);
             s->value[hit - s->rowindex] = A.value[p];
-        }
+            if (s >= owned0 && s < owned0 + placed.size())
+            {
+#pragma omp atomic
+                placed[(size_t)(s - owned0)]++;
+                if (build_lists && (size_t)(s - owned0) < noff)
+                {
+                    ent_slot[p] = (u32)(s - owned0);
+                    ent_code[p] = (u32)(hit - s->rowindex) << 16 | c << 8 | r;
+                }
+            }
+        }
+    }
+    if (build_lists)
+    {
+        std::vector<u32> &off = S.storage.a_list_off, &list = S.storage.a_list;
+        off.assign(noff + 1, 0u);
+        for (size_t i = 0; i < noff; i++)
+            off[i + 1] = off[i] + placed[i];
+        list.assign(off[noff], 0u);
+        std::vector<u32> cursor(off.begin(), off.end() - 1);
+        for (size_t p = 0; p < ent_slot.size(); p++)
+            if (ent_slot[p] != ~0u)
+                list[cursor[ent_slot[p]]++] = ent_code[p];
     }
 }
 
@@ -416,7 +449,7 @@
     for (auto &s : st.owned)
         if (s.value)
             memset((void *)s.value, 0, sizeof(val_t) * (size_t)s.columnpointer[nb]);
-    scatter_values(S, A);
+    scatter_values(S, A, false);
     if (!plat.host_memory)
     {
         plat.synchronize();
@@ -676,7 +709,7 @@
     }
 
     if (!analysis_only)
-        scatter_values(S, A);
+        scatter_values(S, A, true);
 
     lap("patterns + values into the records");
     S.remain.assign(nblk, 0);
@@ -928,6 +961,18 @@
             for (size_t i = 0; i < st.n_owned_nondiag; i++)
                 offdiag[i] = &st.owned[i];
             plat.prepare_blocks((pangulu_inblock_idx)nb, offdiag.size(), offdiag.data());
+            if (plat.prepare_fill)
+            {
+                if (!st.a_list.empty())
+                {
+                    plat.malloc_((void **)&st.d_a_list, sizeof(u32) * st.a_list.size());
+                    plat.memcpy_(st.d_a_list, st.a_list.data(), sizeof(u32) * st.a_list.size(), 0);
+                    plat.synchronize();
+                }
+                plat.prepare_fill((pangulu_inblock_idx)nb, offdiag.size(), offdiag.data(), st.a_entries.data(),
+                                  st.d_a_list ? st.a_list_off.data() : nullptr, st.d_a_list);
+                std::vector<u32>().swap(st.a_list);
+            }
         }
         lap("back-end preparation (diagonal column views, pattern summaries)");
     }
@@ -966,6 +1011,8 @@
         else
             plat.free_(arena_snapshot);
     }
+    if (storage.d_a_list)
+        plat.free_(storage.d_a_list);
     if (storage.harena)
     {
         for (char *c : storage.dchunks)
diff --git a/pangulu_amd/csrc/platform/pg_hip_backend.h b/pangulu_amd/csrc/platform/pg_hip_backend.h
--- a/pangulu_amd/csrc/platform/pg_hip_backend.h
+++ b/pangulu_amd/csrc/platform/pg_hip_backend.h
@@ -43,6 +43,7 @@
     hipStream_t stream_front = nullptr;
     hipEvent_t ev_front_fork = nullptr, ev_front_join = nullptr;
     long long opt_front_fork = 1;
+    long long opt_densify_fast = 1;
     bool getrf_join_pending = false;
     hipStream_t stream_rec = nullptr;
     hipEvent_t ev_rec_fork = nullptr, ev_rec = nullptr;
@@ -244,6 +245,8 @@
     HIP_CHECK(hipEventCreateWithFlags(&B.ev_front_join, hipEventDisableTiming));
     if (const char *e = getenv("PANGULU_HIP_FRONT_FORK"))
         B.opt_front_fork = atol(e);
+    if (const char *e = getenv("PANGULU_HIP_DENSIFY_FAST"))
+        B.opt_densify_fast = atol(e) != 0;
     HIP_CHECK(hipEventCreateWithFlags(&B.ev_fork, hipEventDisableTiming));
     HIP_CHECK(hipEventCreateWithFlags(&B.ev_join, hipEventDisableTiming));
     HIP_CHECK(hipStreamCreateWithFlags(&B.stream3, hipStreamNonBlocking));
diff --git a/pangulu_amd/csrc/platform/pg_hip_dense.h b/pangulu_amd/csrc/platform/pg_hip_dense.h
--- a/pangulu_amd/csrc/platform/pg_hip_dense.h
+++ b/pangulu_amd/csrc/platform/pg_hip_dense.h
@@ -460,6 +460,12 @@
     double *dense;
     const double *diag_tiles;
     unsigned long long move_bytes;
+    unsigned short map[16];
+    unsigned char has_map;
+    const u32 *alist;
+    unsigned acount;
+    unsigned char census_class;
+    unsigned record_bytes;
 };
 
 #define MIRROR_MAX_COLS 256
@@ -515,7 +521,7 @@
             occ[threadIdx.x] = 0;
         for (int i = threadIdx.x; i <= ncols; i += blockDim.x)
         {
-            sp[i] = ptr0(J.lo.ptr, c0 + i);
+            sp[i] = J.alist ? 0u : ptr0(J.lo.ptr, c0 + i);
             su[i] = J.ucp ? J.ucp[c0 + i] : 0u;
         }
         __syncthreads();
@@ -523,16 +529,24 @@
         const bool by_tiles = mapped && !J.ucp;
         if (by_tiles)
         {
-            for (u32 p0 = e0 + threadIdx.x; p0 < e1; p0 += 4 * blockDim.x)
-            {
-                u32 r4[4];
-#pragma unroll
-                for (int u = 0; u < 4; u++)
-                    r4[u] = p0 + u * blockDim.x < e1 ? J.lo.idx[p0 + u * blockDim.x] : 0u;
-#pragma unroll
-                for (int u = 0; u < 4; u++)
-                    if (p0 + u * blockDim.x < e1)
-                        atomicOr(&occ[(c0 + mirror_column_of(sp, ncols, p0 + u * blockDim.x)) >> 4], 1u << (r4[u] >> 4));
+            if (J.has_map)
+            {
+                if (threadIdx.x < 16)
+                    occ[threadIdx.x] = jobs[blockIdx.x].map[threadIdx.x];
+            }
+            else
+            {
+                for (u32 p0 = e0 + threadIdx.x; p0 < e1; p0 += 4 * blockDim.x)
+                {
+                    u32 r4[4];
+#pragma unroll
+                    for (int u = 0; u < 4; u++)
+                        r4[u] = p0 + u * blockDim.x < e1 ? J.lo.idx[p0 + u * blockDim.x] : 0u;
+#pragma unroll
+                    for (int u = 0; u < 4; u++)
+                        if (p0 + u * blockDim.x < e1)
+                            atomicOr(&occ[(c0 + mirror_column_of(sp, ncols, p0 + u * blockDim.x)) >> 4], 1u << (r4[u] >> 4));
+                }
             }
             __syncthreads();
             const int tpc = nb / 2;
@@ -595,6 +609,14 @@
                 }
             }
         }
+        if (J.alist)
+            for (u32 p = threadIdx.x; p < J.acount; p += blockDim.x)
+            {
+                const u32 w = J.alist[p];
+                const int c = (int)((w >> 8) & 255u);
+                if (c >= c0 && c < c1)
+                    mirror_put(J.dense, (size_t)c * nb + (w & 255u), nb, J.lo.val[w >> 16]);
+            }
         for (u32 p = f0 + threadIdx.x; p < f1; p += blockDim.x)
         {
             const int c = c0 + mirror_column_of(su, ncols, p);
diff --git a/pangulu_amd/csrc/platform/pg_hip_dense_host.h b/pangulu_amd/csrc/platform/pg_hip_dense_host.h
--- a/pangulu_amd/csrc/platform/pg_hip_dense_host.h
+++ b/pangulu_amd/csrc/platform/pg_hip_dense_host.h
@@ -16,6 +16,9 @@
     bool occ_valid = false;
     unsigned short occ_a[2] = {0, 0}, occ_b[2] = {0, 0}, occ_rows = 0, occ_cols = 0;
     unsigned short occ_map[16] = {0}, occ_map_t[16] = {0};
+    bool fill_known = false, fill_only = false;
+    const u32 *a_list = nullptr;
+    u32 a_count = 0;
 };
 
 struct BlockTable
@@ -218,6 +221,46 @@
             ptrs *= 2;
         }
         J.move_bytes = (unsigned long long)(nnz * (sizeof(double) + 2.0 + sizeof(double)) + ptrs);
+        J.record_bytes = (unsigned)(nnz * (sizeof(val_t) + 2.0) + ptrs);
+    }
+    J.census_class = 2;
+    return J;
+}
+
+MirrorJobD densify_job(slot_t *s, const BlockState &st, double *m, int nb)
+{
+    MirrorJobD J = mirror_job(s, m, nb);
+    const bool summarised = s->brow_pos != s->bcol_pos && st.occ_valid && nb <= 256;
+    const bool first = !st.written && !st.densified_once;
+    if (summarised && B.opt_densify_fast)
+    {
+        memcpy(J.map, st.occ_map, sizeof(J.map));
+        J.has_map = 1;
+    }
+    if (summarised && first && st.fill_known)
+    {
+        if (!st.fill_only)
+        {
+            if (B.opt_densify_fast && st.a_list)
+            {
+                J.census_class = 1;
+                J.alist = st.a_list;
+                J.acount = st.a_count;
+                unsigned live = 0;
+                for (int c = 0; c < nb / 16; c++)
+                    live += (unsigned)__builtin_popcount(st.occ_map[c]);
+                J.move_bytes = sizeof(MirrorJobD) + (unsigned long long)PG_PLANES * (2048ull * live + 2ull * (nb / 16)) +
+                               (unsigned long long)st.a_count * (4 + 2 * sizeof(val_t));
+            }
+        }
+        else if (B.opt_densify_fast)
+        {
+            J.census_class = 0;
+            unsigned live = 0;
+            for (int c = 0; c < nb / 16; c++)
+                live += (unsigned)__builtin_popcount(st.occ_map[c]);
+            J.move_bytes = sizeof(MirrorClearJobD) + (unsigned long long)PG_PLANES * (2048ull * live + 2ull * (nb / 16));
+        }
     }
     return J;
 }
@@ -307,9 +350,9 @@
     if (!st.mirror_current)
     {
         if (early_densify_on() && !st.written && !st.densified_once)
-            MP.early.push_back(mirror_job(s, m, nb));
+            MP.early.push_back(densify_job(s, st, m, nb));
         else
-            MP.to_densify.push_back(mirror_job(s, m, nb));
+            MP.to_densify.push_back(densify_job(s, st, m, nb));
         st.densified_once = true;
         st.mirror_current = true;
     }
@@ -332,6 +375,53 @@
     }
 }
 
+inline unsigned mirror_job_slices(size_t jobs, int nb)
+{
+    static const long target_env = getenv("PANGULU_HIP_MIRROR_JOB_WGS") ? atol(getenv("PANGULU_HIP_MIRROR_JOB_WGS")) : 16384;
+    unsigned slices = 16;
+    while (slices > 1 && (size_t)slices * jobs > (size_t)target_env)
+        slices >>= 1;
+    return std::min<unsigned>(slices, (unsigned)std::max(1, nb / 16));
+}
+
+void launch_densify_jobs(const MirrorJobD *jobs, size_t take, char *h, char *d, int nb, hipStream_t st)
+{
+    size_t nc = 0;
+    for (size_t k = 0; k < take; k++)
+        nc += jobs[k].census_class == 0;
+    const size_t ns = take - nc, off = (sizeof(MirrorClearJobD) * nc + 15) & ~(size_t)15;
+    MirrorClearJobD *hc = reinterpret_cast<MirrorClearJobD *>(h);
+    MirrorJobD *hs = reinterpret_cast<MirrorJobD *>(h + off);
+    for (size_t k = 0, ic = 0, is = 0; k < take; k++)
+    {
+        const MirrorJobD &J = jobs[k];
+        if (J.census_class == 0)
+        {
+            hc[ic].dense = J.dense;
+            memcpy(hc[ic].map, J.map, sizeof(J.map));
+            ic++;
+        }
+        else
+            hs[is++] = J;
+        B.stats.alg_bytes[6] += J.move_bytes;
+        B.stats.densify_jobs[J.census_class]++;
+        B.stats.densify_record_bytes[J.census_class] += J.record_bytes;
+    }
+    if (nc)
+    {
+        PG_LAUNCH(mirror_clear_kernel, dim3((unsigned)(nc * (size_t)(nb / 16))), dim3(256), 0, st, reinterpret_cast<const MirrorClearJobD *>(d), nb,
+                  (int)PG_PLANES, mirror_plane_stride(nb));
+        B.stats.launches[6]++;
+    }
+    if (ns)
+    {
+        const unsigned slices = mirror_job_slices(ns, nb);
+        PG_LAUNCH(densify_kernel, dim3((unsigned)ns, slices), dim3(256), 0, st, reinterpret_cast<const MirrorJobD *>(d + off), nb);
+        B.stats.launches[6]++;
+    }
+    B.stats.tasks[6] += take;
+}
+
 void flush_mirror_jobs(int nb, std::vector<MirrorJobD> &jobs, bool densify, bool on_records_stream = false, hipStream_t after = nullptr,
                        bool fork_recorded = false)
 {
@@ -349,27 +439,31 @@
     {
         Segment seg = acquire_segment();
         size_t take = std::min(jobs.size() - i, seg.cap / (sizeof(MirrorJobD) + 16));
-        MirrorJobD *d_jobs;
-        MirrorJobD *h = seg.alloc<MirrorJobD>(take, &d_jobs);
-        memcpy(h, jobs.data() + i, sizeof(MirrorJobD) * take);
-        commit_segment(seg);
-        static const long target_env = getenv("PANGULU_HIP_MIRROR_JOB_WGS") ? atol(getenv("PANGULU_HIP_MIRROR_JOB_WGS")) : 16384;
-        unsigned slices = 16;
-        while (slices > 1 && (size_t)slices * take > (size_t)target_env)
-            slices >>= 1;
-        slices = std::min<unsigned>(slices, (unsigned)std::max(1, nb / 16));
-        {
-            LaunchTimer lt(densify ? 6 : 7, st);
-            if (densify)
-                PG_LAUNCH(densify_kernel, dim3((unsigned)take, slices), dim3(256), 0, st, d_jobs, nb);
-            else
+        if (densify)
+        {
+            char *d_raw;
+            char *h_raw = seg.alloc<char>(sizeof(MirrorJobD) * take + 16, &d_raw);
+            commit_segment(seg);
+            LaunchTimer lt(6, st);
+            launch_densify_jobs(jobs.data() + i, take, h_raw, d_raw, nb, st);
+        }
+        else
+        {
+            MirrorJobD *d_jobs;
+            MirrorJobD *h = seg.alloc<MirrorJobD>(take, &d_jobs);
+            memcpy(h, jobs.data() + i, sizeof(MirrorJobD) * take);
+            commit_segment(seg);
+            const unsigned slices = mirror_job_slices(take, nb);
+            {
+                LaunchTimer lt(7, st);
                 PG_LAUNCH(sparsify_kernel, dim3((unsigned)take, slices), dim3(256), 0, st, d_jobs, nb);
+            }
+            B.stats.launches[7]++;
+            B.stats.tasks[7] += take;
+            for (size_t k = 0; k < take; k++)
+                B.stats.alg_bytes[7] += jobs[i + k].move_bytes;
         }
         HIP_CHECK(hipGetLastError());
-        B.stats.launches[densify ? 6 : 7]++;
-        B.stats.tasks[densify ? 6 : 7] += take;
-        for (size_t k = 0; k < take; k++)
-            B.stats.alg_bytes[densify ? 6 : 7] += jobs[i + k].move_bytes;
         release_pending_segments(st);
         i += take;
     }
@@ -403,26 +497,15 @@
         MP.early_used = 0;
     }
     const size_t off = (MP.early_used + 15) & ~(size_t)15;
-    memcpy(MP.early_h + off, MP.early.data(), sizeof(MirrorJobD) * take);
-    const MirrorJobD *d_jobs = reinterpret_cast<const MirrorJobD *>(MP.early_d + off);
-    MP.early_used = off + sizeof(MirrorJobD) * take;
-    static const long target_env = getenv("PANGULU_HIP_MIRROR_JOB_WGS") ? atol(getenv("PANGULU_HIP_MIRROR_JOB_WGS")) : 16384;
-    unsigned slices = 16;
-    while (slices > 1 && (size_t)slices * take > (size_t)target_env)
-        slices >>= 1;
-    slices = std::min<unsigned>(slices, (unsigned)std::max(1, nb / 16));
+    MP.early_used = off + sizeof(MirrorJobD) * take + 16;
     hipEvent_t ev;
     HIP_CHECK(hipEventCreateWithFlags(&ev, hipEventDisableTiming));
     REC.early_events.push_back(ev);
     REC.in_prologue = true;
-    PG_LAUNCH(densify_kernel, dim3((unsigned)take, slices), dim3(256), 0, B.stream_early, d_jobs, nb);
+    launch_densify_jobs(MP.early.data(), take, MP.early_h + off, MP.early_d + off, nb, B.stream_early);
     pg_event_record(ev, B.stream_early);
     REC.in_prologue = false;
     pg_stream_wait(B.stream, ev);
-    B.stats.launches[6]++;
-    B.stats.tasks[6] += take;
-    for (const MirrorJobD &J : MP.early)
-        B.stats.alg_bytes[6] += J.move_bytes;
     MP.early_jobs += take;
     MP.early_chunks++;
     MP.early.clear();
@@ -445,6 +528,10 @@
                            fresh.occ_cols = st.occ_cols;
                            memcpy(fresh.occ_map, st.occ_map, sizeof(fresh.occ_map));
                            memcpy(fresh.occ_map_t, st.occ_map_t, sizeof(fresh.occ_map_t));
+                           fresh.fill_known = st.fill_known;
+                           fresh.fill_only = st.fill_only;
+                           fresh.a_list = st.a_list;
+                           fresh.a_count = st.a_count;
                            st = fresh; });
     MP.cursor = 0;
     MP.to_densify.clear();
diff --git a/pangulu_amd/csrc/platform/pg_hip_mirror_clear.h b/pangulu_amd/csrc/platform/pg_hip_mirror_clear.h
--- /dev/null
+++ b/pangulu_amd/csrc/platform/pg_hip_mirror_clear.h
@@ -0,0 +1,28 @@
+#pragma once
+
+struct MirrorClearJobD
+{
+    double *dense;
+    unsigned short map[16];
+};
+
+__global__ __launch_bounds__(256) void mirror_clear_kernel(const MirrorClearJobD *__restrict__ jobs, int nb, int planes, size_t plane_stride)
+{
+    const unsigned slabs = (unsigned)nb / 16u;
+    const MirrorClearJobD *J = jobs + blockIdx.x / slabs;
+    const int slab = (int)(blockIdx.x % slabs);
+    double *dense = J->dense;
+    const unsigned live = J->map[slab];
+    const int tpc = nb / 2;
+    if (live)
+        for (int i = (int)threadIdx.x; i < 16 * tpc; i += 256)
+        {
+            const int c = slab * 16 + i / tpc, within = i % tpc;
+            if ((live >> (within >> 3)) & 1u)
+                for (int pl = 0; pl < planes; pl++)
+                    reinterpret_cast<double2 *>(dense + (size_t)pl * plane_stride + (size_t)c * nb)[within] = make_double2(0.0, 0.0);
+        }
+    if (threadIdx.x == 0)
+        for (int pl = 0; pl < planes; pl++)
+            reinterpret_cast<unsigned short *>(dense + (size_t)pl * plane_stride + (size_t)nb * nb)[slab] = (unsigned short)live;
+}
diff --git a/pangulu_amd/csrc/platform/pg_hip_platform.hip b/pangulu_amd/csrc/platform/pg_hip_platform.hip
--- a/pangulu_amd/csrc/platform/pg_hip_platform.hip
+++ b/pangulu_amd/csrc/platform/pg_hip_platform.hip
@@ -432,6 +432,7 @@
 #if defined(PG_DENSE_UPDATES)
 typedef double v4f64 __attribute__((ext_vector_type(4)));
 #include "pg_hip_dense.h"
+#include "pg_hip_mirror_clear.h"
 #include "pg_hip_front.h"
 #endif
 #if defined(PG_DENSE_PANELS) || defined(PG_COMPLEX_PANELS)
@@ -1599,6 +1600,33 @@
 #endif
     }
 
+    void pangulu_platform_0201001_prepare_fill(pangulu_inblock_idx nb, pangulu_uint64_t nslot, pangulu_storage_slot_t **slots,
+                                               const unsigned int *a_entries, const unsigned int *a_list_off, const unsigned int *d_a_list)
+    {
+        flush_pending_getrf_locked();
+#if defined(PG_DENSE_UPDATES)
+        if (nb > 256 || nb % 16 != 0 || nslot == 0 || !a_entries)
+            return;
+        ensure_ready();
+        std::lock_guard<std::mutex> g(B.mutex);
+        for (size_t i = 0; i < (size_t)nslot; i++)
+        {
+            BlockState &st = block_state(slots[i], (int)nb);
+            st.fill_known = true;
+            st.fill_only = a_entries[i] == 0;
+            st.a_count = a_entries[i];
+            st.a_list = (a_list_off && d_a_list && a_list_off[i + 1] - a_list_off[i] == a_entries[i]) ? d_a_list + a_list_off[i] : nullptr;
+        }
+#else
+        (void)nb;
+        (void)nslot;
+        (void)slots;
+        (void)a_entries;
+        (void)a_list_off;
+        (void)d_a_list;
+#endif
+    }
+
     int pangulu_platform_0201001_set_option(int option, long long value)
     {
         switch (option)
@@ -1884,7 +1912,8 @@
     {
         const long long v[] = {B.opt_host_mirror, B.opt_dense_permille, B.opt_profile, B.opt_assume_independent, B.opt_getrf_strict, B.opt_count_flops,
                                B.opt_group_chunk, B.opt_small_launch_tasks, B.opt_trsm_dense_permille, B.opt_two_streams, B.opt_records_stream,
-                               B.opt_background_updates, B.opt_front_stages, B.opt_front_unit, B.opt_tiles_stages, B.opt_tiles_unit, B.opt_front_min_wgs};
+                               B.opt_background_updates, B.opt_front_stages, B.opt_front_unit, B.opt_tiles_stages, B.opt_tiles_unit, B.opt_front_min_wgs,
+                               B.opt_densify_fast};
         unsigned long long h = 1469598103934665603ull;
         for (long long x : v)
         {
@@ -1923,6 +1952,11 @@
             d.alg_bytes[c] = after.alg_bytes[c] - before.alg_bytes[c];
         }
         d.trsm_dense_tasks = after.trsm_dense_tasks - before.trsm_dense_tasks;
+        for (int k = 0; k < 3; k++)
+        {
+            d.densify_jobs[k] = after.densify_jobs[k] - before.densify_jobs[k];
+            d.densify_record_bytes[k] = after.densify_record_bytes[k] - before.densify_record_bytes[k];
+        }
     }
     static void host_counters_add(pangulu_hip_stats_t &to, const pangulu_hip_stats_t &d)
     {
@@ -1933,6 +1967,11 @@
             to.alg_bytes[c] += d.alg_bytes[c];
         }
         to.trsm_dense_tasks += d.trsm_dense_tasks;
+        for (int k = 0; k < 3; k++)
+        {
+            to.densify_jobs[k] += d.densify_jobs[k];
+            to.densify_record_bytes[k] += d.densify_record_bytes[k];
+        }
     }
 
     long long pangulu_platform_0201001_schedule(int cmd, const void *owner)
@@ -1998,6 +2037,11 @@
                     B.stats.alg_bytes[c] = REC.stats_before.alg_bytes[c];
                 }
                 B.stats.trsm_dense_tasks = REC.stats_before.trsm_dense_tasks;
+                for (int k = 0; k < 3; k++)
+                {
+                    B.stats.densify_jobs[k] = REC.stats_before.densify_jobs[k];
+                    B.stats.densify_record_bytes[k] = REC.stats_before.densify_record_bytes[k];
+                }
                 B.front_workgroups = REC.wgs_before[0];
                 B.general_workgroups = REC.wgs_before[1];
                 B.chase_launches = REC.wgs_before[2];
diff --git a/pangulu_amd/solver.py b/pangulu_amd/solver.py
--- a/pangulu_amd/solver.py
+++ b/pangulu_amd/solver.py
@@ -310,4 +310,7 @@
     out["ssssm_dense_mfma"]["front_flops_executed"] = float(st.ssssm_front_flops_executed)
     out["getrf"]["chase_launches"] = int(st.chase_launches)
     out["tstrf"]["chase_solves"] = int(st.chase_solves)
+    for k, name in enumerate(("clear_only", "pristine_with_a", "other")):
+        out["densify"][name + "_jobs"] = int(st.densify_jobs[k])
+        out["densify"][name + "_record_bytes"] = float(st.densify_record_bytes[k])
     return out
```

Measured after the change: 50850 (median of 6 runs). 1.02x the previous value.
